# ming71/rotate-yolov3

Measured on AMD Instinct MI355X. Metric: images/sec fwd+bwd at 608^2 (train step, backend=hip), higher is better.
Workload: dtype bf16; 1 GPU; configs[3]: Darknet-53 train step (fwd + riou loss + bwd + grad all-reduce + SGD), bs=64/GPU 608x608, synthetic HRSC-shaped targets; global_batch=64, parallelism=dp1, gradients=250 MB fp32 in 4 flat buckets, fp32 on the wire

## Files before the change

### __graft_entry__.py

```python
import os
import subprocess
import sys

ROOT = os.path.dirname(os.path.abspath(__file__))
PKG = os.path.join(ROOT, "rotate-yolov3_amd")
CSRC = os.path.join(PKG, "csrc")
LIB = os.path.join(PKG, "libryolo_hip.so")
LIB_ABL = os.path.join(PKG, "libryolo_hip_ablation.so")

UNITS = {
    "rnms.hip": ["-ffp-contract=off", "-fhip-fp32-correctly-rounded-divide-sqrt"],
    "conv.hip": [],
    "conv_dispatch.hip": [],
    "conv_dgrad.hip": [],
    "conv_mp.hip": [],
    "conv_mq.hip": [],
    "conv_stem.hip": [],
    "conv_pw.hip": [],
    "conv_dil.hip": [],
    "conv0_bwd.hip": [],
    "yolo.hip": [],
    "se.hip": [],
    "se_bwd.hip": [],
    "skewiou.hip": ["-ffp-contract=off"],
    "wgrad.hip": [],
    "wgrad_dil.hip": [],
    "train.hip": [],
    "optim.hip": ["-ffp-contract=off", "-fhip-fp32-correctly-rounded-divide-sqrt"],
    "loss.hip": ["-ffp-contract=off"],
    "augment.hip": ["-ffp-contract=off", "-fhip-fp32-correctly-rounded-divide-sqrt"],
    "letterbox_area.hip": ["-ffp-contract=off", "-fhip-fp32-correctly-rounded-divide-sqrt"],
    "detpost.hip": ["-ffp-contract=off", "-fhip-fp32-correctly-rounded-divide-sqrt"],
}
COMMON = ["--offload-arch=gfx950", "-O3", "-std=c++17", "-fPIC", "-fno-gpu-rdc", "-Wno-unused-value"]


def _sha(*chunks):
    import hashlib
    h = hashlib.sha256()
    for c in chunks:
        h.update(c if isinstance(c, bytes) else str(c).encode())
        h.update(b"\0")
    return h.hexdigest()


def _headers():
    hs = [os.path.join(ROOT, "include", "ryolo.h")] + sorted(os.path.join(CSRC, h) for h in os.listdir(CSRC) if h.endswith(".h"))
    return [open(h, "rb").read() for h in hs]


def unit_hashes(defines=()):
    hdr = _headers()
    out = {}
    for unit, extra in sorted(UNITS.items()):
        src = os.path.join(CSRC, unit)
        if os.path.exists(src):
            out[unit] = _sha(open(src, "rb").read(), *hdr, " ".join(COMMON + list(defines) + extra))
    return out


def source_id(defines=()):
    hs = unit_hashes(defines)
    return _sha(*["%s=%s" % kv for kv in sorted(hs.items())])[:16]


def embedded_id(lib):
    if not os.path.exists(lib):
        return None
    data = open(lib, "rb").read()
    k = data.find(b"RYOLO_BUILD_ID=")
    return data[k + 15:k + 31].decode("ascii", "replace") if k >= 0 else None


def _compile(lib, objsuffix, defines, force=False):
    hipcc = os.environ.get("HIPCC", "hipcc")
    objs = []
    hashes = unit_hashes(defines)
    for unit, extra in UNITS.items():
        src = os.path.join(CSRC, unit)
        if not os.path.exists(src):
            continue
        obj = os.path.join(CSRC, unit.replace(".hip", objsuffix))
        side = obj + ".hash"
        have = open(side).read().strip() if os.path.exists(side) and os.path.exists(obj) else None
        if force or have != hashes[unit]:
            subprocess.run([hipcc] + COMMON + defines + extra + ["-c", src, "-o", obj], check=True)
            with open(side, "w") as fh:
                fh.write(hashes[unit])
        objs.append(obj)
    want = source_id(defines)
    if force or embedded_id(lib) != want:
        idobj = os.path.join(CSRC, "build_id" + objsuffix)
        subprocess.run([hipcc] + COMMON + defines + ['-DRYOLO_BUILD_ID="%s"' % want, "-c", os.path.join(CSRC, "build_id.hip"), "-o", idobj],
                       check=True)
        subprocess.run([hipcc, "--offload-arch=gfx950", "-shared", "-fPIC", "-o", lib] + objs + [idobj], check=True)
    assert embedded_id(lib) == want, "library %s carries id %s, sources are %s" % (lib, embedded_id(lib), want)
    return want


def build_ablation(force=False):
    _compile(LIB_ABL, ".abl.o", ["-DRYOLO_MP_ABLATION"], force)
    return LIB_ABL


def build(force=False):
    bid = _compile(LIB, ".o", [], force)
    subprocess.run(["make", "-C", os.path.join(ROOT, "oracle"), "-s"], check=True)
    if ROOT not in sys.path:
        sys.path.insert(0, ROOT)
    import rotate_yolov3_amd
    from rotate_yolov3_amd import _lib
    assert _lib.lib().ryolo_abi_version() >= 1
    got = _lib.lib().ryolo_build_id().decode()
    assert got == "RYOLO_BUILD_ID=" + bid, (got, bid)
    print("build id %s (library == sources)" % bid)


def smoke():
    if ROOT not in sys.path:
        sys.path.insert(0, ROOT)
    import numpy as np
    import torch
    assert torch.cuda.is_available(), "smoke() needs cuda:0"
    if not os.path.exists(LIB):
        build()
    from rotate_yolov3_amd import _lib
    lib_id, src_id = _lib.lib().ryolo_build_id().decode().split("=", 1)[1], source_id()
    assert lib_id == src_id, "libryolo_hip.so was built from other sources (library %s, tree %s): run build()" % (lib_id, src_id)
    print("smoke: build id %s (the loaded library is this tree's sources)" % lib_id)
    from oracle import riou
    from rotate_yolov3_amd.utils.nms.r_nms import r_nms
    dev = torch.device("cuda:0")
    d = riou.random_boxes(3000, seed=5, extent=300.0)
    keep = r_nms(torch.from_numpy(d).to(dev), 0.5).cpu().numpy()
    want = riou.rnms(d, 0.5)
    assert np.array_equal(keep, want), "rotated NMS keep list differs from the oracle"
    print("smoke: rotated NMS n=3000 kept %d, identical to the oracle" % len(keep))
    _smoke_forward(dev)


def _smoke_forward(dev):
    import torch
    import oracle
    from oracle import darknet_oracle as do
    from tests.procedural import fill_procedural
    from rotate_yolov3_amd.cfg import make_cfg
    from rotate_yolov3_amd.model.models import Darknet
    from rotate_yolov3_amd.utils.nms.nms import non_max_suppression
    torch.set_num_threads(oracle.host_cores(16))
    cfg = make_cfg.darknet53()
    m = fill_procedural(Darknet(cfg, {"context_factor": 1.0}).eval())
    x = torch.rand(1, 3, 96, 96, generator=torch.Generator().manual_seed(0))
    sd = {k: v.clone() for k, v in m.state_dict().items()}
    mg = m.to(dev)
    with torch.no_grad():
        io, p = mg(x.to(dev))
    torch.cuda.synchronize()
    io_o, _ = do.forward(cfg, sd, x, bf16=True)
    scale = io_o.abs().mean().item()
    err = (io.cpu() - io_o).abs().mean().item() / scale
    assert err < 0.01, "HIP forward differs from the oracle: mean rel err %.4g" % err
    thr = float(io[..., 5].flatten().kthvalue(int(io[..., 5].numel() * 0.8)).values)
    det = non_max_suppression(io.clone(), thr, 0.3)
    ref = do.non_max_suppression(io.cpu().clone(), thr, 0.3)
    assert (det[0] is None) == (ref[0] is None)
    if det[0] is not None:
        assert torch.equal(det[0].cpu(), ref[0]), "NMS wrapper output differs from the oracle"
    print("smoke: Darknet-53 96x96 forward on the HIP path, mean rel err vs oracle %.2e; %d detections, NMS identical"
          % (err, 0 if det[0] is None else len(det[0])))


if __name__ == "__main__":
    build(force="--force" in sys.argv)
    print("built", LIB)
    if "--ablation" in sys.argv:
        print("built", build_ablation(force="--force" in sys.argv))
```

### include/ryolo.h

```cpp
#ifndef RYOLO_H
#define RYOLO_H

#include <stddef.h>
#include <stdint.h>

#ifdef __cplusplus
extern "C" {
#endif

#define RYOLO_OK 0
#define RYOLO_EINVAL -1
#define RYOLO_ELAUNCH -2
#define RYOLO_ETOOBIG -3

#define RYOLO_RNMS_MAX_BOXES 262144

const char *ryolo_strerror(int code);
int ryolo_abi_version(void);
const char *ryolo_build_id(void);
int ryolo_set_tuning(const char *name, const char *value);

size_t ryolo_rnms_workspace_bytes(int n);
int ryolo_rnms(const float *dets, int n, int row_stride, float thr, int64_t *keep_out, int32_t *num_keep,
               void *workspace, size_t workspace_bytes, void *stream);
// ... 25 lines not shown

typedef struct ryolo_conv_desc {
    int N, H, W;
    int Cin, Cout;
    int ksize, stride, pad;
    int in_cstride, out_cstride, res_cstride;
    int act;
    float slope;
    int upsample;
    int tile;
} ryolo_conv_desc;

size_t ryolo_conv_packed_weight_bytes(int Cout, int Cin_pad, int ksize);
int ryolo_conv_pack_weights(const float *w_oihw, int Cout, int Cin, int ksize, int Cin_pad, void *packed,
                            void *stream);
int ryolo_conv2d_bn_act(const ryolo_conv_desc *desc , const void *x, const void *w_packed,
                        const float *scale, const float *shift, const void *residual , void *y,
                        void *stream);
int ryolo_conv_pair_supported(const ryolo_conv_desc *first, const ryolo_conv_desc *second, int shortcut_from_input);
int ryolo_conv2d_bn_act_pair(const ryolo_conv_desc *first, const ryolo_conv_desc *second, const void *x, const void *w_first,
                             const float *scale_first, const float *shift_first, const void *w_second, const float *scale_second,
                             const float *shift_second, int shortcut_from_input, void *y, void *stream);
#define RYOLO_CONV_KERNEL_MP256 1
#define RYOLO_CONV_KERNEL_MP192 2
#define RYOLO_CONV_KERNEL_MQ 3
#define RYOLO_CONV_KERNEL_DIRECT8 4
#define RYOLO_CONV_KERNEL_STEM 5
#define RYOLO_CONV_KERNEL_PW 6
#define RYOLO_CONV_KERNEL_STEM0 8
#define RYOLO_CONV_KERNEL_STEM_DGRAD 7
#define RYOLO_CONV_KERNEL_STEM64 11
#define RYOLO_CONV_KERNEL_MQ128 9
#define RYOLO_CONV_KERNEL_MQ64 10
#define RYOLO_CONV_KERNEL_IGEMM 16
int ryolo_conv_kernel_choice(const ryolo_conv_desc *desc, int with_residual, int with_statistics);
#define RYOLO_WGRAD_KERNEL_TAPS 1000
int ryolo_conv_dgrad_kernel_choice(const ryolo_conv_desc *forward_desc, int with_bn_reduce );
int ryolo_conv_wgrad_kernel_choice(const ryolo_conv_desc *forward_desc);
int ryolo_conv2d_dilated_supported(const ryolo_conv_desc *desc, int dil_h, int dil_w);
int ryolo_conv2d_dilated(const ryolo_conv_desc *desc, int dil_h, int dil_w, const void *x, const void *w_packed, const float *scale,
                         const float *shift, const void *residual , void *y, void *stream);
int ryolo_conv2d_dilated_dgrad_supported(const ryolo_conv_desc *forward_desc, int dil_h, int dil_w);
int ryolo_conv2d_dilated_dgrad(const ryolo_conv_desc *forward_desc, int dil_h, int dil_w, const void *dz, int dz_cstride,
                               const void *packed_dgrad, const float *ones, const float *zeros , void *dx,
                               void *stream);
int ryolo_conv2d_dilated_wgrad_supported(const ryolo_conv_desc *forward_desc, int dil_h, int dil_w);
size_t ryolo_conv2d_dilated_wgrad_workspace_bytes(const ryolo_conv_desc *forward_desc, int dil_h, int dil_w);
int ryolo_conv2d_dilated_wgrad(const ryolo_conv_desc *forward_desc, int dil_h, int dil_w, const void *x, const void *dz, int dz_cstride,
                               float *grad_oihw, int accumulate, void *workspace, size_t workspace_bytes, void *stream);
int ryolo_nchw_f32_to_nhwc_bf16(const float *x, int N, int C, int H, int W, int Cpad, void *y, void *stream);
int ryolo_nhwc_bf16_to_nchw_f32(const void *x, int N, int C, int H, int W, int cstride, float *y, void *stream);

int ryolo_aug_nparam(void);
float ryolo_aug_max_blur_sigma(void);
int ryolo_letterbox_augment(const uint8_t *pixels, const long long *img_offset, const int *img_hw , int n_cache,
                            const int *src_index , const float *params , long long seed, int N, int H, int W,
                            void *y , void *stream);

int ryolo_letterbox_area(const uint8_t *pixels, const long long *img_offset, const int *img_hw , int n_cache,
                         const int *src_index , const int *place , int N, int H, int W,
                         void *y , void *stream);

int ryolo_det_rescale(float *det , int M, const int *det_off , int bs,
                      const float *geom , void *stream);
int ryolo_det_quads(const float *det , int M, int *quad , void *stream);


int ryolo_yolo_decode_filter(const void *head, int head_cstride, int bs, int ny, int nx, int na, int no,
                             const float *anchors, float stride, float context_factor, int arc, float conf_thres,
                             float min_wh, long long io_rows_per_image, long long io_row_offset, float *cand,
                             long long *cand_row, int *counter, int capacity, void *stream);

int ryolo_yolo_decode(const void *head, int head_cstride, int bs, int ny, int nx, int na, int no,
                      const float *anchors, float stride, float context_factor, int arc, float *io,
                      long long io_rows_per_image, long long io_row_offset, float *p, void *stream);

int ryolo_conv_head_decode_supported(const ryolo_conv_desc *desc, int na, int no);
int ryolo_conv_head_decode(const ryolo_conv_desc *desc, const void *x, const void *w_packed, const float *scale, const float *shift,
                           const float *anchors, int na, int no, float stride, float context_factor, int arc, float *io,
                           long long io_rows_per_image, long long io_row_offset, float *p, void *stream);
int ryolo_conv_head_decode_store(const ryolo_conv_desc *desc, const void *x, const void *w_packed, const float *scale, const float *shift,
                                 int na, int no, void *head, int head_cstride, float *p, void *stream);

int ryolo_add_nhwc(const void *a, int a_cstride, const void *b, int b_cstride, void *y, int y_cstride,
                   long long npix, int C, void *stream);
int ryolo_upsample_nhwc(const void *x, int x_cstride, void *y, int y_cstride, int N, int H, int W, int C, int scale,
                        void *stream);
int ryolo_maxpool_nhwc(const void *x, int x_cstride, void *y, int y_cstride, int N, int H, int W, int C, int ksize,
                       int stride, void *stream);

size_t ryolo_se_workspace_bytes(int N, int H, int W, int C);
int ryolo_se_nhwc(const void *x, int x_cstride, const float *w1 , const float *w2 ,
                  int hidden, void *y, int y_cstride, int N, int H, int W, int C,
                  float *gate_out , void *workspace, size_t workspace_bytes, void *stream);
size_t ryolo_se_bwd_workspace_bytes(int N, int H, int W, int C, int hidden);
int ryolo_se_bwd_nhwc(const void *x, int x_cstride, const void *dy, int dy_cstride, const float *w1 ,
                      const float *w2 , int hidden, void *dx , int dx_cstride, int dx_accumulate,
                      float *dw1, float *dw2 , int accumulate_w, int N, int H, int W, int C,
                      float *gate_out , void *workspace, size_t workspace_bytes, void *stream);


int ryolo_conv0_recompute_supported(const ryolo_conv_desc *desc);
int ryolo_conv0_bn_act_fwd(const ryolo_conv_desc *desc, const void *x, const void *w_packed, const float *scale, const float *shift,
                           int act, const float *slope, void *y, void *stream);
size_t ryolo_conv0_bn_bwd_workspace_bytes(void);
int ryolo_conv0_bn_bwd(const ryolo_conv_desc *desc, const void *x, const void *w_packed, const void *dy, int dy_cstride,
                       const float *scale, const float *shift, const float *mean, const float *invstd, int act, const float *slope,
                       void *dz, int dz_cstride, float *dgamma, float *dbeta, float *dslope, void *workspace, size_t workspace_bytes,
                       int workspace_is_zero, void *stream);
size_t ryolo_conv0_bn_bwd_wgrad_workspace_bytes(void);
int ryolo_conv0_bn_bwd_wgrad(const ryolo_conv_desc *desc, const void *x, const void *w_packed, const void *dy, int dy_cstride,
                             const float *scale, const float *shift, const float *mean, const float *invstd, int act, const float *slope,
                             float *dgamma, float *dbeta, float *dslope, float *grad_oihw, int cin_real, int accumulate, void *workspace,
                             size_t workspace_bytes, void *stream);
int ryolo_conv_stat_rows(const ryolo_conv_desc *desc);
int ryolo_conv2d_bn_act_stats(const ryolo_conv_desc *desc, const void *x, const void *w_packed, const float *scale,
                              const float *shift, const void *residual, void *y,
                              double *stat_part ,
                              void *stream);
int ryolo_bn_finalize(double *stat_part, int rows, int cpad, int C, long long count, float eps, float momentum,
                      const float *gamma, const float *beta, float *mean, float *invstd, float *scale, float *shift,
                      float *running_mean , float *running_var, void *stream);
int ryolo_bn_act_fwd(const void *z, int z_cstride, const float *scale, const float *shift, int act,
                     const float *slope , const void *residual, int res_cstride, void *y,
                     int y_cstride, long long npix, int C, void *stream);
size_t ryolo_bn_act_bwd_workspace_bytes(long long npix, int C);
int ryolo_bn_act_bwd(const void *z, int z_cstride, const void *dy, int dy_cstride, const float *scale, const float *shift,
                     const float *mean, const float *invstd, int act, const float *slope, void *dz, int dz_cstride,
                     long long npix, int C, float *dgamma, float *dbeta, float *dslope, void *workspace,
                     size_t workspace_bytes, void *stream);
size_t ryolo_conv_packed_dgrad_bytes(int Cout, int Cin, int ksize, int stride);
int ryolo_conv_dgrad_tap_table(int ksize, int stride, int *host_out );
int ryolo_conv_pack_weights_dgrad(const float *w_oihw, int Cout, int Cin, int ksize, int stride, void *packed,
                                  const int *taps_table ,
                                  void *stream);
int ryolo_conv2d_dgrad(const ryolo_conv_desc *forward_desc, const void *dz, int dz_cstride, const void *packed_dgrad,
                       const float *ones, const float *zeros , void *dx, int accumulate, void *stream);
int ryolo_conv2d_dgrad_bnreduce_rows(const ryolo_conv_desc *forward_desc);
int ryolo_conv2d_dgrad_bnreduce(const ryolo_conv_desc *forward_desc, const void *dz, int dz_cstride, const void *packed_dgrad,
                                const float *ones, const float *zeros, void *dx, int accumulate,
                                const void *z , int z_cstride,
                                const float *scale, const float *shift, const float *mean, const float *invstd ,
                                const float *slope , float *part , void *stream);
int ryolo_bn_act_bwd_reduced(const void *z, int z_cstride, const void *dy, int dy_cstride, const float *scale, const float *shift,
                             const float *mean, const float *invstd, int act , const float *slope, void *dz,
                             int dz_cstride, long long npix, int C, float *dgamma, float *dbeta, float *dslope, const float *part,
                             int rows, void *workspace , size_t workspace_bytes, void *stream);
size_t ryolo_conv_wgrad_workspace_bytes(const ryolo_conv_desc *forward_desc);
int ryolo_conv2d_wgrad_partials(const ryolo_conv_desc *forward_desc, const void *x, const void *dz, int dz_cstride, int Cin_real,
                                float *grad_oihw, int accumulate, void *workspace, size_t workspace_bytes, void *stream);
int ryolo_conv2d_wgrad_reduce(const ryolo_conv_desc *forward_desc, const void *x, const void *dz, int dz_cstride, int Cin_real,
                              float *grad_oihw, int accumulate, void *workspace, size_t workspace_bytes, void *stream);

typedef struct ryolo_wgrad_reduce_job {
    const float *part;
    float *g;
    int S, Cout, Cin_real, Cin_k, ks, Kpad, Cout_pad, accumulate;
    int kind;
    int block_begin, block_end;
    int wide;
} ryolo_wgrad_reduce_job;
int ryolo_conv_wgrad_reduce_job_fill(ryolo_wgrad_reduce_job *host_job, const ryolo_conv_desc *forward_desc, int Cin_real, const void *workspace,
                                     float *grad_oihw, int accumulate);
int ryolo_conv_wgrad_reduce_batch(const ryolo_wgrad_reduce_job *device_jobs, int njobs, int total_blocks, void *stream);
int ryolo_conv2d_wgrad(const ryolo_conv_desc *forward_desc, const void *x, const void *dz, int dz_cstride, int Cin_real,
                       float *grad_oihw , int accumulate, void *workspace,
                       size_t workspace_bytes, void *stream);
int ryolo_upsample2x_bwd(const void *dy, int dy_cstride, void *dx, int dx_cstride, int N, int H, int W, int C,
                         int accumulate, void *stream);
int ryolo_pgrad_to_nhwc(const float *pgrad, int bs, int na, int ny, int nx, int no, void *out, int out_cstride,
                        void *stream);

typedef struct ryolo_pack_job {
    const void *src;
    void *dst;
    int kind, Cout, Cin, KS, Cin_pad, ntaps, Kpad, rows;
    int khs[9], kws[9];
    int block_begin, block_end;
} ryolo_pack_job;
int ryolo_conv_pack_job_fill(ryolo_pack_job *host_jobs, const float *w_oihw, int Cout, int Cin, int ksize, int stride,
                             int Cin_pad, void *packed_fwd, void *packed_dgrad);
int ryolo_conv_pack_batch(const ryolo_pack_job *device_jobs, int njobs, int total_blocks, void *stream);

#define RYOLO_MAX_HEADS 4
int ryolo_build_targets(const float *tpad, const unsigned char *valid, int NT, int nheads, int na, const float *const *ng,
                        const float *const *anchor_vec, float iou_t, float ang_t, float context_factor, float *const *w,
                        long long *const *idx, float *const *box, float *const *npos, void *stream);
size_t ryolo_yolo_loss_bitmap_bytes(long long cells);
int ryolo_yolo_loss(const float *p, int bs, int na, int ny, int nx, int no, int nc, const float *w, int NT,
                    const long long *b, const long long *gj, const long long *gi, const long long *cls, const float *txy,
                    const float *twh, const float *ta, const float *anchor_vec , const float *npos, float giou,
                    float reg_w, float cls_w, float cls_pw, float obj_w, float obj_pw,
                    int iou_mode ,
                    unsigned *bitmap, float *dp, float *items , void *stream);

int ryolo_yolo_loss_nhwc(const void *head, int head_cstride, const float *p, int bs, int na, int ny, int nx, int no, int nc,
                         const float *w, int NT, const long long *b, const long long *gj, const long long *gi,
                         const long long *cls, const float *txy, const float *twh, const float *ta, const float *anchor_vec,
                         const float *npos, float giou, float reg_w, float cls_w, float cls_pw, float obj_w, float obj_pw,
                         int iou_mode, unsigned *bitmap, float *dp_sparse, void *head_grad, int head_grad_cstride, float *items,
                         void *stream);
#define RYOLO_ARC_FOCAL 1
#define RYOLO_ARC_UBCE 2
#define RYOLO_ARC_UCE 4
size_t ryolo_yolo_loss_bitmap_bytes_arc(long long cells, int nc, int arc);
int ryolo_yolo_loss_arc(const float *p, int bs, int na, int ny, int nx, int no, int nc, const float *w, int NT,
                        const long long *b, const long long *gj, const long long *gi, const long long *cls, const float *txy,
                        const float *twh, const float *ta, const float *anchor_vec, const float *npos, float giou, float reg_w,
                        float cls_w, float cls_pw, float obj_w, float obj_pw, int iou_mode, int arc, float fl_gamma, unsigned *bitmap,
                        float *dp, float *items, void *stream);
int ryolo_yolo_loss_nhwc_arc(const void *head, int head_cstride, const float *p, int bs, int na, int ny, int nx, int no, int nc,
                             const float *w, int NT, const long long *b, const long long *gj, const long long *gi,
                             const long long *cls, const float *txy, const float *twh, const float *ta, const float *anchor_vec,
                             const float *npos, float giou, float reg_w, float cls_w, float cls_pw, float obj_w, float obj_pw,
                             int iou_mode, int arc, float fl_gamma, unsigned *bitmap, float *dp_sparse, void *head_grad,
                             int head_grad_cstride, float *items, void *stream);
int ryolo_scale_bf16_if(const float *g, void *buf, int cstride, long long npix, int C, void *stream);
int ryolo_bn_act_bwd_bias_order(long long npix, int C, long long *slab_pixels, int *pixel_lanes);
int ryolo_yolo_loss_bias_rows(int bs, int na, int ny, int nx, int no, int arc);
int ryolo_yolo_loss_nhwc_bias(const void *head, int head_cstride, const float *p, int bs, int na, int ny, int nx, int no, int nc,
                              const float *w, int NT, const long long *b, const long long *gj, const long long *gi,
                              const long long *cls, const float *txy, const float *twh, const float *ta, const float *anchor_vec,
                              const float *npos, float giou, float reg_w, float cls_w, float cls_pw, float obj_w, float obj_pw,
                              int iou_mode, int arc, float fl_gamma, unsigned *bitmap, float *dp_sparse, void *head_grad,
                              int head_grad_cstride, float *items, float *bias_part, int bias_cstride, void *stream);
size_t ryolo_head_bias_workspace_bytes(long long npix, int C);
int ryolo_head_bias_finalize(const float *bias_part, long long npix, int bias_cstride, int C, const float *g, float *dbias, void *workspace,
                             size_t workspace_bytes, void *stream);

int ryolo_riou_loss_pairs(const float *pbox, const float *tbox, int n, float *iou, float *grad, void *stream);

typedef struct ryolo_sgd_job {
    void *p;
    const void *g;
    void *buf;
    long long n;
    int group, first, block_begin, block_end;
} ryolo_sgd_job;
int ryolo_sgd_step(const ryolo_sgd_job *device_jobs, int njobs, int total_blocks, const float *group_hparams, int nesterov,
                   void *stream);

typedef struct ryolo_adam_job {
    void *p;
    const void *g;
    void *m;
    void *v;
    long long n;
    int row, block_begin, block_end;
} ryolo_adam_job;
int ryolo_adam_step(const ryolo_adam_job *device_jobs, int njobs, int total_blocks, const float *rows, void *stream);

#ifdef __cplusplus
}
#endif
#endif
```

### rotate-yolov3_amd/csrc/conv_common.h

```cpp
#pragma once
#include <hip/hip_runtime.h>
#include <stdint.h>
#include <stdlib.h>

#include "../../include/ryolo.h"

namespace ryolo_detail {

typedef __attribute__((ext_vector_type(8))) __bf16 bf16x8;
typedef __attribute__((ext_vector_type(4))) __bf16 bf16x4;
typedef __attribute__((ext_vector_type(2))) __bf16 bf16x2;
typedef __attribute__((ext_vector_type(4))) float f32x4;
typedef __attribute__((ext_vector_type(4))) unsigned int u32x4;
typedef __attribute__((address_space(3))) void *lds_vp;
typedef const __attribute__((address_space(1))) void *glb_vp;

constexpr int BK = 64;
constexpr long long NT_OUT_MIN_BYTES = 128ll << 20;
constexpr int STAT_ROWS = 128;

struct ConvParams {
    const __bf16 *x;
    const __bf16 *w;
    const float *scale;
// ... 125 lines not shown
    hipStream_t stream = nullptr;
    const BnRed *bnred = nullptr;
};

struct IgemmTile {
    int code, BM, BN, WGM, WGN, NSTAGE;
};
constexpr IgemmTile IGEMM_TILES[] = {{1, 128, 128, 2, 4, 2}, {2, 256, 64, 4, 1, 2}, {3, 256, 32, 4, 1, 2},
                                     {4, 256, 128, 4, 2, 3}, {6, 128, 128, 4, 2, 2}, {7, 128, 128, 2, 2, 2}};
constexpr int IGEMM_NTILES = sizeof(IGEMM_TILES) / sizeof(IGEMM_TILES[0]);
constexpr const IgemmTile *igemm_tile(int code) {
    for (int i = 0; i < IGEMM_NTILES; i++)
        if (IGEMM_TILES[i].code == code) return &IGEMM_TILES[i];
    return nullptr;
}

struct ConvPlan {
    int kernel = -1;
    int ksize = 0;
    int bm = 0;
    bool persist = false;
    int grid = 0;
    int rows = 0;
    int variant = 0;
};

inline int cu_count() {
    static const int cus = [] {
        int dev = 0, n = 0;
        return hipGetDevice(&dev) == hipSuccess && hipDeviceGetAttribute(&n, hipDeviceAttributeMultiprocessorCount, dev) == hipSuccess && n > 0 ? n : 256;
    }();
    return cus;
}

template <auto KFN, typename... Args>
int launch_kernel(dim3 grid, dim3 block, size_t smem, hipStream_t stream, Args... args) {
    if (smem > 64 * 1024) {
        static const hipError_t raised = hipFuncSetAttribute((const void *)KFN, hipFuncAttributeMaxDynamicSharedMemorySize, (int)smem);
        if (raised != hipSuccess) return RYOLO_ELAUNCH;
    }
    hipLaunchKernelGGL(KFN, grid, block, smem, stream, args...);
    return hipGetLastError() == hipSuccess ? RYOLO_OK : RYOLO_ELAUNCH;
}

inline bool buffer_extent(unsigned long long npix, long long cs, long long c, unsigned *bytes = nullptr) {
    const unsigned long long b = ((npix - 1) * (unsigned long long)cs + (unsigned long long)c) * 2ull;
    if (b >= 0x7fffff00ull) return false;
    if (bytes) *bytes = (unsigned)b;
    return true;
}

struct PersistGrid {
    int grid, nt;
    long long tiles;
    bool deep, exact;
};
inline PersistGrid persist_grid(long long M, int BM, int Cout, int BN, int Ho, int Wo, bool force = false, int rounds2 = 5) {
    const long long mt = (M + BM - 1) / BM, nt = (Cout + BN - 1) / BN, dmax = Wo > Ho ? Wo : Ho;
    PersistGrid g;
    g.grid = (2 * cu_count()) & ~7;
    g.nt = (int)nt;
    g.tiles = mt * nt;
    g.deep = force ? g.tiles > g.grid : 2 * g.tiles >= (long long)rounds2 * g.grid;
    g.exact = g.grid >= 8 && mt * BM * dmax < 0x100000000ll && g.tiles * nt < 0x100000000ll;
    return g;
}

inline unsigned magic_u32(int d) { return d <= 1 ? 0u : (unsigned)((0x100000000ull + (unsigned)d - 1) / (unsigned)d); }

struct TileList {
    int nt;
    long long T;
    unsigned y_bytes, res_bytes;
    bool fits;
};
inline TileList tile_list(const ConvParams &p, int bm, int bn) {
    TileList t;
    const long long mt = ((long long)p.M + bm - 1) / bm, dmax = p.Wo > p.Ho ? p.Wo : p.Ho;
    t.nt = (p.Cout + bn - 1) / bn;
    t.T = mt * t.nt;
    const unsigned long long yb = (((unsigned long long)p.N * p.OH * p.OW - 1) * p.out_cs + p.Cout) * 2ull;
    const unsigned long long rb = p.res ? (((unsigned long long)p.N * p.OH * p.OW - 1) * p.res_cs + p.Cout) * 2ull : 0ull;
    t.fits = mt * bm * dmax < 0x100000000ll && t.T * t.nt < 0x100000000ll && t.T <= 0x7fffffffll && yb < 0x7fffff00ull && rb < 0x7fffff00ull;
    t.y_bytes = (unsigned)yb;
    t.res_bytes = (unsigned)rb;
    return t;
}
inline void set_tile_list(ConvParams &p, const TileList &t) {
    p.nt = t.nt;
    p.ntiles = (int)t.T;
    p.use_magic = 1;
    p.magic_wo = magic_u32(p.Wo);
    p.magic_ho = magic_u32(p.Ho);
    p.magic_nt = magic_u32(p.nt);
    p.y_bytes = t.y_bytes;
    p.res_bytes = t.res_bytes;
}

inline int grid_for(long long total, int tb = 256, int cap = 32768) {
    long long nb = (total + tb - 1) / tb;
    return (int)(nb < 1 ? 1 : (nb > cap ? cap : nb));
}

inline int ilog2_exact(int v) {
    int l = 0;
    while ((1 << l) < v) l++;
    return (1 << l) == v ? l : -1;
}

int conv_validate(const ryolo_conv_desc *d);
bool conv_shape(const ryolo_conv_desc *d, ConvParams &p);
bool conv_pixels(ConvParams &p, long long Ho, long long Wo);
bool conv0_shape(const ryolo_conv_desc *d, int out_cs);
bool conv0_params(const ryolo_conv_desc *d, int out_cs, ConvParams &p, int gpw, unsigned *nblk);
bool conv0_halo_on();
ConvPlan conv_plan(const ConvParams &p, int ksize, int pick, bool want_reduce);
int conv_launch(const ConvPlan &pl, ConvParams &p, const ConvLaunch &lc);
long long nt_out_min_bytes();

bool conv_igemm_plan(const ConvParams &p, int ksize, int tile, bool no_persist, bool force_persist, bool reduce, ConvPlan &pl);
int launch_conv_igemm(const ConvPlan &pl, ConvParams &p, const ConvLaunch &lc);
int launch_conv0_direct(const ConvPlan &pl, ConvParams &p, const ConvLaunch &lc);
bool conv_mp_eligible(const ConvParams &p);
int conv_mp_pick_bm(const ConvParams &p);
bool conv_mp_plan(const ConvParams &p, int bm, int variant, ConvPlan &pl);
int launch_conv_mp(const ConvPlan &pl, ConvParams &p, const ConvLaunch &lc);
bool conv_mq_plan(const ConvParams &p, int variant, ConvPlan &pl);
int launch_conv_mq(const ConvPlan &pl, ConvParams &p, const ConvLaunch &lc);
bool conv_mq128_eligible(const ConvParams &p);
bool conv_mq128_plan(const ConvParams &p, int bm, bool reduce, ConvPlan &pl);
int launch_conv_mq128(const ConvPlan &pl, ConvParams &p, const ConvLaunch &lc);
bool conv_stem_plan(const ConvParams &p, int ksize, ConvPlan &pl);
int launch_conv_stem(const ConvPlan &pl, ConvParams &p, const ConvLaunch &lc);
bool conv_stem64_plan(const ConvParams &p, int ksize, ConvPlan &pl);
int launch_conv_stem64(const ConvPlan &pl, ConvParams &p, const ConvLaunch &lc);
int launch_conv0_halo(ConvParams &p, const float *slope_dev, int round_z, const ConvLaunch &lc);
bool conv_stem_dgrad_plan(const ryolo_conv_desc *d, int dz_cs, ConvPlan &pl);
int launch_conv_stem_dgrad(const ConvPlan &pl, const ryolo_conv_desc *d, const void *dz, int dz_cs, const void *w_classes, void *dx, int accumulate,
                           int nt_out, const ConvLaunch &lc);
int conv_stem_pair_kind(const ryolo_conv_desc *first, const ryolo_conv_desc *second, int shortcut_from_input);
int launch_conv_stem_pair(int kind, ConvParams &p , const void *x, unsigned x_bytes, int in_cs, int H, int W,
                          const void *w_first, int kpad_first, const float *scale_first, const float *shift_first, int act_first,
                          float slope_first, hipStream_t stream);
bool conv_pw_plan(const ConvParams &p, int ksize, bool reduce, ConvPlan &pl);
bool conv_pw_preferred(const ConvParams &p);
int launch_conv_pw(const ConvPlan &pl, ConvParams &p, const ConvLaunch &lc);
bool conv_pw_decode_supported(const ConvParams &p, int na, int no);
int launch_conv_pw_decode(ConvParams &p, float *io, long long io_img_rows, long long io_row0, float *pout, const float *anchors, int na, int no,
                          float stride, float cf, int arc, hipStream_t stream, void *head = nullptr, int head_cs = 0);
#ifdef RYOLO_MP_ABLATION
int ryolo_mp_ablation_variant(int slot);
#endif

enum TuneKey { TUNE_CONV3X3 = 0, TUNE_CONV1X1, TUNE_RNMS_TILES, TUNE_MQ_KORDER, TUNE_BN_REDUCE_TILES, TUNE_STEM_DGRAD, TUNE_COUNT };
const char *tune(TuneKey k);
#ifdef RYOLO_MP_ABLATION
inline const char *abl_env(const char *name) { return getenv(name); }
#else
inline const char *abl_env(const char *) { return nullptr; }
#endif

}
```

### rotate-yolov3_amd/csrc/train.hip

```cpp
#include "conv_common.h"

using namespace ryolo_detail;

namespace {

__global__ void __launch_bounds__(1024) bn_finalize_kernel(double *__restrict__ part, int R, int cpad, int C, float count, float eps,
                                   float momentum, const float *__restrict__ gamma, const float *__restrict__ beta,
                                   float *__restrict__ mean, float *__restrict__ invstd, float *__restrict__ scale,
                                   float *__restrict__ shift, float *__restrict__ run_mean, float *__restrict__ run_var) {
    __shared__ double red[2][32][33];
    const int cx = threadIdx.x & 31, ry = threadIdx.x >> 5;
    const int c = blockIdx.x * 32 + cx;
    double s = 0.0, q = 0.0;
    if (c < C) {
        for (int r0 = ry; r0 < R; r0 += 32 * 8) {
            double a[8], b[8];
#pragma unroll
            for (int u = 0; u < 8; u++) {
                const int r = r0 + 32 * u;
                a[u] = r < R ? part[(size_t)r * 2 * cpad + c] : 0.0;
                b[u] = r < R ? part[(size_t)r * 2 * cpad + cpad + c] : 0.0;
            }
#pragma unroll
            for (int u = 0; u < 8; u++) {
                const int r = r0 + 32 * u;
                s += a[u];
                q += b[u];
                if (r < R) {
                    part[(size_t)r * 2 * cpad + c] = 0.0;
                    part[(size_t)r * 2 * cpad + cpad + c] = 0.0;
                }
            }
        }
    }
    red[0][ry][cx] = s;
    red[1][ry][cx] = q;
    __syncthreads();
    if (ry != 0 || c >= C) return;
    for (int k = 1; k < 32; k++) { s += red[0][k][cx]; q += red[1][k][cx]; }
    const double mu = s / count;
    double var = q / count - mu * mu;
    if (var < 0) var = 0;
    const float is = (float)(1.0 / sqrt(var + (double)eps));
    mean[c] = (float)mu;
    invstd[c] = is;
    scale[c] = gamma[c] * is;
    shift[c] = beta[c] - (float)mu * gamma[c] * is;
    if (run_mean) {
        const double unb = count > 1.f ? var * count / (count - 1.0) : var;
        run_mean[c] = (1.f - momentum) * run_mean[c] + momentum * (float)mu;
        run_var[c] = (1.f - momentum) * run_var[c] + momentum * (float)unb;
    }
}

__device__ __forceinline__ float mish_f(float x) {
    const float e = __expf(fminf(x, 20.f));
    const float n = (1.f + e) * (1.f + e);
    return x * (n - 1.f) / (n + 1.f);
}
__device__ __forceinline__ float mish_grad(float x) {
    const float e = __expf(fminf(x, 20.f));
    const float n = (1.f + e) * (1.f + e);
    const float t = (n - 1.f) / (n + 1.f);
    return t + x * (1.f - t * t) * (e / (1.f + e));
}

constexpr long long NT_MIN_BYTES = 128ll << 20;
#ifdef RYOLO_MP_ABLATION
static int g_nt[3] = {-1, -1, -1};
inline bool nt_pass(int kind, long long npix, int C) { return g_nt[kind] < 0 ? npix * C * 2 >= NT_MIN_BYTES : g_nt[kind] != 0; }
#else
inline bool nt_pass(int, long long npix, int C) { return npix * C * 2 >= NT_MIN_BYTES; }
#endif
template <bool NTL>
__device__ __forceinline__ bf16x8 ld8(const __bf16 *p) {
    if constexpr (NTL) return __builtin_nontemporal_load((const bf16x8 *)p);
    else return *(const bf16x8 *)p;
}
template <bool NTL>
__device__ __forceinline__ void st8(__bf16 *p, const bf16x8 &v) {
    if constexpr (NTL) __builtin_nontemporal_store(v, (bf16x8 *)p);
    else *(bf16x8 *)p = v;
}

template <int ACT, bool NTL = false>
__global__ void bn_act_fwd_kernel(const __bf16 *__restrict__ z, int z_cs, const float *__restrict__ scale,
                                  const float *__restrict__ shift, const float *__restrict__ slope_p,
                                  const __bf16 *__restrict__ res, int res_cs, __bf16 *__restrict__ y, int y_cs,
                                  long long npix, int C) {
    const int cpr = C / 8;
    const long long total = npix * cpr;
    const float slope = slope_p ? slope_p[0] : 0.f;
    for (long long i = (long long)blockIdx.x * blockDim.x + threadIdx.x; i < total;
         i += (long long)gridDim.x * blockDim.x) {
        const long long pix = i / cpr;
        const int c = (int)(i % cpr) * 8;
        const bf16x8 v = ld8<NTL>(z + pix * z_cs + c);
        bf16x8 o;
#pragma unroll
        for (int e = 0; e < 8; e++) {
            float u = (float)v[e] * scale[c + e] + shift[c + e];
            if (ACT == 1) u = u > 0.f ? u : u * slope;
            else if (ACT == 2) u = mish_f(u);
            o[e] = (__bf16)u;
        }
        if (res) {
            const bf16x8 r = ld8<NTL>(res + pix * res_cs + c);
#pragma unroll
            for (int e = 0; e < 8; e++) o[e] = (__bf16)((float)o[e] + (float)r[e]);
        }
        st8<NTL>(y + pix * y_cs + c, o);
    }
}

constexpr int BWD_SLAB_MIN = 128;
#ifdef RYOLO_MP_ABLATION
static int g_bwd_slabs = 1024, g_bwd_slab_min = BWD_SLAB_MIN;
inline long long bwd_slab(long long npix) {
    long long s = (npix + g_bwd_slabs - 1) / g_bwd_slabs;
    return s < g_bwd_slab_min ? g_bwd_slab_min : s;
}
#else
inline long long bwd_slab(long long npix) {
    const long long s = (npix + 1023) / 1024;
    return s < BWD_SLAB_MIN ? BWD_SLAB_MIN : s;
}
#endif
template <int ACT, bool NTL = false>
__global__ void __launch_bounds__(256)
bn_act_bwd_reduce_kernel(const __bf16 *__restrict__ z, int z_cs, const __bf16 *__restrict__ dy, int dy_cs,
                         const float *__restrict__ scale, const float *__restrict__ shift,
                         const float *__restrict__ mean, const float *__restrict__ invstd,
                         const float *__restrict__ slope_p, long long npix, int C, int CT, float *__restrict__ part, long long SL) {
    __shared__ float red[256][25];
    const int cl = threadIdx.x % CT, pl = threadIdx.x / CT, npl = 256 / CT;
    const int c = (blockIdx.x * CT + cl) * 8;
    const int slab = blockIdx.y;
    const long long p0 = (long long)slab * SL;
    const long long p1 = p0 + SL < npix ? p0 + SL : npix;
    const float slope = slope_p ? slope_p[0] : 0.f;
    float s1[8], s2[8], s3[8];
#pragma unroll
    for (int e = 0; e < 8; e++) s1[e] = s2[e] = s3[e] = 0.f;
    if (c < C) {
        float sc[8], sh[8], mu[8], is[8];
#pragma unroll
        for (int e = 0; e < 8; e++) {
            sc[e] = scale ? scale[c + e] : 1.f; sh[e] = scale ? shift[c + e] : 0.f;
            mu[e] = scale ? mean[c + e] : 0.f; is[e] = scale ? invstd[c + e] : 0.f;
        }
        auto accum = [&](const bf16x8 &zv, const bf16x8 &gv) {
#pragma unroll
            for (int e = 0; e < 8; e++) {
// ... 8 lines not shown
                s1[e] += g;
            }
        };
        long long pix = p0 + pl;
        for (; pix + 3 * npl < p1; pix += 4 * npl) {
            bf16x8 zv[4], gv[4];
#pragma unroll
            for (int k = 0; k < 4; k++) {
                zv[k] = ld8<NTL>(z + (pix + k * npl) * z_cs + c);
                gv[k] = ld8<NTL>(dy + (pix + k * npl) * dy_cs + c);
            }
#pragma unroll
            for (int k = 0; k < 4; k++) accum(zv[k], gv[k]);
        }
        for (; pix < p1; pix += npl) accum(*(const bf16x8 *)(z + pix * z_cs + c), *(const bf16x8 *)(dy + pix * dy_cs + c));
#pragma unroll
        for (int e = 0; e < 8; e++) s2[e] *= is[e];
    }
#pragma unroll
    for (int e = 0; e < 8; e++) { red[threadIdx.x][e] = s1[e]; red[threadIdx.x][8 + e] = s2[e]; red[threadIdx.x][16 + e] = s3[e]; }
    __syncthreads();
    for (int t = threadIdx.x; t < CT * 24; t += 256) {
        const int l = t / 24, k = t % 24;
        float v = 0.f;
        for (int q = 0; q < npl; q++) v += red[q * CT + l][k];
        const int ch = (blockIdx.x * CT + l) * 8 + (k & 7);
        if (ch < C) part[((size_t)slab * 3 + (k >> 3)) * C + ch] = v;
    }
}

__global__ void __launch_bounds__(1024)
bn_act_bwd_finalize_kernel(const float *__restrict__ part, int nslab, int C, float *__restrict__ s1o,
                           float *__restrict__ s2o, float *__restrict__ dgamma, float *__restrict__ dbeta,
                           float *__restrict__ s3o) {
    __shared__ float red[3][32][33];
    const int cx = threadIdx.x & 31, ry = threadIdx.x >> 5;
    const int c = blockIdx.x * 32 + cx;
    float a = 0.f, b = 0.f, d = 0.f;
    if (c < C) {
        for (int s0 = ry; s0 < nslab; s0 += 32 * 8) {
            float va[8], vb[8], vd[8];
#pragma unroll
            for (int u = 0; u < 8; u++) {
                const int s = s0 + 32 * u;
                va[u] = s < nslab ? part[((size_t)s * 3 + 0) * C + c] : 0.f;
                vb[u] = s < nslab ? part[((size_t)s * 3 + 1) * C + c] : 0.f;
                vd[u] = s < nslab ? part[((size_t)s * 3 + 2) * C + c] : 0.f;
            }
#pragma unroll
            for (int u = 0; u < 8; u++) { a += va[u]; b += vb[u]; d += vd[u]; }
        }
    }
    red[0][ry][cx] = a; red[1][ry][cx] = b; red[2][ry][cx] = d;
    __syncthreads();
    if (ry != 0) return;
    for (int k = 1; k < 32; k++) { a += red[0][k][cx]; b += red[1][k][cx]; d += red[2][k][cx]; }
    if (c < C) {
        s1o[c] = a;
        s2o[c] = b;
        if (dgamma) dgamma[c] += b;
        if (dbeta) dbeta[c] += a;
        if (s3o) s3o[c] = d;
    }
}

constexpr int BWD_FOLD = 64, BWD_FOLD_MIN_ROWS = 2048;
__global__ void __launch_bounds__(1024)
bn_act_bwd_fold_kernel(const float *__restrict__ part, int nrows, int C, int per, float *__restrict__ out) {
    __shared__ float red[3][32][33];
    const int cx = threadIdx.x & 31, ry = threadIdx.x >> 5;
    const int c = blockIdx.x * 32 + cx, g = blockIdx.y;
    const int r0 = g * per, r1 = min(nrows, r0 + per);
    float a = 0.f, b = 0.f, d = 0.f;
    if (c < C) {
        for (int s0 = r0 + ry; s0 < r1; s0 += 32 * 4) {
            float va[4], vb[4], vd[4];
#pragma unroll
            for (int u = 0; u < 4; u++) {
                const int s = s0 + 32 * u;
                va[u] = s < r1 ? part[((size_t)s * 3 + 0) * C + c] : 0.f;
                vb[u] = s < r1 ? part[((size_t)s * 3 + 1) * C + c] : 0.f;
                vd[u] = s < r1 ? part[((size_t)s * 3 + 2) * C + c] : 0.f;
            }
#pragma unroll
            for (int u = 0; u < 4; u++) { a += va[u]; b += vb[u]; d += vd[u]; }
        }
    }
    red[0][ry][cx] = a; red[1][ry][cx] = b; red[2][ry][cx] = d;
    __syncthreads();
    if (ry != 0 || c >= C) return;
    for (int k = 1; k < 32; k++) { a += red[0][k][cx]; b += red[1][k][cx]; d += red[2][k][cx]; }
    out[((size_t)g * 3 + 0) * C + c] = a;
    out[((size_t)g * 3 + 1) * C + c] = b;
    out[((size_t)g * 3 + 2) * C + c] = d;
}

__global__ void __launch_bounds__(256)
head_bias_lanes_kernel(const float *__restrict__ rows, int npl, int cs, int C, float *__restrict__ out) {
    const int c = blockIdx.x * 256 + threadIdx.x, slab = blockIdx.y;
    if (c >= C) return;
    float v = 0.f;
    for (int q = 0; q < npl; q++) v += rows[((size_t)slab * npl + q) * cs + c];
    out[(size_t)slab * C + c] = v;
}

__global__ void __launch_bounds__(1024)
head_bias_finalize_kernel(const float *__restrict__ part, int nslab, int C, const float *__restrict__ gsc, float *__restrict__ dbias) {
    __shared__ float red[32][33];
    const int cx = threadIdx.x & 31, ry = threadIdx.x >> 5;
    const int c = blockIdx.x * 32 + cx;
    float a = 0.f;
    if (c < C) {
        for (int s0 = ry; s0 < nslab; s0 += 32 * 8) {
            float va[8];
#pragma unroll
            for (int u = 0; u < 8; u++) {
                const int s = s0 + 32 * u;
                va[u] = s < nslab ? part[(size_t)s * C + c] : 0.f;
            }
#pragma unroll
            for (int u = 0; u < 8; u++) a += va[u];
        }
    }
    red[ry][cx] = a;
    __syncthreads();
    if (ry != 0 || c >= C) return;
    for (int k = 1; k < 32; k++) a += red[k][cx];
    dbias[c] += gsc[0] * a;
}

template <int ACT, bool NTL = false>
__global__ void __launch_bounds__(256) bn_act_bwd_apply_kernel(const __bf16 *__restrict__ z, int z_cs, const __bf16 *__restrict__ dy, int dy_cs,
                                        const float *__restrict__ scale, const float *__restrict__ shift,
                                        const float *__restrict__ mean, const float *__restrict__ invstd,
                                        const float *__restrict__ s1, const float *__restrict__ s2, float inv_count,
                                        const float *__restrict__ slope_p, __bf16 *__restrict__ dz, int dz_cs,
                                        long long npix, int C, const float *__restrict__ s3, float *__restrict__ dslope) {
    if (dslope && blockIdx.x == 0 && threadIdx.x < 64) {
        float v = 0.f;
        for (int c = threadIdx.x; c < C; c += 64) v += s3[c];
#pragma unroll
        for (int o = 32; o > 0; o >>= 1) v += __shfl_xor(v, o);
        if (threadIdx.x == 0) dslope[0] += v;
    }
    const int cpr = C / 8;
    const long long total = npix * cpr;
    const float slope = slope_p ? slope_p[0] : 0.f;
    const long long stride = (long long)gridDim.x * blockDim.x;
    long long i = (long long)blockIdx.x * blockDim.x + threadIdx.x;
    if (stride % cpr == 0) {
        if (i >= total) return;
        const int c = (int)(i % cpr) * 8;
        const long long dp = stride / cpr;
        float sc[8], sh[8], kb[8], kd[8];
#pragma unroll
        for (int e = 0; e < 8; e++) {
            sc[e] = scale[c + e];
            sh[e] = shift[c + e];
            const float k = sc[e] * invstd[c + e] * s2[c + e] * inv_count;
            kb[e] = -k;
            kd[e] = k * mean[c + e] - sc[e] * s1[c + e] * inv_count;
        }
        auto one = [&](const bf16x8 &zv, const bf16x8 &gv) {
            bf16x8 o;
#pragma unroll
            for (int e = 0; e < 8; e++) {
                const float zf = (float)zv[e];
                float g = (float)gv[e];
                const float u = zf * sc[e] + sh[e];
                if (ACT == 1 && u <= 0.f) g *= slope;
                else if (ACT == 2) g *= mish_grad(u);
                o[e] = (__bf16)(sc[e] * g + (kb[e] * zf + kd[e]));
            }
            return o;
        };
        long long pix = i / cpr;
        for (; pix + 3 * dp < npix; pix += 4 * dp) {
            bf16x8 zv[4], gv[4];
#pragma unroll
            for (int k = 0; k < 4; k++) {
                zv[k] = ld8<NTL>(z + (pix + k * dp) * z_cs + c);
                gv[k] = ld8<NTL>(dy + (pix + k * dp) * dy_cs + c);
            }
#pragma unroll
            for (int k = 0; k < 4; k++) st8<NTL>(dz + (pix + k * dp) * dz_cs + c, one(zv[k], gv[k]));
        }
        for (; pix < npix; pix += dp)
            *(bf16x8 *)(dz + pix * dz_cs + c) = one(*(const bf16x8 *)(z + pix * z_cs + c), *(const bf16x8 *)(dy + pix * dy_cs + c));
        return;
    }
    for (; i < total; i += stride) {
        const long long pix = i / cpr;
        const int c = (int)(i % cpr) * 8;
        const bf16x8 zv = *(const bf16x8 *)(z + pix * z_cs + c);
        const bf16x8 gv = *(const bf16x8 *)(dy + pix * dy_cs + c);
        bf16x8 o;
#pragma unroll
        for (int e = 0; e < 8; e++) {
            const float zf = (float)zv[e];
            float g = (float)gv[e];
            const float u = zf * scale[c + e] + shift[c + e];
            if (ACT == 1 && u <= 0.f) g *= slope;
            else if (ACT == 2) g *= mish_grad(u);
            const float xh = (zf - mean[c + e]) * invstd[c + e];
            o[e] = (__bf16)(scale[c + e] * (g - s1[c + e] * inv_count - xh * s2[c + e] * inv_count));
        }
        *(bf16x8 *)(dz + pix * dz_cs + c) = o;
    }
}

__global__ void upsample2x_bwd_kernel(const __bf16 *__restrict__ dy, int dy_cs, __bf16 *__restrict__ dx, int dx_cs, int N,
                                      int H, int W, int C, int accumulate) {
    const int cpr = C / 8;
    const long long total = (long long)N * H * W * cpr;
    for (long long i = (long long)blockIdx.x * blockDim.x + threadIdx.x; i < total;
         i += (long long)gridDim.x * blockDim.x) {
        const int c = (int)(i % cpr) * 8;
        const long long pix = i / cpr;
        const int w = (int)(pix % W);
        const long long t = pix / W;
        const int h = (int)(t % H);
        const long long n = t / H;
        float s[8];
#pragma unroll
        for (int e = 0; e < 8; e++) s[e] = 0.f;
        for (int a = 0; a < 2; a++)
            for (int b = 0; b < 2; b++) {
                const bf16x8 v = *(const bf16x8 *)(dy + ((n * 2 * H + 2 * h + a) * 2 * W + 2 * w + b) * dy_cs + c);
#pragma unroll
                for (int e = 0; e < 8; e++) s[e] += (float)v[e];
            }
        bf16x8 o;
        if (accumulate) {
            const bf16x8 old = *(const bf16x8 *)(dx + pix * dx_cs + c);
#pragma unroll
            for (int e = 0; e < 8; e++) s[e] += (float)old[e];
        }
#pragma unroll
        for (int e = 0; e < 8; e++) o[e] = (__bf16)s[e];
        *(bf16x8 *)(dx + pix * dx_cs + c) = o;
    }
}

__global__ void pgrad_to_nhwc_kernel(const float *__restrict__ g, int bs, int na, int ny, int nx, int no,
                                     __bf16 *__restrict__ out, int out_cs) {
    const long long total = (long long)bs * na * ny * nx * no;
    for (long long i = (long long)blockIdx.x * blockDim.x + threadIdx.x; i < total;
         i += (long long)gridDim.x * blockDim.x) {
        const int k = (int)(i % no);
        long long t = i / no;
        const int x = (int)(t % nx); t /= nx;
        const int y = (int)(t % ny); t /= ny;
        const int a = (int)(t % na);
        const long long n = t / na;
        out[((n * ny + y) * nx + x) * out_cs + a * no + k] = (__bf16)g[i];
    }
}

constexpr int PG_PIX = 32;
__global__ void __launch_bounds__(256) pgrad_to_nhwc_tiled_kernel(const float *__restrict__ g, int na, int plane, int no,
                                                                  __bf16 *__restrict__ out, int out_cs, int npix) {
    extern __shared__ __attribute__((aligned(16))) __bf16 pg_lds[];
    const int C = na * no;
    const int p0 = blockIdx.x * PG_PIX;
    const int per_a = PG_PIX * no;
    for (int idx = threadIdx.x; idx < na * per_a; idx += 256) {
        const int a = idx / per_a, rem = idx - a * per_a;
        const int pl = rem / no, k = rem - pl * no;
        const int gp = p0 + pl;
        if (gp < npix) {
            const int n = gp / plane, pp = gp - n * plane;
            pg_lds[pl * C + a * no + k] = (__bf16)g[((size_t)(n * na + a) * plane + pp) * no + k];
        }
    }
    __syncthreads();
    const int cpr = C / 8;
    for (int idx = threadIdx.x; idx < PG_PIX * cpr; idx += 256) {
        const int pl = idx / cpr, c = (idx - pl * cpr) * 8;
        if (p0 + pl < npix) *(bf16x8 *)(out + (size_t)(p0 + pl) * out_cs + c) = *(const bf16x8 *)(pg_lds + pl * C + c);
    }
}

constexpr int ELEM_BLOCKS = 4096;
inline int ok_launch() { return hipGetLastError() == hipSuccess ? RYOLO_OK : RYOLO_ELAUNCH; }

}

extern "C" {

int ryolo_bn_finalize(double *stat_part, int rows, int cpad, int C, long long count, float eps, float momentum,
                      const float *gamma, const float *beta, float *mean, float *invstd, float *scale, float *shift,
                      float *running_mean, float *running_var, void *stream) {
    if (!stat_part || !gamma || !beta || !mean || !invstd || !scale || !shift || rows <= 0 || C <= 0 || count <= 0)
        return RYOLO_EINVAL;
    hipLaunchKernelGGL(bn_finalize_kernel, dim3((C + 31) / 32), dim3(1024), 0, (hipStream_t)stream, stat_part, rows, cpad, C,
                       (float)count, eps, momentum, gamma, beta, mean, invstd, scale, shift, running_mean, running_var);
    return ok_launch();
}

int ryolo_bn_act_fwd(const void *z, int z_cstride, const float *scale, const float *shift, int act, const float *slope,
                     const void *residual, int res_cstride, void *y, int y_cstride, long long npix, int C, void *stream) {
    if (!z || !scale || !shift || !y || npix <= 0 || C <= 0 || (C & 7) || (z_cstride & 7) || (y_cstride & 7))
        return RYOLO_EINVAL;
    if (act < 0 || act > 2) return RYOLO_EINVAL;
    const bool ntl = nt_pass(0, npix, C);
#define RYOLO_BN_FWD(A)                                                                                                   \
    hipLaunchKernelGGL((ntl ? bn_act_fwd_kernel<A, true> : bn_act_fwd_kernel<A, false>), dim3(grid_for(npix * (C / 8))), dim3(256), 0, (hipStream_t)stream,           \
                       (const __bf16 *)z, z_cstride, scale, shift, slope, (const __bf16 *)residual, res_cstride,          \
                       (__bf16 *)y, y_cstride, npix, C)
    if (act == 0) RYOLO_BN_FWD(0); else if (act == 1) RYOLO_BN_FWD(1); else RYOLO_BN_FWD(2);
#undef RYOLO_BN_FWD
    return ok_launch();
}

size_t ryolo_bn_act_bwd_workspace_bytes(long long npix, int C) {
    const long long nslab = (npix + bwd_slab(npix) - 1) / bwd_slab(npix);
    return (size_t)nslab * 3 * C * 4 + (size_t)3 * C * 4;
}

static int bn_act_bwd_impl(const void *z, int z_cstride, const void *dy, int dy_cstride, const float *scale, const float *shift,
                           const float *mean, const float *invstd, int act, const float *slope, void *dz, int dz_cstride,
                           long long npix, int C, float *dgamma, float *dbeta, float *dslope, void *workspace,
                           size_t workspace_bytes, const float *pre_part, int pre_rows, void *stream_);

int ryolo_bn_act_bwd(const void *z, int z_cstride, const void *dy, int dy_cstride, const float *scale, const float *shift,
                     const float *mean, const float *invstd, int act, const float *slope, void *dz, int dz_cstride,
                     long long npix, int C, float *dgamma, float *dbeta, float *dslope, void *workspace,
                     size_t workspace_bytes, void *stream_) {
    return bn_act_bwd_impl(z, z_cstride, dy, dy_cstride, scale, shift, mean, invstd, act, slope, dz, dz_cstride, npix, C, dgamma, dbeta,
                           dslope, workspace, workspace_bytes, nullptr, 0, stream_);
}

int ryolo_bn_act_bwd_reduced(const void *z, int z_cstride, const void *dy, int dy_cstride, const float *scale, const float *shift,
                             const float *mean, const float *invstd, int act, const float *slope, void *dz, int dz_cstride,
                             long long npix, int C, float *dgamma, float *dbeta, float *dslope, const float *part, int rows,
                             void *workspace, size_t workspace_bytes, void *stream_) {
    if (!part || rows <= 0 || !scale || act != 1) return RYOLO_EINVAL;
    return bn_act_bwd_impl(z, z_cstride, dy, dy_cstride, scale, shift, mean, invstd, act, slope, dz, dz_cstride, npix, C, dgamma, dbeta,
                           dslope, workspace, workspace_bytes, part, rows, stream_);
}

static int bn_act_bwd_impl(const void *z, int z_cstride, const void *dy, int dy_cstride, const float *scale, const float *shift,
                           const float *mean, const float *invstd, int act, const float *slope, void *dz, int dz_cstride,
                           long long npix, int C, float *dgamma, float *dbeta, float *dslope, void *workspace,
                           size_t workspace_bytes, const float *pre_part, int pre_rows, void *stream_) {
    if (!z || !dy || npix <= 0 || C <= 0 || (C & 7) || (z_cstride & 7) || (dy_cstride & 7) || !workspace) return RYOLO_EINVAL;
    if (workspace_bytes < (pre_part ? (size_t)3 * C * 4 : ryolo_bn_act_bwd_workspace_bytes(npix, C))) return RYOLO_EINVAL;
    if (scale && (!shift || !mean || !invstd || !dz || (dz_cstride & 7))) return RYOLO_EINVAL;
    hipStream_t stream = (hipStream_t)stream_;
    int nslab = pre_part ? pre_rows : (int)((npix + bwd_slab(npix) - 1) / bwd_slab(npix));
    float *part = pre_part ? const_cast<float *>(pre_part) : (float *)workspace;
    float *s1 = pre_part ? (float *)workspace : part + (size_t)nslab * 3 * C, *s2 = s1 + C, *s3 = s2 + C;
    if (pre_part && pre_rows >= BWD_FOLD_MIN_ROWS && workspace_bytes >= (size_t)(3 + 3 * BWD_FOLD) * C * 4) {
        float *folded = s3 + C;
        const int per = (pre_rows + BWD_FOLD - 1) / BWD_FOLD;
        hipLaunchKernelGGL(bn_act_bwd_fold_kernel, dim3((C + 31) / 32, BWD_FOLD), dim3(1024), 0, stream, part, pre_rows, C, per, folded);
        part = folded;
        nslab = (pre_rows + per - 1) / per;
    }
    float *dsl = (scale && act == 1) ? dslope : nullptr;
    int CT = 32;
    while (CT > 1 && CT > C / 8) CT >>= 1;
    if (act < 0 || act > 2) return RYOLO_EINVAL;
    const bool nt_red = nt_pass(1, npix, C), nt_app = nt_pass(2, npix, C);
#define RYOLO_BN_REDK(A) (nt_red ? bn_act_bwd_reduce_kernel<A, true> : bn_act_bwd_reduce_kernel<A, false>)
#define RYOLO_BN_RED(A)                                                                                                   \
    hipLaunchKernelGGL(RYOLO_BN_REDK(A), dim3((C / 8 + CT - 1) / CT, nslab), dim3(256), 0, stream,             \
                       (const __bf16 *)z, z_cstride, (const __bf16 *)dy, dy_cstride, scale, shift, mean, invstd, slope,   \
                       npix, C, CT, part, bwd_slab(npix))
    if (pre_part) {  }
    else if (act == 0) RYOLO_BN_RED(0); else if (act == 1) RYOLO_BN_RED(1); else RYOLO_BN_RED(2);
#undef RYOLO_BN_RED
    hipLaunchKernelGGL(bn_act_bwd_finalize_kernel, dim3((C + 31) / 32), dim3(1024), 0, stream, part, nslab, C, s1, s2,
                       scale ? dgamma : nullptr, dbeta, dsl ? s3 : nullptr);
#define RYOLO_BN_APP(A)                                                                                                   \
    hipLaunchKernelGGL((nt_app ? bn_act_bwd_apply_kernel<A, true> : bn_act_bwd_apply_kernel<A, false>), dim3(grid_for(npix * (C / 8), 256, ELEM_BLOCKS)), dim3(256), 0, stream,                  \
                       (const __bf16 *)z, z_cstride, (const __bf16 *)dy, dy_cstride, scale, shift, mean, invstd, s1, s2,  \
                       1.0f / (float)npix, slope, (__bf16 *)dz, dz_cstride, npix, C, s3, dsl)
    if (scale) {
        if (act == 0) RYOLO_BN_APP(0); else if (act == 1) RYOLO_BN_APP(1); else RYOLO_BN_APP(2);
    }
#undef RYOLO_BN_APP
    return ok_launch();
}

int ryolo_bn_act_bwd_bias_order(long long npix, int C, long long *slab_pixels, int *pixel_lanes) {
    if (npix <= 0 || C <= 0 || (C & 7) || !slab_pixels || !pixel_lanes) return 0;
    int CT = 32;
    while (CT > 1 && CT > C / 8) CT >>= 1;
    const long long SL = bwd_slab(npix), nslab = (npix + SL - 1) / SL;
    if (nslab > 0x7fffffffll) return 0;
    *slab_pixels = SL;
    *pixel_lanes = 256 / CT;
    return (int)nslab;
}

size_t ryolo_head_bias_workspace_bytes(long long npix, int C) {
    long long SL;
    int npl;
    const int nslab = ryolo_bn_act_bwd_bias_order(npix, C, &SL, &npl);
    return (size_t)nslab * C * 4;
}

int ryolo_head_bias_finalize(const float *bias_part, long long npix, int bias_cstride, int C, const float *g, float *dbias, void *workspace,
                             size_t workspace_bytes, void *stream_) {
    long long SL;
    int npl;
    const int nslab = ryolo_bn_act_bwd_bias_order(npix, C, &SL, &npl);
    if (!bias_part || !g || !dbias || nslab <= 0 || bias_cstride < C || !workspace || workspace_bytes < (size_t)nslab * C * 4 || nslab > 65535)
        return RYOLO_EINVAL;
    hipStream_t stream = (hipStream_t)stream_;
    hipLaunchKernelGGL(head_bias_lanes_kernel, dim3((C + 255) / 256, nslab), dim3(256), 0, stream, bias_part, npl, bias_cstride, C,
                       (float *)workspace);
    hipLaunchKernelGGL(head_bias_finalize_kernel, dim3((C + 31) / 32), dim3(1024), 0, stream, (const float *)workspace, nslab, C, g, dbias);
    return ok_launch();
}

#ifdef RYOLO_MP_ABLATION
void ryolo_debug_bn_set(int slabs, int slab_min, int nt_fwd, int nt_red, int nt_app) {
    g_bwd_slabs = slabs; g_bwd_slab_min = slab_min; g_nt[0] = nt_fwd; g_nt[1] = nt_red; g_nt[2] = nt_app;
}
#endif

int ryolo_upsample2x_bwd(const void *dy, int dy_cstride, void *dx, int dx_cstride, int N, int H, int W, int C,
                         int accumulate, void *stream) {
    if (!dy || !dx || N <= 0 || H <= 0 || W <= 0 || C <= 0 || (C & 7) || (dy_cstride & 7) || (dx_cstride & 7))
        return RYOLO_EINVAL;
    hipLaunchKernelGGL(upsample2x_bwd_kernel, dim3(grid_for((long long)N * H * W * (C / 8))), dim3(256), 0,
                       (hipStream_t)stream, (const __bf16 *)dy, dy_cstride, (__bf16 *)dx, dx_cstride, N, H, W, C, accumulate);
    return ok_launch();
}

int ryolo_pgrad_to_nhwc(const float *pgrad, int bs, int na, int ny, int nx, int no, void *out, int out_cstride,
                        void *stream) {
    if (!pgrad || !out || bs <= 0 || na <= 0 || ny <= 0 || nx <= 0 || no <= 0 || out_cstride < na * no) return RYOLO_EINVAL;
    const long long npix = (long long)bs * ny * nx;
    const size_t smem = (size_t)PG_PIX * na * no * 2;
    if ((na * no) % 8 == 0 && (out_cstride & 7) == 0 && (((uintptr_t)out) & 15) == 0 && smem <= 64 * 1024 && npix < 0x7fffffffll) {
        hipLaunchKernelGGL(pgrad_to_nhwc_tiled_kernel, dim3((unsigned)((npix + PG_PIX - 1) / PG_PIX)), dim3(256), smem,
                           (hipStream_t)stream, pgrad, na, ny * nx, no, (__bf16 *)out, out_cstride, (int)npix);
        return ok_launch();
    }
    hipLaunchKernelGGL(pgrad_to_nhwc_kernel, dim3(grid_for((long long)bs * na * ny * nx * no)), dim3(256), 0,
                       (hipStream_t)stream, pgrad, bs, na, ny, nx, no, (__bf16 *)out, out_cstride);
    return ok_launch();
}

}
```

### rotate-yolov3_amd/csrc/wgrad.hip

```cpp
#include "conv_common.h"

using namespace ryolo_detail;

namespace {

typedef short s16x4 __attribute__((ext_vector_type(4)));
typedef short s16x8 __attribute__((ext_vector_type(8)));

__device__ __forceinline__ s16x4 lds_read_tr16(const char *addr) {
#if defined(__HIP_DEVICE_COMPILE__)
    return __builtin_amdgcn_ds_read_tr16_b64_v4i16((__attribute__((address_space(3))) s16x4 *)(addr));
#else
    return s16x4{0, 0, 0, 0};
#endif
}

template <int T>
__device__ __forceinline__ int wg_swz(int row) {
    if (T >= 128) return (row & 3) | (((row >> 3) & 1) << 2);
    if (T == 64) return ((row >> 1) & 1) | (((row >> 3) & 1) << 1);
    return (row >> 3) & 1;
}

typedef int i32x4 __attribute__((ext_vector_type(4)));
__device__ __forceinline__ i32x4 make_rsrc_words(const void *base, unsigned bytes) {
    const unsigned long long a = (unsigned long long)base;
    i32x4 r;
    r[0] = __builtin_amdgcn_readfirstlane((int)(unsigned)a);
    r[1] = __builtin_amdgcn_readfirstlane((int)(unsigned)(a >> 32));
    r[2] = __builtin_amdgcn_readfirstlane((int)bytes);
    r[3] = 0x00020000;
    return r;
}
__device__ __forceinline__ void buffer_load_lds16_raw(i32x4 rsrc, unsigned lds_addr , int voffset) {
#if defined(__HIP_DEVICE_COMPILE__)
    asm volatile("s_mov_b32 m0, %0\n\ts_nop 0\n\tbuffer_load_dwordx4 %1, %2, 0 offen lds" ::"s"(lds_addr), "v"(voffset), "s"(rsrc) : "memory", "m0");
#endif
}

constexpr int KP = 64;

struct WgradParams {
    const __bf16 *x;
    const __bf16 *dz;
    float *part;
    int N, H, W, Cin, x_cs;
    int Ho, Wo, Cout, dz_cs;
    int ks, stride, pad;
    int Kpad, Cout_pad;
    int M;
    int S, chunk;
    int co_tiles, ci_tiles;
    unsigned x_bytes, dz_bytes;
};

template <int T>
__global__ void __launch_bounds__(256) wgrad_kernel(const WgradParams p) {
    constexpr int WT = T / 2, NF = WT / 16;
    constexpr int CHUNKS = T / 8;
    constexpr int ROWB = T * 2;
    constexpr int TILE_B = KP * ROWB;
    constexpr int PIECES = TILE_B / 1024;
    constexpr int PPW = PIECES / 4 > 0 ? PIECES / 4 : 1;
    constexpr int PIX_PER_PIECE = 64 / CHUNKS;
    static_assert(PIECES % 4 == 0 || PIECES < 4, "pieces must split over the 4 waves");
    extern __shared__ __attribute__((aligned(16))) char smem[];

    const int tid = threadIdx.x, lane = tid & 63;
    const int wave = __builtin_amdgcn_readfirstlane(tid >> 6);
    int b = blockIdx.x;
    {
        const int per = gridDim.x >> 3;
        if (b < per * 8) b = (b & 7) * per + (b >> 3);
    }
    const int ci_t = b % p.ci_tiles; b /= p.ci_tiles;
    const int co_t = b % p.co_tiles; b /= p.co_tiles;
    const int tap = b % (p.ks * p.ks); b /= (p.ks * p.ks);
    const int split = b;
    const int kh = tap / p.ks, kw = tap % p.ks;
    const int co0 = co_t * T, ci0 = ci_t * T;
    const int pix_lo = split * p.chunk, pix_hi = min(p.M, pix_lo + p.chunk);

    const int lp = lane / CHUNKS, lc = lane % CHUNKS;
    int a_off[PPW], b_img[PPW], b_ho[PPW], b_wo[PPW], s_pix[PPW];
#pragma unroll
    for (int j = 0; j < PPW; j++) {
        const int piece = wave * PPW + j;
        const int tp = piece * PIX_PER_PIECE + lp;
        s_pix[j] = tp;
        const int pg = pix_lo + tp;
        const int chunk = lc ^ (wg_swz<T>(tp) << 1);
        a_off[j] = (int)(((long long)pg * p.dz_cs + co0 + chunk * 8) * 2);
        b_wo[j] = pg % p.Wo;
        const int t = pg / p.Wo;
        b_ho[j] = t % p.Ho;
        b_img[j] = t / p.Ho;
    }
    const bool piece_active = (wave * PPW) < PIECES;

    auto stage = [&](int kt, int buf) {
        char *abuf = smem + buf * 2 * TILE_B;
        char *bbuf = abuf + TILE_B;
#pragma unroll
        for (int j = 0; j < PPW; j++) {
            if (!piece_active) continue;
            const int piece = wave * PPW + j;
            const int pg = pix_lo + kt * KP + s_pix[j];
            const int chunk = lc ^ (wg_swz<T>(s_pix[j]) << 1);
            const bool in_rng = pg < pix_hi;
            const bool a_ok = in_rng && (co0 + chunk * 8 < p.Cout);
            const int a_v = a_ok ? a_off[j] + kt * KP * p.dz_cs * 2 : (int)0x80000000;
            buffer_load_lds16(p.dz, p.dz_bytes, abuf + piece * 1024, a_v, 0);
            const int hi = b_ho[j] * p.stride - p.pad + kh, wi = b_wo[j] * p.stride - p.pad + kw;
            const bool b_ok = in_rng && (unsigned)hi < (unsigned)p.H && (unsigned)wi < (unsigned)p.W &&
                              (ci0 + chunk * 8 < p.Cin);
            const int b_v = b_ok ? (int)((((long long)(b_img[j] * p.H + hi) * p.W + wi) * p.x_cs + ci0 + chunk * 8) * 2)
                                 : (int)0x80000000;
            buffer_load_lds16(p.x, p.x_bytes, bbuf + piece * 1024, b_v, 0);
            b_wo[j] += KP;
            while (b_wo[j] >= p.Wo) {
                b_wo[j] -= p.Wo;
                if (++b_ho[j] == p.Ho) { b_ho[j] = 0; b_img[j]++; }
            }
        }
    };

    const int wr = wave >> 1, wc = wave & 1;
    const int fr = lane & 15, kg = lane >> 4;
    const int trow = kg * 8 + (fr >> 2);
    const int tsw = wg_swz<T>(trow);
    const int tbase = trow * ROWB + (fr & 3) * 8;
    int offa[NF], offb[NF];
#pragma unroll
    for (int f = 0; f < NF; f++) {
        offa[f] = tbase + ((((wr * WT) >> 4) + f) ^ tsw) * 32;
        offb[f] = tbase + ((((wc * WT) >> 4) + f) ^ tsw) * 32;
    }

    f32x4 acc[NF][NF];
#pragma unroll
    for (int a = 0; a < NF; a++)
#pragma unroll
        for (int c = 0; c < NF; c++) acc[a][c] = f32x4{0.f, 0.f, 0.f, 0.f};

    const int nsteps = (pix_hi - pix_lo + KP - 1) / KP;
    if (nsteps > 0) stage(0, 0);
    for (int kt = 0; kt < nsteps; kt++) {
        __syncthreads();
        if (kt + 1 < nsteps) stage(kt + 1, (kt + 1) & 1);
        const char *abuf = smem + (kt & 1) * 2 * TILE_B;
        const char *bbuf = abuf + TILE_B;
#pragma unroll
        for (int ks = 0; ks < 2; ks++) {
            bf16x8 af[NF], bfr[NF];
#pragma unroll
            for (int f = 0; f < NF; f++) {
                const s16x4 a0 = lds_read_tr16(abuf + offa[f] + (ks * 32) * ROWB);
                const s16x4 a1 = lds_read_tr16(abuf + offa[f] + (ks * 32 + 4) * ROWB);
                const s16x4 b0 = lds_read_tr16(bbuf + offb[f] + (ks * 32) * ROWB);
                const s16x4 b1 = lds_read_tr16(bbuf + offb[f] + (ks * 32 + 4) * ROWB);
                af[f] = __builtin_bit_cast(bf16x8, __builtin_shufflevector(a0, a1, 0, 1, 2, 3, 4, 5, 6, 7));
                bfr[f] = __builtin_bit_cast(bf16x8, __builtin_shufflevector(b0, b1, 0, 1, 2, 3, 4, 5, 6, 7));
            }
#pragma unroll
            for (int a = 0; a < NF; a++)
#pragma unroll
                for (int c = 0; c < NF; c++)
                    acc[a][c] = __builtin_amdgcn_mfma_f32_16x16x32_bf16(af[a], bfr[c], acc[a][c], 0, 0, 0);
        }
    }
    float *out = p.part + (size_t)split * p.Cout_pad * p.Kpad;
#pragma unroll
    for (int a = 0; a < NF; a++)
#pragma unroll
        for (int c = 0; c < NF; c++)
#pragma unroll
            for (int r = 0; r < 4; r++) {
                const int co = co0 + wr * WT + a * 16 + kg * 4 + r;
                const int ci = ci0 + wc * WT + c * 16 + fr;
                if (co < p.Cout && ci < p.Cin) out[(size_t)co * p.Kpad + tap * p.Cin + ci] = acc[a][c][r];
            }
}

template <int TM, int TN, int ABL = 0, int NW = 4, int NT = 1>
__global__ void __launch_bounds__(NW * 64, NW == 8 ? (TM * TN > 256 * 128 ? 2 : 4) : 1) wgrad_wide_kernel(const WgradParams p) {
    constexpr int KPX = 32, NST = 3;
    constexpr int WM = TM / (NW / 2), WN = NT * TN / 2, NFA = WM / 16, NFB = WN / 16;
    constexpr int ROW_A = TM * 2, ROW_B = TN * 2;
    constexpr int TILE_A = KPX * ROW_A, TILE_B = KPX * ROW_B, STAGE = TILE_A + NT * TILE_B;
    constexpr int CH_A = TM / 8, CH_B = TN / 8;
    constexpr int PPP_A = 64 / CH_A, PPP_B = 64 / CH_B;
// ... 715 lines not shown
        if (S > nsteps) S = nsteps;
        if (S < 1) S = 1;
        const long long per = (nsteps + S - 1) / S;
        w.S = (int)((nsteps + per - 1) / per);
        w.chunk = (int)per;
    } else {
        const int mn = d->Cin < d->Cout ? d->Cin : d->Cout;
        const bool square = d->tile & 0x2000;
        const int co256 = (d->Cout + 255) / 256;
        w.kernel = mn >= 128 ? WG_SQ128 : (mn >= 64 ? WG_SQ64 : WG_SQ32);
        if (d->Cout >= 256 && (co256 * 256 - d->Cout) * 8 <= 256 && d->Cin % 128 == 0 && !square) {
            w.kernel = WG_256x128;
#ifdef RYOLO_MP_ABLATION
            if (g_wgrad_abl == 9 && d->Cin % 256 == 0) w.kernel = WG_ABL_256x256;
#endif
        } else if (d->Cout % 128 == 0 && d->Cin == 64 && ks == 3 && !square) {
            w.kernel = WG_128x3x64;
#ifdef RYOLO_MP_ABLATION
            if (g_wgrad_abl == 11) w.kernel = WG_ABL_128x64;
#endif
        } else if (d->Cout == 64 && d->Cin % 128 == 0 && !square) {
            w.kernel = WG_64x128;
        } else if (d->Cout % 128 == 0 && d->Cin % 128 == 0 && !square) {
            w.kernel = WG_128x128;
        } else if (d->Cout % 128 == 0 && d->Cin % 256 == 0 && (d->tile & 0x4000)) {
            w.kernel = WG_128x256;
        }
        const WgradTile t = wgrad_tile(w.kernel);
        w.Cout_pad = (d->Cout + 127) / 128 * 128;
        w.co_tiles = (d->Cout + t.tm - 1) / t.tm;
        w.ci_tiles = (d->Cin + t.tn - 1) / t.tn;
        w.tap_groups = ks * ks / t.taps;
        const int base = w.co_tiles * w.ci_tiles * w.tap_groups;
        const int target = (ks == 3 ? t.split3 : t.split1) * (d->Cin <= 8 ? 2 : 1);
        int S = target / base;
        if (2 * base > target) {
            double best = -1.0;
            for (int c = 1; c <= 5; c++) {
                const int blocks = c * base;
                const double eff = (double)blocks / (double)((blocks + 511) / 512 * 512);
                if (eff > best + 0.02) { best = eff; S = c; }
            }
        }
        if (forced_s) S = forced_s;
        const long long max_s = (M + KP - 1) / KP;
        if (S > max_s) S = (int)max_s;
        const size_t per = (size_t)w.Cout_pad * w.Kpad * 4;
        while (S > 1 && per * S > (size_t)512 << 20) S--;
        if (S < 1) S = 1;
        long long chunk = (M + S - 1) / S;
        chunk = (chunk + KP - 1) / KP * KP;
        w.S = (int)((M + chunk - 1) / chunk);
        w.chunk = (int)chunk;
    }
    const WgradTile t = wgrad_tile(w.kernel);
    w.blocks = (unsigned)(w.co_tiles * w.ci_tiles * w.tap_groups * w.S);
    w.threads = (unsigned)t.waves * 64;
    w.lds = (size_t)t.lds;
    w.part_bytes = (size_t)w.S * w.Cout_pad * w.Kpad * 4;
    const long long total = (long long)d->Cout * Cin_real * ks * ks;
    if (w.S < 8 && ks == 3 && Cin_real % 64 == 0 && total >= (1 << 20)) {
        w.reduce_kind = 2;
        w.reduce_blocks = (unsigned)(d->Cout * (Cin_real / 64));
    } else {
        w.reduce_kind = w.S >= 8 ? 1 : 0;
        w.reduce_blocks = (unsigned)grid_for(total, w.S >= 8 ? 64 : 256);
    }
    return w;
}

template <int K>
int launch_wgrad_tiles(const WgradPlan &w, const WgradParams &p, hipStream_t stream) {
    constexpr WgradTile t = wgrad_tile(K);
    const dim3 grid(w.blocks), block(w.threads);
#ifdef RYOLO_MP_ABLATION
    if constexpr (K == WG_256x128) {
#define RYOLO_WG_ABL(A, NW) \
    if (g_wgrad_abl == (NW == 8 ? 8 : A)) return launch_kernel<wgrad_wide_kernel<t.tm, t.tn, A, NW>>(grid, dim3(NW * 64), w.lds, stream, p);
        RYOLO_WG_ABL(1, 4) RYOLO_WG_ABL(2, 4) RYOLO_WG_ABL(4, 4) RYOLO_WG_ABL(6, 4) RYOLO_WG_ABL(7, 4) RYOLO_WG_ABL(0, 8)
#undef RYOLO_WG_ABL
    }
#endif
    if constexpr (t.stages == 2) return launch_kernel<wgrad_kernel<t.tm>>(grid, block, w.lds, stream, p);
    else return launch_kernel<wgrad_wide_kernel<t.tm, t.tn, 0, t.waves, t.taps>>(grid, block, w.lds, stream, p);
}

template <int CO, int CI, int KS, int ST>
int launch_wgrad_taps(const WgradPlan &w, const WgradParams &p, hipStream_t stream) {
    WgradTapsParams q;
    q.x = p.x; q.dz = p.dz; q.part = p.part;
    q.N = p.N; q.H = p.H; q.W = p.W; q.x_cs = p.x_cs; q.Ho = p.Ho; q.Wo = p.Wo; q.dz_cs = p.dz_cs; q.pad = p.pad;
    q.Cout = p.Cout; q.Kpad = p.Kpad;
    q.nseg = w.nseg; q.nsteps = w.nsteps; q.steps_per_split = w.chunk;
    q.x_bytes = p.x_bytes; q.dz_bytes = p.dz_bytes;
    return launch_kernel<wgrad_taps_kernel<CO, CI, KS, ST>>(dim3(w.blocks), dim3(w.threads), w.lds, stream, q);
}

enum WgradPhase { WG_BOTH, WG_TILES_ONLY, WG_REDUCE_ONLY };

int wgrad_launch(const WgradPlan &w, const ryolo_conv_desc *d, const void *x, const void *dz, int dz_cstride, int Cin_real, float *grad_oihw,
                 int accumulate, void *workspace, WgradPhase phase, hipStream_t stream) {
    WgradParams p;
    p.x = (const __bf16 *)x; p.dz = (const __bf16 *)dz; p.part = (float *)workspace;
    p.N = d->N; p.H = d->H; p.W = d->W; p.Cin = d->Cin; p.x_cs = d->in_cstride;
    p.Ho = w.Ho; p.Wo = w.Wo; p.Cout = d->Cout; p.dz_cs = dz_cstride;
    p.ks = d->ksize; p.stride = d->stride; p.pad = d->pad;
    p.Kpad = w.Kpad; p.Cout_pad = w.Cout_pad; p.M = w.M;
    p.S = w.S; p.chunk = w.chunk; p.co_tiles = w.co_tiles; p.ci_tiles = w.ci_tiles;
    if (!buffer_extent((unsigned long long)d->N * d->H * d->W, d->in_cstride, d->Cin, &p.x_bytes) ||
        !buffer_extent((unsigned long long)w.M, dz_cstride, d->Cout, &p.dz_bytes))
        return RYOLO_EINVAL;
    int rc = RYOLO_OK;
    if (phase != WG_REDUCE_ONLY) switch (w.kernel) {
    case WG_TAPS + 1: rc = launch_wgrad_taps<64, 32, 3, 1>(w, p, stream); break;
    case WG_TAPS + 2: rc = launch_wgrad_taps<64, 32, 3, 2>(w, p, stream); break;
    case WG_TAPS + 3: rc = launch_wgrad_taps<32, 64, 1, 1>(w, p, stream); break;
    case WG_TAPS + 4: rc = launch_wgrad_taps<32, 8, 3, 1>(w, p, stream); break;
    case WG_256x128: rc = launch_wgrad_tiles<WG_256x128>(w, p, stream); break;
    case WG_128x256: rc = launch_wgrad_tiles<WG_128x256>(w, p, stream); break;
    case WG_128x3x64: rc = launch_wgrad_tiles<WG_128x3x64>(w, p, stream); break;
    case WG_128x128: rc = launch_wgrad_tiles<WG_128x128>(w, p, stream); break;
    case WG_64x128: rc = launch_wgrad_tiles<WG_64x128>(w, p, stream); break;
#ifdef RYOLO_MP_ABLATION
    case WG_ABL_256x256: rc = launch_wgrad_tiles<WG_ABL_256x256>(w, p, stream); break;
    case WG_ABL_128x64: rc = launch_wgrad_tiles<WG_ABL_128x64>(w, p, stream); break;
#endif
    case WG_SQ128: rc = launch_wgrad_tiles<WG_SQ128>(w, p, stream); break;
    case WG_SQ64: rc = launch_wgrad_tiles<WG_SQ64>(w, p, stream); break;
    default: rc = launch_wgrad_tiles<WG_SQ32>(w, p, stream); break;
    }
    if (rc != RYOLO_OK || phase == WG_TILES_ONLY) return rc;
    const float *part = (const float *)workspace;
    const dim3 grid(w.reduce_blocks), block(256);
    if (w.reduce_kind == 2)
        return launch_kernel<wgrad_reduce_t3_kernel>(grid, block, 0, stream, part, w.S, Cin_real, d->Cin, w.Kpad, w.Cout_pad, grad_oihw, accumulate);
    if (w.reduce_kind == 1)
        return launch_kernel<wgrad_reduce_kernel<4>>(grid, block, 0, stream, part, w.S, d->Cout, Cin_real, d->Cin, d->ksize, w.Kpad, w.Cout_pad,
                                                     grad_oihw, accumulate);
    return launch_kernel<wgrad_reduce_kernel<1>>(grid, block, 0, stream, part, w.S, d->Cout, Cin_real, d->Cin, d->ksize, w.Kpad, w.Cout_pad, grad_oihw,
                                                 accumulate);
}

int wgrad_call(WgradPhase phase, const ryolo_conv_desc *d, const void *x, const void *dz, int dz_cstride, int Cin_real, float *grad_oihw,
               int accumulate, void *workspace, size_t workspace_bytes, void *stream) {
    if (!x || !dz || !grad_oihw || !workspace || !wgrad_validate(d)) return RYOLO_EINVAL;
    if ((d->Cin & 7) || (d->Cout & 7) || (d->in_cstride & 7) || (dz_cstride & 7) || Cin_real <= 0 || Cin_real > d->Cin) return RYOLO_EINVAL;
    const WgradPlan w = wgrad_plan(d, Cin_real);
    if (workspace_bytes < w.part_bytes) return RYOLO_EINVAL;
    return wgrad_launch(w, d, x, dz, dz_cstride, Cin_real, grad_oihw, accumulate, workspace, phase, (hipStream_t)stream);
}

}

extern "C" {

#ifdef RYOLO_MP_ABLATION
void ryolo_debug_wgrad_set(int abl) { g_wgrad_abl = abl; }
#endif

size_t ryolo_conv_wgrad_workspace_bytes(const ryolo_conv_desc *d) { return wgrad_validate(d) ? wgrad_plan(d, d->Cin).part_bytes : 0; }

int ryolo_conv_wgrad_kernel_choice(const ryolo_conv_desc *d) { return wgrad_validate(d) ? wgrad_plan(d, d->Cin).kernel : -1; }

int ryolo_conv2d_wgrad(const ryolo_conv_desc *d, const void *x, const void *dz, int dz_cstride, int Cin_real, float *grad_oihw, int accumulate,
                       void *workspace, size_t workspace_bytes, void *stream) {
    return wgrad_call(WG_BOTH, d, x, dz, dz_cstride, Cin_real, grad_oihw, accumulate, workspace, workspace_bytes, stream);
}
int ryolo_conv2d_wgrad_partials(const ryolo_conv_desc *d, const void *x, const void *dz, int dz_cstride, int Cin_real, float *grad_oihw,
                                int accumulate, void *workspace, size_t workspace_bytes, void *stream) {
    return wgrad_call(WG_TILES_ONLY, d, x, dz, dz_cstride, Cin_real, grad_oihw, accumulate, workspace, workspace_bytes, stream);
}
int ryolo_conv2d_wgrad_reduce(const ryolo_conv_desc *d, const void *x, const void *dz, int dz_cstride, int Cin_real, float *grad_oihw,
                              int accumulate, void *workspace, size_t workspace_bytes, void *stream) {
    return wgrad_call(WG_REDUCE_ONLY, d, x, dz, dz_cstride, Cin_real, grad_oihw, accumulate, workspace, workspace_bytes, stream);
}

int ryolo_conv_wgrad_reduce_job_fill(ryolo_wgrad_reduce_job *job, const ryolo_conv_desc *d, int Cin_real, const void *workspace, float *grad_oihw,
                                     int accumulate) {
    if (!job || !workspace || !grad_oihw || !wgrad_validate(d) || Cin_real <= 0 || Cin_real > d->Cin) return 0;
    const WgradPlan w = wgrad_plan(d, Cin_real);
    *job = ryolo_wgrad_reduce_job{};
    job->part = (const float *)workspace; job->g = grad_oihw; job->accumulate = accumulate ? 1 : 0;
    job->S = w.S; job->Cout = d->Cout; job->Cin_real = Cin_real; job->Cin_k = d->Cin; job->ks = d->ksize;
    job->Kpad = w.Kpad; job->Cout_pad = w.Cout_pad; job->kind = w.reduce_kind;
    unsigned blocks = w.reduce_blocks;
    const char *env = abl_env("RYOLO_WGRAD_REDUCE_V4");
    const bool v4 = !(env && env[0] == '0'), t3v = !(env && (env[0] == '0' || env[0] == '1'));
    const int wide = !(env && env[0] >= '0' && env[0] <= '2');
    const long long step_bytes = (long long)w.Cout_pad * w.Kpad * 4;
    if (job->kind == 1 && v4 && Cin_real % 4 == 0 && d->Cin % 4 == 0 && ((uintptr_t)workspace & 15) == 0 &&
        ((w.S + 3) / 4 + 17) * step_bytes < (1ll << 31)) {
        job->kind = 3;
        job->wide = wide;
        blocks = (unsigned)grid_for((long long)d->Cout * Cin_real * d->ksize * d->ksize, 256 * (wide ? wgrad_reduce_v4_groups(w.S) : 1));
    }
    if (job->kind == 2 && t3v && w.S < 8 && 8 * step_bytes < (1ll << 31)) {
        job->kind = 4;
        job->wide = wide;
        const int r = wide ? wgrad_reduce_t3v_units_per_block(w.S) : 1;
        blocks = (blocks + r - 1) / r;
    }
    job->block_begin = 0;
    job->block_end = (int)blocks;
    return (int)blocks;
}

int ryolo_conv_wgrad_reduce_batch(const ryolo_wgrad_reduce_job *device_jobs, int njobs, int total_blocks, void *stream) {
    if (!device_jobs || njobs <= 0 || total_blocks <= 0) return RYOLO_EINVAL;
    return launch_kernel<wgrad_reduce_batch_kernel>(dim3((unsigned)total_blocks), dim3(256), 0, (hipStream_t)stream, device_jobs, njobs);
}

}
```

### rotate-yolov3_amd/model/hip_train_ops.py

```python
import ctypes as C

import torch

from .. import _lib
from .._lib import PackJob, WgradReduceJob
from . import hip_ops
from .hip_ops import ConvDesc, _check_nhwc, cpad, pack_weights

ARC_FOCAL, ARC_UBCE, ARC_UCE = 1, 2, 4


def arc_flags(arc):
    f = ARC_FOCAL if 'F' in arc else 0
    if 'default' in arc:
        return f
    if 'BCE' in arc:
        return f | ARC_UBCE
    if 'CE' in arc:
        return f | ARC_UCE
    raise ValueError("unknown arc %r" % (arc,))


class WgradReduceBatch(object):

# ... 116 lines not shown


def conv0_bn_bwd(d, x, packed_w, dy, stats, act, slope, dz, dgamma, dbeta, dslope, ws, ws_is_zero=True):
    mean, invstd, scale, shift = stats
    _lib.check(_lib.lib().ryolo_conv0_bn_bwd(C.byref(d), x.data_ptr(), packed_w.data_ptr(), dy.data_ptr(), dy.stride(2),
                                             scale.data_ptr(), shift.data_ptr(), mean.data_ptr(), invstd.data_ptr(), act,
                                             slope.data_ptr() if slope is not None else None, dz.data_ptr(), dz.stride(2),
                                             dgamma.data_ptr(), dbeta.data_ptr(), dslope.data_ptr() if dslope is not None else None,
                                             ws.data_ptr(), ws.numel(), 1 if ws_is_zero else 0, _s(x.device)), "ryolo_conv0_bn_bwd")
    return dz


def conv0_bn_bwd_wgrad_ws(device):
    return torch.empty(_lib.lib().ryolo_conv0_bn_bwd_wgrad_workspace_bytes(), dtype=torch.uint8, device=device)


def conv0_bn_bwd_wgrad(d, x, packed_w, dy, stats, act, slope, dgamma, dbeta, dslope, grad_w, cin_real, accumulate, ws):
    mean, invstd, scale, shift = stats
    _lib.check(_lib.lib().ryolo_conv0_bn_bwd_wgrad(C.byref(d), x.data_ptr(), packed_w.data_ptr(), dy.data_ptr(), dy.stride(2),
                                                   scale.data_ptr(), shift.data_ptr(), mean.data_ptr(), invstd.data_ptr(), act,
                                                   slope.data_ptr() if slope is not None else None, dgamma.data_ptr(), dbeta.data_ptr(),
                                                   dslope.data_ptr() if dslope is not None else None, grad_w.data_ptr(), int(cin_real),
                                                   1 if accumulate else 0, ws.data_ptr(), ws.numel(), _s(x.device)), "ryolo_conv0_bn_bwd_wgrad")


def conv_fwd_plain(d, x, packed_w, ones, shift, z):
    d.out_cstride = _check_nhwc(z, "z")
    _lib.check(_lib.lib().ryolo_conv2d_bn_act(C.byref(d), x.data_ptr(), packed_w.data_ptr(), ones.data_ptr(), shift.data_ptr(),
                                              None, z.data_ptr(), _s(x.device)), "ryolo_conv2d_bn_act")


def conv_head_decode_store(hf, x, packed_w, ones, shift, head, p):
    d = ConvDesc(*hf['desc'])
    d.in_cstride = _check_nhwc(x, "x")
    hcs = _check_nhwc(head, "head")
    if not p.is_contiguous() or p.dtype != torch.float32:
        raise ValueError("conv_head_decode_store: p must be contiguous fp32")
    _lib.check(_lib.lib().ryolo_conv_head_decode_store(C.byref(d), x.data_ptr(), packed_w.data_ptr(), ones.data_ptr(), shift.data_ptr(),
                                                       hf['na'], hf['no'], head.data_ptr(), hcs, p.data_ptr(), _s(x.device)),
               "ryolo_conv_head_decode_store")


def bn_finalize(part, C_, count, gamma, beta, eps=1e-5, momentum=0.1, running_mean=None, running_var=None, out=None):
    dev = part.device
    if out is None:
        out = [torch.empty(C_, dtype=torch.float32, device=dev) for _ in range(4)]
    _lib.check(_lib.lib().ryolo_bn_finalize(part.data_ptr(), part.shape[0], part.shape[2], C_, int(count), eps, momentum,
                                            gamma.data_ptr(), beta.data_ptr(), out[0].data_ptr(), out[1].data_ptr(),
                                            out[2].data_ptr(), out[3].data_ptr(),
                                            running_mean.data_ptr() if running_mean is not None else None,
                                            running_var.data_ptr() if running_var is not None else None, _s(dev)),
               "ryolo_bn_finalize")
    return out


def bn_act_fwd(z, scale, shift, act, slope, y, residual=None):
    n, h, w, c = z.shape
    _lib.check(_lib.lib().ryolo_bn_act_fwd(z.data_ptr(), z.stride(2), scale.data_ptr(), shift.data_ptr(), act,
                                           slope.data_ptr() if slope is not None else None,
                                           residual.data_ptr() if residual is not None else None,
                                           residual.stride(2) if residual is not None else 0, y.data_ptr(), y.stride(2),
                                           n * h * w, c, _s(z.device)), "ryolo_bn_act_fwd")
    return y


def bn_act_bwd(z, dy, stats, act, slope, dz, dgamma, dbeta, dslope, ws):
    n, h, w, c = z.shape
    mean, invstd, scale, shift = stats if stats is not None else (None, None, None, None)
    p = lambda t: t.data_ptr() if t is not None else None
    _lib.check(_lib.lib().ryolo_bn_act_bwd(z.data_ptr(), z.stride(2), dy.data_ptr(), dy.stride(2), p(scale), p(shift), p(mean),
                                           p(invstd), act, p(slope), p(dz), dz.stride(2) if dz is not None else 0,
                                           n * h * w, c, p(dgamma), p(dbeta), p(dslope), ws.data_ptr(), ws.numel(),
                                           _s(z.device)), "ryolo_bn_act_bwd")


def bn_bwd_ws_bytes(npix, c):
    return _lib.lib().ryolo_bn_act_bwd_workspace_bytes(npix, c)


_tap_tables = {}


def dgrad_tap_table(ksize, stride, device):
    key = (ksize, stride, device.index)
    t = _tap_tables.get(key)
    if t is None:
        host = (C.c_int * 72)()
        _lib.check(_lib.lib().ryolo_conv_dgrad_tap_table(ksize, stride, host), "ryolo_conv_dgrad_tap_table")
        t = torch.tensor(list(host), dtype=torch.int32, device=device)
        _tap_tables[key] = t
    return t


def pack_weights_dgrad(weight, stride, out=None):
    cout, cin, k, _ = weight.shape
    L = _lib.lib()
    nbytes = L.ryolo_conv_packed_dgrad_bytes(cout, cin, k, stride)
    if out is None:
        out = torch.empty(nbytes, dtype=torch.uint8, device=weight.device)
    w = weight.contiguous()
    table = dgrad_tap_table(k, stride, weight.device)
    _lib.check(L.ryolo_conv_pack_weights_dgrad(w.data_ptr(), cout, cin, k, stride, out.data_ptr(), table.data_ptr(),
                                               _s(weight.device)), "ryolo_conv_pack_weights_dgrad")
    return out


def conv_dgrad(d, dz, packed_dgrad, ones, zeros, dx, accumulate):
    _lib.check(_lib.lib().ryolo_conv2d_dgrad(C.byref(d), dz.data_ptr(), dz.stride(2), packed_dgrad.data_ptr(), ones.data_ptr(),
                                             zeros.data_ptr(), dx.data_ptr(), 1 if accumulate else 0, _s(dz.device)),
               "ryolo_conv2d_dgrad")


def dgrad_bnreduce_rows(d):
    return _lib.lib().ryolo_conv2d_dgrad_bnreduce_rows(C.byref(d))


def conv_dgrad_bnreduce(d, dz, packed_dgrad, ones, zeros, dx, accumulate, z, stats, slope, part):
    mean, invstd, scale, shift = stats
    _lib.check(_lib.lib().ryolo_conv2d_dgrad_bnreduce(C.byref(d), dz.data_ptr(), dz.stride(2), packed_dgrad.data_ptr(), ones.data_ptr(),
                                                      zeros.data_ptr(), dx.data_ptr(), 1 if accumulate else 0, z.data_ptr(), z.stride(2),
                                                      scale.data_ptr(), shift.data_ptr(), mean.data_ptr(), invstd.data_ptr(),
                                                      slope.data_ptr(), part.data_ptr(), _s(dz.device)), "ryolo_conv2d_dgrad_bnreduce")


def bn_act_bwd_reduced(z, dy, stats, act, slope, dz, dgamma, dbeta, dslope, part, ws):
    n, h, w, c = z.shape
    mean, invstd, scale, shift = stats
    p = lambda t: t.data_ptr() if t is not None else None
    _lib.check(_lib.lib().ryolo_bn_act_bwd_reduced(z.data_ptr(), z.stride(2), dy.data_ptr(), dy.stride(2), scale.data_ptr(), shift.data_ptr(),
                                                   mean.data_ptr(), invstd.data_ptr(), act, p(slope), dz.data_ptr(), dz.stride(2), n * h * w, c,
                                                   p(dgamma), p(dbeta), p(dslope), part.data_ptr(), part.shape[0], ws.data_ptr(), ws.numel(),
                                                   _s(z.device)), "ryolo_bn_act_bwd_reduced")


def wgrad_ws_bytes(d):
    return _lib.lib().ryolo_conv_wgrad_workspace_bytes(C.byref(d))


def conv_wgrad(d, x, dz, cin_real, grad, accumulate, ws):
    L = _lib.lib()
    args = (C.byref(d), x.data_ptr(), dz.data_ptr(), dz.stride(2), cin_real, grad.data_ptr(), 1 if accumulate else 0, ws.data_ptr(),
            ws.numel(), _s(x.device))
    if isinstance(L, _lib._CallTracer):
        _lib.check(L.ryolo_conv2d_wgrad_partials(*args), "ryolo_conv2d_wgrad_partials")
        _lib.check(L.ryolo_conv2d_wgrad_reduce(*args), "ryolo_conv2d_wgrad_reduce")
        return
    _lib.check(L.ryolo_conv2d_wgrad(*args), "ryolo_conv2d_wgrad")


def conv_wgrad_partials(d, x, dz, cin_real, grad, accumulate, ws):
    _lib.check(_lib.lib().ryolo_conv2d_wgrad_partials(C.byref(d), x.data_ptr(), dz.data_ptr(), dz.stride(2), cin_real, grad.data_ptr(),
                                                      1 if accumulate else 0, ws.data_ptr(), ws.numel(), _s(x.device)),
               "ryolo_conv2d_wgrad_partials")


def _dil(dil):
    dh, dw = (dil, dil) if isinstance(dil, int) else dil
    return int(dh), int(dw)


def dilated_desc(n, h, w, cin, cout, in_cs=None, out_cs=None):
    return ConvDesc(n, h, w, cin, cout, 3, 1, 1, in_cs or cin, out_cs or cout, 0, 0, 0.0, 1, 0)


def conv_dilated_dgrad_supported(d, dil):
    return bool(_lib.lib().ryolo_conv2d_dilated_dgrad_supported(C.byref(d), *_dil(dil)))


def conv_dilated_wgrad_supported(d, dil):
    return bool(_lib.lib().ryolo_conv2d_dilated_wgrad_supported(C.byref(d), *_dil(dil)))


def conv_dilated_wgrad_ws_bytes(d, dil):
    return _lib.lib().ryolo_conv2d_dilated_wgrad_workspace_bytes(C.byref(d), *_dil(dil))


def conv_dilated_dgrad(d, dil, dz, packed_dgrad, ones, zeros, dx):
    _check_nhwc(dz, "dz")
    _check_nhwc(dx, "dx")
    dh, dw = _dil(dil)
    with torch.cuda.device(dz.device):
        rc = _lib.lib().ryolo_conv2d_dilated_dgrad(C.byref(d), dh, dw, dz.data_ptr(), dz.stride(2), packed_dgrad.data_ptr(), ones.data_ptr(),
                                                   zeros.data_ptr(), dx.data_ptr(), _s(dz.device))
    _lib.check(rc, "ryolo_conv2d_dilated_dgrad")


def conv_dilated_wgrad(d, dil, x, dz, grad, accumulate, ws):
    _check_nhwc(x, "x")
    _check_nhwc(dz, "dz")
    dh, dw = _dil(dil)
    with torch.cuda.device(x.device):
        rc = _lib.lib().ryolo_conv2d_dilated_wgrad(C.byref(d), dh, dw, x.data_ptr(), dz.data_ptr(), dz.stride(2), grad.data_ptr(),
                                                   1 if accumulate else 0, ws.data_ptr(), ws.numel() * ws.element_size(), _s(x.device))
    _lib.check(rc, "ryolo_conv2d_dilated_wgrad")


class SharedConvPacks(object):

    def __init__(self):
        self._fwd, self._dgrad, self._vec = {}, {}, {}

    @staticmethod
    def _get(table, weight, pack):
        ent = table.get(weight.data_ptr())
        if ent is None or ent[0] != weight._version:
            ent = (weight._version, pack(weight))
            table[weight.data_ptr()] = ent
        return ent[1]

    def forward_image(self, weight):
        return self._get(self._fwd, weight, lambda w: pack_weights(w.detach()))

    def dgrad_image(self, weight):
        return self._get(self._dgrad, weight, lambda w: pack_weights_dgrad(w.detach(), 1))

    def vectors(self, c, device):
        key = (cpad(c), device.index)
        v = self._vec.get(key)
        if v is None:
            v = (torch.ones(key[0], dtype=torch.float32, device=device), torch.zeros(key[0], dtype=torch.float32, device=device))
            self._vec[key] = v
        return v


class SharedDilatedConv(torch.autograd.Function):

    @staticmethod
    def forward(ctx, x, weight, dil, packs=None):
        packs = packs if packs is not None else SharedConvPacks()
        cout, cin = weight.shape[0], weight.shape[1]
        xb = hip_ops.nchw_f32_to_nhwc_bf16(x)
        ones, zeros = packs.vectors(cout, x.device)
        yb = hip_ops.conv2d_dilated(xb, packs.forward_image(weight), ones, zeros, cout, dil)
        ctx.save_for_backward(xb, weight)
        ctx.dil, ctx.packs = _dil(dil), packs
        return hip_ops.nhwc_bf16_to_nchw_f32(yb)

    @staticmethod
    def backward(ctx, dy):
        xb, weight = ctx.saved_tensors
        n, h, w, cin = xb.shape
        cout = weight.shape[0]
        d = dilated_desc(n, h, w, cin, cout)
        dyb = hip_ops.nchw_f32_to_nhwc_bf16(dy.float())
        dx = dw = None
        if ctx.needs_input_grad[0]:
            ones, zeros = ctx.packs.vectors(cin, dy.device)
            dxb = torch.empty((n, h, w, cin), dtype=torch.bfloat16, device=dy.device)
            conv_dilated_dgrad(d, ctx.dil, dyb, ctx.packs.dgrad_image(weight), ones, zeros, dxb)
            dx = hip_ops.nhwc_bf16_to_nchw_f32(dxb)
        if ctx.needs_input_grad[1]:
            dw = torch.empty(weight.shape, dtype=torch.float32, device=dy.device)
            ws = torch.empty(conv_dilated_wgrad_ws_bytes(d, ctx.dil), dtype=torch.uint8, device=dy.device)
            conv_dilated_wgrad(d, ctx.dil, xb, dyb, dw, False, ws)
        return dx, dw, None, None


def se_bwd_ws_bytes(n, h, w, c, hidden):
    return _lib.lib().ryolo_se_bwd_workspace_bytes(int(n), int(h), int(w), int(c), int(hidden))


def se_bwd_nhwc(x, dy, w1, w2, dx=None, dw1=None, dw2=None, dx_accumulate=False, accumulate_w=False, gate_out=None, workspace=None):
    x_cs = _check_nhwc(x, "x")
    dy_cs = _check_nhwc(dy, "dy")
    n, h, w, c = x.shape
    assert tuple(dy.shape) == (n, h, w, c), (tuple(dy.shape), (n, h, w, c))
    hidden = w1.shape[0]
    for t, shape, name in ((w1, (hidden, c), "w1"), (w2, (c, hidden), "w2"), (dw1, (hidden, c), "dw1"), (dw2, (c, hidden), "dw2"),
                           (gate_out, (n, c), "gate_out")):
        if t is not None and not (t.is_cuda and t.dtype == torch.float32 and t.is_contiguous() and tuple(t.shape) == shape):
            raise RuntimeError("%s must be a contiguous fp32 GPU tensor of shape %s" % (name, shape))
    dx_cs = 0
    if dx is not None:
        dx_cs = _check_nhwc(dx, "dx")
        assert tuple(dx.shape) == (n, h, w, c), (tuple(dx.shape), (n, h, w, c))
    if workspace is None:
        nbytes = se_bwd_ws_bytes(n, h, w, c, hidden)
        if nbytes == 0:
            raise RuntimeError("se backward: unsupported shape N %d, H %d, W %d, C %d, hidden %d (C a multiple of 8 from 16 to 2048, "
                               "hidden from 1 to 128)" % (n, h, w, c, hidden))
        workspace = torch.empty(nbytes, dtype=torch.uint8, device=x.device)

    def ptr(t):
        return t.data_ptr() if t is not None else None
    with torch.cuda.device(x.device):
        rc = _lib.lib().ryolo_se_bwd_nhwc(x.data_ptr(), x_cs, dy.data_ptr(), dy_cs, w1.data_ptr(), w2.data_ptr(), hidden, ptr(dx), dx_cs,
                                          1 if dx_accumulate else 0, ptr(dw1), ptr(dw2), 1 if accumulate_w else 0, n, h, w, c,
                                          ptr(gate_out), workspace.data_ptr(), workspace.numel() * workspace.element_size(), _s(x.device))
    _lib.check(rc, "ryolo_se_bwd_nhwc")
    return dx


def se_supported(n, h, w, c, hidden):
    return _lib.lib().ryolo_se_workspace_bytes(int(n), int(h), int(w), int(c)) > 0 and se_bwd_ws_bytes(n, h, w, c, hidden) > 0


class SqueezeExcite(torch.autograd.Function):

    @staticmethod
    def forward(ctx, x, w1, w2):
        if not (x.is_cuda and w1.is_cuda and w2.is_cuda):
            raise RuntimeError("SqueezeExcite runs on the HIP kernels: x, w1 and w2 must be GPU tensors")
        if x.shape[1] % 8:
            raise RuntimeError("SqueezeExcite: %d channels (the kernels need a multiple of 8)" % x.shape[1])
        xb = hip_ops.nchw_f32_to_nhwc_bf16(x.float())
        w1c, w2c = w1.detach().float().contiguous(), w2.detach().float().contiguous()
# ... 148 lines not shown
```

### rotate-yolov3_amd/model/plan.py

```python
import ctypes as C
from collections import namedtuple

from .. import _lib
from .._lib import ACT_LINEAR, ConvDesc

View = namedtuple('View', 'buf off C H W cs')
EvalPlan = namedtuple('EvalPlan', 'shapes buffers x views ops')
CONV_TYPES = ('convolutional', 'd-convolutional')
TrainPlan = namedtuple('TrainPlan', 'shapes buffers x act grd forward blocks backward')


class Refused(RuntimeError):
    """the configuration is refused at plan time (as opposed to a bug in the planner)"""


def _abs(i, l):
    return l if l > 0 else i + l


def _sources(i, d):
    return [_abs(i, int(v)) for v in d['layers'].split(',')]


def shared_attrs(d):
# ... 204 lines not shown
            desc = (N, xin.H, xin.W, xin.C, cv['cout'], cv['k'], cv['s'], cv['pad'], xin.cs, out.cs, res.cs if res is not None else 0,
                    cv['act'], cv['slope'], ups, 0)
            if src is not None and res is None and ups == 1 and i not in home:
                shared_seen.setdefault(key, i)
            ops.append(dict(kind='conv', layer=i, xin=xin, out=out, res=res, res_layer=conv_res.get(i), ups=ups, desc=desc, src=src))
        elif t == 'shortcut':
            views[i] = view_for(i)
            ops.append(dict(kind='add', layer=i, a=views[i - 1], b=views[_abs(i, int(d['from']))], out=views[i]))
        elif t == 'upsample':
            views[i] = view_for(i)
            ops.append(dict(kind='upsample', layer=i, xin=views[i - 1], out=views[i], stride=int(d['stride'])))
        elif t == 'maxpool':
            views[i] = view_for(i)
            ops.append(dict(kind='maxpool', layer=i, xin=views[i - 1], out=views[i], size=int(d['size']), stride=int(d['stride'])))
        elif t == 'se':
            c = shp[i][0]
            if c % 8 or c < 16 or c > 2048:
                raise Refused("se %d: %d channels (the HIP path serves multiples of 8 from 16 to 2048)" % (i, c))
            views[i] = view_for(i)
            ops.append(dict(kind='se', layer=i, xin=views[i - 1], out=views[i], C=c))
        elif t == 'route':
            if i in alias:
                views[i] = views[alias[i]]
            for src, off in copies.get(i, ()):
                ops.append(dict(kind='copy', layer=i, xin=views[src], out=_slice(views[i], off, shp[src][0])))
        elif t == 'yolo':
            if pending_head is not None:
                ops.append(dict(pending_head, layer=i))
                pending_head = None
            else:
                views[i] = views[i - 1]
                ops.append(dict(kind='decode', layer=i, xin=views[i]))
        elif t == 'reorg3d':
            views[i] = views[i - 1]
    return EvalPlan(shp, buffers, x, views, ops)


def plan_train(defs, convs, N, H, W, conv0_recompute=True, conv0_one_pass=True, cin=3, yolos=None, head_decode=True):
    n = len(defs)
    if any(d['type'] == 'd-convolutional' or 'weight_from' in d for d in defs):
        raise Refused("training path: weight_from / d-convolutional layers have no HIP training kernels (use model.backend = 'torch')")
    shp = _shapes(defs, convs, cin, H, W)
    for i, d in enumerate(defs):
        if d['type'] == 'upsample' and int(d['stride']) != 2:
            raise Refused("training path: only x2 upsampling")
        if d['type'] == 'se':
            raise Refused("training path: se layers have no HIP training kernels (use model.backend = 'torch')")
        if d['type'] == 'maxpool':
            raise Refused("training path: maxpool graphs (yolov3-tiny) cannot train in the reference either "
                          "(model/loss.py:248 hard-codes three heads)")
    readers = _readers(defs)
    fused_into, conv_res = {}, {}
    for i, d in enumerate(defs):
        if d['type'] == 'shortcut' and i > 0 and defs[i - 1]['type'] == 'convolutional' and readers[i - 1] == [i] \
                and _abs(i, int(d['from'])) != i - 1 and convs[i - 1]['bn']:
            fused_into[i] = i - 1
            conv_res[i - 1] = _abs(i, int(d['from']))

    buffers = []
    x = _new(buffers, 8, H, W)

    def new_pair(c, h, w):
        return _new(buffers, c, h, w), _new(buffers, c, h, w)

    act, grd = [None] * n, [None] * n
    alias, concat = _routes(defs, shp)
    home = {}
    children = {}
    for i, srcs in concat.items():
        act[i], grd[i] = new_pair(*shp[i])
        for src, off in srcs:
            if src in home or defs[src]['type'] not in ('convolutional', 'shortcut', 'upsample') or shp[src][0] % 8 or off % 8:
                raise Refused("training path: route %d needs a copy (unsupported graph)" % i)
            home[src] = (_slice(act[i], off, shp[src][0]), _slice(grd[i], off, shp[src][0]))
            children.setdefault(grd[i], []).append(home[src][1])

    def pair_for(i):
        return home[i] if i in home else new_pair(*shp[i])

    forward, blocks = [], []
    for i, d in enumerate(defs):
        t = d['type']
        if i in fused_into:
            act[i], grd[i] = act[fused_into[i]], grd[fused_into[i]]
            continue
        if t == 'convolutional':
            cv = convs[i]
            if cv.get('refuse'):
                raise Refused(cv['refuse'])
            xin, xin_g = (x, None) if i == 0 else (act[i - 1], grd[i - 1])
            final = i + 1 if i in conv_res else i
            y, dy = pair_for(final)
            res_alias = False
            if i in conv_res and final not in home:
                rg = grd[conv_res[i]]
                if rg is not None and rg[2:5] == dy[2:5] and rg.cs == rg.C:
                    dy, res_alias = rg, True
            act[i], grd[i] = y, dy
            c, h, w = shp[i]
            desc = (N, xin.H, xin.W, xin.C, c, cv['k'], cv['s'], cv['pad'], xin.cs, c, 0, 0, 0.0, 1, 0)
            recompute = bool(i == 0 and cv['bn'] and i not in conv_res and conv0_recompute
                             and _query('ryolo_conv0_recompute_supported', desc))
            head_fused = None
            if (head_decode and yolos is not None and i + 1 < n and defs[i + 1]['type'] == 'yolo' and readers[i] == [i + 1] and i not in home
                    and i not in conv_res and not cv['bn'] and cv['k'] == 1 and cv['s'] == 1 and c % 8 == 0):
                na, no = yolos[i + 1]
                ht = (N, xin.H, xin.W, xin.C, c, 1, 1, 0, xin.cs, c, 0, ACT_LINEAR, 0.0, 1, 0)
                if _query('ryolo_conv_head_decode_supported', ht, int(na), int(no)):
                    head_fused = dict(desc=ht, na=int(na), no=int(no))
            blk = dict(layer=i, desc=desc, xin=xin, xin_g=xin_g, y=y, dy=dy, res=act[conv_res[i]] if i in conv_res else None,
                       res_g=grd[conv_res[i]] if i in conv_res else None, res_alias=res_alias, bn=cv['bn'], act=cv['act'], shape=shp[i],
                       recompute=recompute, one_pass=bool(recompute and xin_g is None and conv0_one_pass), head_fused=head_fused)
            blocks.append(blk)
            forward.append(('conv', i, blk))
        elif t == 'shortcut':
            a, b = i - 1, _abs(i, int(d['from']))
            act[i], grd[i] = pair_for(i)
            forward.append(('add', i, (act[a], act[b], act[i], grd[a], grd[b], grd[i])))
        elif t == 'upsample':
            act[i], grd[i] = pair_for(i)
            forward.append(('up', i, (act[i - 1], act[i], grd[i - 1], grd[i])))
        elif t == 'route':
            if i in alias:
                act[i], grd[i] = act[alias[i]], grd[alias[i]]
        elif t == 'yolo':
            act[i], grd[i] = act[i - 1], grd[i - 1]
            forward.append(('yolo', i, (act[i], grd[i])))

    init = set()

    def first(g):
        if g in init:
            return False
        init.add(g)
        init.update(children.get(g, ()))
        return True

    heads = [i for kind, i, _ in forward if kind == 'yolo']
    backward = []
    for kind, i, pl in reversed(forward):
        if kind == 'yolo':
            first(pl[1])
            backward.append((kind, i, heads.index(i)))
        elif kind == 'conv':
            res_first = first(pl['res_g']) if (pl['res_g'] is not None and not pl['res_alias']) else None
            backward.append((kind, i, (res_first, first(pl['xin_g']) if pl['xin_g'] is not None else None)))
        elif kind == 'add':
            backward.append((kind, i, (first(pl[3]), first(pl[4]))))
        elif kind == 'up':
            backward.append((kind, i, first(pl[2])))
    return TrainPlan(shp, buffers, x, act, grd, forward, blocks, backward)


def reduce_fusion_pairs(tp):
    by = {b['layer']: b for b in tp.blocks}
    pairs = []
    for (k0, i0, _), (k1, i1, _) in zip(tp.backward[:-1], tp.backward[1:]):
        if k0 != 'conv' or k1 != 'conv':
            continue
        x, y = by[i0], by[i1]
        g, dy = x['xin_g'], y['dy']
        if g is None or not y['bn'] or y['recompute'] or g != dy or dy[2:5] != y['shape'] or g.cs != g.C:
            continue
        rows = _query('ryolo_conv2d_dgrad_bnreduce_rows', x['desc'])
        if rows > 0:
            pairs.append((x, y, rows))
    return pairs
```

### rotate-yolov3_amd/model/train_engine.py

```python
import ctypes as C
import os

import torch
import torch.nn as nn

from .. import _lib
from . import hip_ops as ops
from . import hip_train_ops as tr
from . import plan
from .engine import HipEngine
from .nhwc_batch import NHWC8Batch


class _Fn(torch.autograd.Function):
    @staticmethod
    def forward(ctx, engine, x, anchor):
        ctx.engine = engine
        outs = engine.forward(x)
        return tuple(outs)

    @staticmethod
    def backward(ctx, *grads):
        ctx.engine.backward(grads)
        return None, None, None


class TrainEngine(object):
    def __init__(self, model, x_shape, device, use_graph=True):
        _lib.lib()
        self.model = model
        self.no_graph_env = os.environ.get('RYOLO_NO_GRAPH', '0') == '1'
        self.use_graph = use_graph and not self.no_graph_env
        self.graph_fallback = None
        self.reduce_fallback = None
        self.force_eager = False
        self.g_fwd = self.g_bwd = None
        self._segs = None
        self._red_planned = False
        self.nbt = None
        self.packs = None
        self.steps = 0
        self.device = device
        self.bs, cin, self.H, self.W = [int(v) for v in x_shape]
        defs, mods = model.module_defs, model.module_list
        self.defs, self.mods = defs, mods

        convs = {i: self._conv_attrs(mods[i]) for i, d in enumerate(defs) if d['type'] == 'convolutional'}
        tp = self._tplan = plan.plan_train(defs, convs, self.bs, self.H, self.W,
                                           conv0_recompute=os.environ.get('RYOLO_CONV0_RECOMPUTE', '1') != '0',
                                           conv0_one_pass=os.environ.get('RYOLO_CONV0_ONE_PASS', '1') != '0', cin=cin,
                                           yolos={i: (mods[i].na, model.nc + 6) for i, d in enumerate(defs) if d['type'] == 'yolo'},
                                           head_decode=os.environ.get('RYOLO_HEAD_DECODE', '1') != '0')
        self.shp = tp.shapes

        def new_buf(c, h, w):
            return torch.empty((self.bs, h, w, c), dtype=torch.bfloat16, device=device)

        bufs = [new_buf(*b) for b in tp.buffers]
        tensors = {None: None}

        def tv(v):
            if v not in tensors:
                tensors[v] = bufs[v.buf][..., v.off:v.off + v.C]
            return tensors[v]

        self.x_nhwc = tv(tp.x)
        cmax = max(ops.cpad(max(c.out_channels, c.in_channels)) for c in (HipEngine._conv_of(mods[i]) for i in convs))
        self.ones = torch.ones(cmax, device=device)
        self.zeros = torch.zeros(cmax, device=device)
        self.stat_part = torch.zeros((tr.stat_rows(), 2, cmax), dtype=torch.float64, device=device)
        self.blocks = []
        self.p, self.p_src = [], []
        self.static_grad = {}
        self.direct = False
        self.static_flat = None
        wgrad_ws, bn_ws = 0, 0
        self.plan = fwd = []
        for kind, i, rec in tp.forward:
            if kind == 'conv':
                conv = HipEngine._conv_of(mods[i])
                bn = HipEngine._bn_of(mods[i])
                actmod = [s_ for s_ in mods[i] if isinstance(s_, (nn.PReLU, nn.LeakyReLU))]
                xin, y, dy = tv(rec['xin']), tv(rec['y']), tv(rec['dy'])
                c, h, w = rec['shape']
                desc = ops.ConvDesc(*rec['desc'])
                if bn is not None:
                    z = None if rec['recompute'] else new_buf(c, h, w)
                    dz = None if rec['one_pass'] else new_buf(c, h, w)
                else:
                    z, dz = y, dy
                blk = dict(i=i, conv=conv, bn=bn, act=actmod[-1] if actmod else None, mish=any(type(s_).__name__ == 'Mish' for s_ in mods[i]),
                           xin=xin, xin_g=tv(rec['xin_g']), z=z, dz=dz, y=y, dy=dy, desc=desc, res=tv(rec['res']), res_g=tv(rec['res_g']),
                           res_alias=rec['res_alias'], cin_k=xin.shape[-1], k=desc.ksize, s=desc.stride, pad=desc.pad,
                           npix=self.bs * h * w, C=c, recompute=rec['recompute'])
                if rec.get('head_fused') and not actmod and not blk['mish']:
                    blk['head_fused'] = rec['head_fused']
                wgrad_ws = max(wgrad_ws, tr.wgrad_ws_bytes(desc))
                bn_ws = max(bn_ws, tr.bn_bwd_ws_bytes(blk['npix'], c))
                self.blocks.append(blk)
                fwd.append(('conv', i, blk))
            elif kind in ('add', 'up'):
                fwd.append((kind, i, tuple(tv(v) for v in rec)))
            elif kind == 'yolo':
                m = mods[i]
                c, h, w = tp.shapes[i]
                anchors = m.anchors.to(device=device, dtype=torch.float32).contiguous()
                pbuf = torch.empty((self.bs, m.na, h, w, model.nc + 6), dtype=torch.float32, device=device)
                io = None
                if model.nc + 6 > 96 or m.na * (model.nc + 6) > 1024:
                    io = torch.empty((self.bs, m.na * h * w, model.nc + 6), dtype=torch.float32, device=device)
                self.p.append(pbuf)
                hb = self.blocks[-1] if self.blocks and self.blocks[-1]['i'] == i - 1 and self.blocks[-1].get('head_fused') else None
                if hb is not None and (hb['head_fused']['na'], hb['head_fused']['no']) != (m.na, model.nc + 6):
                    hb.pop('head_fused')
                    hb = None
                fwd.append(('yolo', i, (tv(rec[0]), tv(rec[1]), m, anchors, pbuf, io, h, w, hb)))
        self.head_pairs = [(pl[0], pl[1]) for kind, _, pl in fwd if kind == 'yolo']
        self.fused_nhwc = False
        self.head_g_ready = False
        self.head_bias_fold = os.environ.get('RYOLO_HEAD_BIAS_FOLD', '1') != '0'
        self.head_gscale = torch.ones(1, device=device)
        self.head_bias_ready = None
        self._bias_parts = self._bias_ws = None
        self._fold_now = (False,) * len(self.head_pairs)
        self._g_bwd_fold = None
        readers = plan._readers(defs)
        for k, (hd, _) in enumerate(self.head_pairs):
            for b in self.blocks:
                i = b['i']
                if (b['y'] is hd and b['bn'] is None and b['conv'].bias is not None and i + 1 < len(defs) and defs[i + 1]['type'] == 'yolo'
                        and readers[i] == [i + 1]):
                    b['head_k'] = k
        self.batch_reduce = os.environ.get('RYOLO_WGRAD_BATCH_REDUCE', '1') != '0'
        self._wr_batches = {}
        self._ws_w_bytes = max(wgrad_ws, 256)
        self._ws_w = None
        self.ws_b = torch.empty(max(bn_ws, 256), dtype=torch.uint8, device=device)

        self.bplan = [(kind, i, pl, flags) for (kind, i, pl), (_, _, flags) in zip(reversed(fwd), tp.backward)]

    @staticmethod
    def _conv_attrs(m):
        conv = HipEngine._conv_of(m)
        other = [type(s_).__name__ for s_ in m if not isinstance(s_, (nn.Conv2d, nn.BatchNorm2d, nn.PReLU, nn.LeakyReLU))
                 and type(s_).__name__ != 'Mish']
        return dict(cout=conv.out_channels, k=conv.kernel_size[0], s=conv.stride[0], pad=conv.padding[0],
                    bn=HipEngine._bn_of(m) is not None, act=None,
                    refuse="activation %s has no HIP training kernels (use model.backend = 'torch')" % other[0] if other else None)

    def _build_grad_sink(self):
        plist = [q for q in self.model.parameters()]
        views = getattr(self.model, '_dp_grad_views', None)
        ok = views is not None and os.environ.get("RYOLO_DIRECT_GRADS", "1") != "0"
        if ok:
            for q in plist:
                v = views.get(q)
                if (v is None or v.dtype != torch.float32 or not v.is_contiguous() or v.device != q.device or v.shape != q.shape
                        or q.grad is None or q.grad.data_ptr() != v.data_ptr()):
                    ok = False
                    break
        self.direct = bool(ok)
        if ok:
            self.static_flat = None
            self.static_grad = {q: views[q] for q in plist}
        else:
            self.static_flat = torch.zeros(sum(q.numel() for q in plist), dtype=torch.float32, device=self.device)
            off = 0
            for q in plist:
                self.static_grad[q] = self.static_flat[off:off + q.numel()].view_as(q)
                off += q.numel()

    def _reset_grad_sink(self):
        self.static_grad, self.static_flat, self.direct = {}, None, False
        self._segs, self.g_bwd = None, None
        self._wr_batches = {}

    def _check_direct_sink(self):
        if not self.direct:
            return
        rebound = 0
        for q, v in self.static_grad.items():
            g = q.grad
            if g is None:
                v.zero_()
            elif g.data_ptr() != v.data_ptr():
                v.copy_(g)
            else:
                continue
            q.grad = v
            rebound += 1
        if rebound and not getattr(self, '_warned_rebind', False):
            self._warned_rebind = True
            import warnings
            warnings.warn("TrainEngine: %d param.grad tensors had been replaced (zero_grad(set_to_none=True)?) while a GradientAllReducer "
                          "owns them; they were re-bound to the reducer's buckets.  Use reducer.zero_grad() to clear gradients." % rebound)

    def _grad_of(self, p):
        g = self.static_grad.get(p)
        if g is None:
            self._build_grad_sink()
            g = self.static_grad[p]
        return g

    def _flush_param_grads(self, params=None):
        add_to, add_from = [], []
        plist = list(self.static_grad.keys()) if params is None else params
        if not self.direct:
            views = getattr(self.model, '_dp_grad_views', None) or {}
            for p in plist:
                g = self.static_grad[p]
                v = views.get(p)
                if v is not None and (p.grad is None or p.grad.data_ptr() != v.data_ptr()):
                    if p.grad is None:
                        v.zero_()
                    else:
                        v.copy_(p.grad)
                    p.grad = v
                if p.grad is None:
                    p.grad = g.clone()
                else:
                    add_to.append(p.grad)
                    add_from.append(g)
            if add_to:
                torch._foreach_add_(add_to, add_from)
        for p in plist:
            hooks = getattr(p, '_post_accumulate_grad_hooks', None)
            if hooks:
                for hk in list(hooks.values()):
                    hk(p)

    def head_bias_parts(self, arc=0):
        if not self.head_bias_fold or arc != 0:
            return None
        if self._bias_parts is None:
            by_head = {b['head_k']: b for b in self.blocks if 'head_k' in b}
            parts, ws = [], 256
            for k, q in enumerate(self.p):
                rows = tr.yolo_loss_bias_rows(q, arc) if k in by_head else 0
                parts.append(torch.empty((rows, ops.cpad(by_head[k]['C'])), dtype=torch.float32, device=self.device) if rows > 0 else None)
                if rows > 0:
                    ws = max(ws, tr.head_bias_ws_bytes(by_head[k]['npix'], by_head[k]['C']))
            self._bias_parts = parts
            self._bias_ws = torch.empty(ws, dtype=torch.uint8, device=self.device)
        return self._bias_parts if any(q is not None for q in self._bias_parts) else None

    @staticmethod
    def _has_wgrad(b):
        return not (b['bn'] is not None and b['recompute'] and b['xin_g'] is None and b['dz'] is None)

    @property
    def ws_w(self):
        if self._ws_w is None:
            self._ws_w = torch.empty(self._ws_w_bytes, dtype=torch.uint8, device=self.device)
        return self._ws_w

    def _ensure_reduce_batches(self, segs):
        if not self.batch_reduce:
            return
        try:
            self._build_reduce_batches(segs)
        except torch.cuda.OutOfMemoryError as e:
            for kind, i, pl, flags in self.bplan:
                if kind == 'conv':
                    pl.pop('ws_w', None)
            self._wr_batches = {}
            torch.cuda.empty_cache()
            self.batch_reduce = False
            self.reduce_fallback = "per-layer split-K reduces on one shared workspace (the per-layer workspaces did not fit: %s)" % str(e)[:120]
            self.g_bwd = None

    def _build_reduce_batches(self, segs):
        for lo, hi, _ in segs:
            if (lo, hi) in self._wr_batches:
                continue
            blks = [pl for kind, i, pl, flags in self.bplan[lo:hi] if kind == 'conv' and self._has_wgrad(pl)]
            wb = None
            if blks:
                wb = tr.WgradReduceBatch(self.device)
                for b in blks:
                    if 'ws_w' not in b:
                        b['ws_w'] = torch.empty(max(tr.wgrad_ws_bytes(b['desc']), 256), dtype=torch.uint8, device=self.device)
                    wb.add(b['desc'], b['conv'].in_channels, b['ws_w'], self._grad_of(b['conv'].weight), True)
                wb.finalize()
            self._wr_batches[(lo, hi)] = wb

    def _segments(self):
        if self._segs is not None:
            return self._segs
        pos = {}
        for k, (kind, i, pl, flags) in enumerate(self.bplan):
            if kind == 'conv':
                for q in list(pl['conv'].parameters()) + (list(pl['bn'].parameters()) if pl['bn'] is not None else []) + (
                        list(pl['act'].parameters()) if isinstance(pl['act'], nn.Module) else []):
                    pos[q] = k
        cuts = set()
        for bucket in getattr(self.model, '_dp_buckets', None) or []:
            ks = [pos[q] for q in bucket if q in pos]
            if ks:
                cuts.add(max(ks) + 1)
        cuts.add(len(self.bplan))
        segs, lo = [], 0
        for hi in sorted(cuts):
            if hi > lo:
                segs.append((lo, hi, [q for q, k in pos.items() if lo <= k < hi]))
                lo = hi
        self._segs = segs
        return segs


    def forward(self, x):
        dev = self.device
        nhwc = isinstance(x, NHWC8Batch)
        if not nhwc:
            x = x.float().contiguous()
        with torch.cuda.device(dev), torch.no_grad():
            if nhwc:
                x.copy_into(self.x_nhwc)
            else:
                n, c, h, w = x.shape
                _lib.check(_lib.lib().ryolo_nchw_f32_to_nhwc_bf16(x.data_ptr(), n, c, h, w, 8, self.x_nhwc.data_ptr(), _lib.stream_ptr(dev)),
                           "ryolo_nchw_f32_to_nhwc_bf16")
            if not self.use_graph or self.steps < 2 or self.force_eager:
                self._forward_launch()
            else:
                if self.g_fwd is None:
                    self.g_fwd = self._capture(self._forward_launch)
                if self.g_fwd is not None:
                    self.g_fwd.replay()
        return [p for p in self.p]

    def _capture(self, launch):
        dev = self.device
        torch.cuda.synchronize(dev)
        g = torch.cuda.CUDAGraph()
        try:
            with torch.cuda.graph(g, capture_error_mode="thread_local"):
                launch()
            return g
        except Exception as e:
            self.use_graph = False
            self.graph_fallback = "%s: %s" % (type(e).__name__, str(e).splitlines()[0][:200] if str(e) else "")
            import warnings
            warnings.warn("TrainEngine: hipGraph capture failed (%s); continuing with eager launches" % self.graph_fallback)
            try:
                torch.cuda.synchronize(dev)
            except Exception:
                pass
            launch()
            return None

    def _forward_launch(self):
        dev = self.device
        L = _lib.lib()
        if self.nbt is None:
            self.nbt = [pl['bn'].num_batches_tracked for kind, i, pl in self.plan if kind == 'conv' and pl['bn'] is not None]
        if self.nbt:
            torch._foreach_add_(self.nbt, 1)
        if self.packs is None:
            self.packs = tr.WeightPackBatch(dev)
            for kind, i, pl in self.plan:
                if kind != 'conv':
                    continue
                w = pl['conv'].weight
                if w.dtype != torch.float32 or not w.is_contiguous():
                    raise RuntimeError("TrainEngine expects contiguous fp32 conv weights")
                cout, cin, k, _ = w.shape
                pl['packed'] = torch.empty(L.ryolo_conv_packed_weight_bytes(cout, pl['cin_k'], k), dtype=torch.uint8, device=dev)
                pl['packed_d'] = torch.empty(L.ryolo_conv_packed_dgrad_bytes(cout, cin, k, pl['s']), dtype=torch.uint8,
                                             device=dev) if pl['xin_g'] is not None else None
                self.packs.add(w.detach(), pl['s'], pl['cin_k'], pl['packed'], pl['packed_d'])
            self.packs.finalize()
        self.packs.run()
        for kind, i, pl in self.plan:
            if kind == 'conv':
                b = pl
                conv, bn = b['conv'], b['bn']
                if bn is not None:
                    part = tr.conv_fwd_stats(b['desc'], b['xin'], b['packed'], self.ones, self.zeros, b['z'], part=self.stat_part,
                                             clear=False)
                    b['stats'] = tr.bn_finalize(part, b['C'], b['npix'], bn.weight.detach(), bn.bias.detach(), eps=bn.eps,
                                                momentum=bn.momentum, running_mean=bn.running_mean,
                                                running_var=bn.running_var, out=b.get('stats'))
                    slope = b['act'].weight.detach() if isinstance(b['act'], nn.PReLU) else None
                    if isinstance(b['act'], nn.LeakyReLU):
                        if 'leaky' not in b:
                            b['leaky'] = torch.full((1,), b['act'].negative_slope, device=dev)
                        slope = b['leaky']
                    b['slope'] = slope
                    b['actcode'] = 2 if b['mish'] else (1 if slope is not None else 0)
                    if b['recompute']:
                        tr.conv0_bn_act_fwd(b['desc'], b['xin'], b['packed'], b['stats'][2], b['stats'][3], b['actcode'], slope, b['y'])
                    else:
                        tr.bn_act_fwd(b['z'], b['stats'][2], b['stats'][3], b['actcode'], slope, b['y'], residual=b['res'])
                else:
                    if conv.bias is not None:
                        if 'bias_pad' not in b:
                            b['bias_pad'] = torch.zeros(ops.cpad(b['C']), device=dev)
                        b['bias_pad'][:b['C']].copy_(conv.bias.detach())
                        bias = b['bias_pad']
                    else:
                        bias = self.zeros
                    b['bias_now'] = bias
                    if not b.get('head_fused'):
                        tr.conv_fwd_plain(b['desc'], b['xin'], b['packed'], self.ones, bias, b['z'])
                    b['stats'] = None
            elif kind == 'add':
                a, bb, y = pl[0], pl[1], pl[2]
                nn_, hh, ww, cc = y.shape
                _lib.check(L.ryolo_add_nhwc(a.data_ptr(), a.stride(2), bb.data_ptr(), bb.stride(2), y.data_ptr(), y.stride(2),
                                            nn_ * hh * ww, cc, _lib.stream_ptr(dev)), "ryolo_add_nhwc")
            elif kind == 'up':
                xin, y = pl[0], pl[1]
                nn_, hh, ww, cc = xin.shape
                _lib.check(L.ryolo_upsample_nhwc(xin.data_ptr(), xin.stride(2), y.data_ptr(), y.stride(2), nn_, hh, ww, cc, 2,
                                                 _lib.stream_ptr(dev)), "ryolo_upsample_nhwc")
            elif kind == 'yolo':
                head, _, m, anchors, pbuf, io, hh, ww, hb = pl
                stride = float(max(self.H, self.W)) / float(max(hh, ww))
                if hb is not None:
                    tr.conv_head_decode_store(hb['head_fused'], hb['xin'], hb['packed'], self.ones, hb['bias_now'], head, pbuf)
                else:
                    _lib.check(L.ryolo_yolo_decode(head.data_ptr(), head.stride(2), self.bs, hh, ww, m.na, self.model.nc + 6,
                                                   anchors.data_ptr(), stride, 1.0, 0, io.data_ptr() if io is not None else None, m.na * hh * ww, 0,
                                                   pbuf.data_ptr(), _lib.stream_ptr(dev)), "ryolo_yolo_decode")
                if (m.nx, m.ny) != (ww, hh):
                    from .models import create_grids
                    create_grids(m, (self.H, self.W), (ww, hh), dev)

    def backward(self, pgrads):
        dev = self.device
        with torch.cuda.device(dev), torch.no_grad():
            if not hasattr(self, "static_pg"):
                self.static_pg = [torch.zeros_like(p) for p in self.p]
            ready, bias_ready = self.head_g_ready, self.head_bias_ready
            self.head_g_ready, self.head_bias_ready = False, None
            fold = [False] * len(self.static_pg)
            for k, (buf, g) in enumerate(zip(self.static_pg, pgrads)):
                if g is not None and ready and g.data_ptr() == buf.data_ptr():
                    fold[k] = bias_ready is not None and bias_ready[k] is not None
                    continue
                if g is None:
                    buf.zero_()
                elif g.data_ptr() != buf.data_ptr():
                    buf.copy_(g)
                tr.pgrad_to_nhwc(buf, self.head_pairs[k][1])
                if self.fused_nhwc and g is not None:
                    buf.zero_()
            self._check_direct_sink()
            self._grad_of(next(self.model.parameters()))
            segs = self._segments()
            if self.batch_reduce:
                self._ensure_reduce_batches(segs)
            if self.g_bwd is None:
                self.g_bwd = [None] * len(segs)
                self._g_bwd_fold = None
            self._fold_now = tuple(fold)
            eager = not self.use_graph or self.steps < 2 or self.force_eager
            if not eager:
                if self._g_bwd_fold is None:
                    self._g_bwd_fold = self._fold_now
                eager = self._g_bwd_fold != self._fold_now
            for k, (lo, hi, params) in enumerate(segs):
                if eager:
                    self._backward_launch(lo, hi)
                else:
                    if self.g_bwd[k] is None:
                        self.g_bwd[k] = self._capture(lambda lo=lo, hi=hi: self._backward_launch(lo, hi))
                    if self.g_bwd[k] is not None:
                        self.g_bwd[k].replay()
                self._flush_param_grads(params)
            self.steps += 1

    def _backward_launch(self, lo=0, hi=None):
        dev = self.device
        L = _lib.lib()
        pgrads = self.static_pg
        if lo == 0 and self.static_flat is not None:
            self.static_flat.zero_()
        if not self._red_planned:
            self._plan_reduce_fusion()
        hook = getattr(self, 'backward_hook', None)

        def entry(kind, i, pl, flags):
            if kind == 'yolo':
                pass
            elif kind == 'conv':
                b = pl
                conv, bn = b['conv'], b['bn']
                res_first, in_first = flags
                dy = b['dy']
                if b['res_g'] is not None and not b['res_alias']:
                    self._passthrough(dy, b['res_g'], res_first)
                if bn is not None:
                    dsl = self._grad_of(b['act'].weight) if isinstance(b['act'], nn.PReLU) else None
                    if b['recompute'] and b['xin_g'] is None and b['dz'] is None:
                        if 'ws0f' not in b:
                            b['ws0f'] = tr.conv0_bn_bwd_wgrad_ws(dev)
                        tr.conv0_bn_bwd_wgrad(b['desc'], b['xin'], b['packed'], dy, b['stats'], b['actcode'], b['slope'],
                                              self._grad_of(bn.weight), self._grad_of(bn.bias), dsl, self._grad_of(conv.weight),
                                              conv.in_channels, True, b['ws0f'])
                        return
                    elif b['recompute']:
                        if 'ws0' not in b:
                            b['ws0'] = tr.conv0_bn_bwd_ws(dev)
                        tr.conv0_bn_bwd(b['desc'], b['xin'], b['packed'], dy, b['stats'], b['actcode'], b['slope'], b['dz'],
                                        self._grad_of(bn.weight), self._grad_of(bn.bias), dsl, b['ws0'])
                    elif b.get('red_part') is not None:
                        tr.bn_act_bwd_reduced(b['z'], dy, b['stats'], 1, b['slope'], b['dz'],
                                              self._grad_of(bn.weight), self._grad_of(bn.bias), dsl, b['red_part'], self.ws_b)
                    else:
                        tr.bn_act_bwd(b['z'], dy, b['stats'], b['actcode'], b['slope'], b['dz'],
                                      self._grad_of(bn.weight), self._grad_of(bn.bias), dsl, self.ws_b)
                elif conv.bias is not None:
                    hk = b.get('head_k')
                    if hk is not None and self._fold_now[hk]:
                        tr.head_bias_finalize(self._bias_parts[hk], b['npix'], b['C'], self.head_gscale, self._grad_of(conv.bias), self._bias_ws)
                    else:
                        tr.bn_act_bwd(b['z'], dy, None, 0, None, None, None, self._grad_of(conv.bias), None, self.ws_b)
                if self.batch_reduce:
                    tr.conv_wgrad_partials(b['desc'], b['xin'], b['dz'], conv.in_channels, self._grad_of(conv.weight), True, b['ws_w'])
                else:
                    tr.conv_wgrad(b['desc'], b['xin'], b['dz'], conv.in_channels, self._grad_of(conv.weight), True, self.ws_w)
                if b['xin_g'] is not None:
                    y = b.get('red_for')
                    if y is not None:
                        tr.conv_dgrad_bnreduce(b['desc'], b['dz'], b['packed_d'], self.ones, self.zeros, b['xin_g'], not in_first,
                                               y['z'], y['stats'], y['slope'], y['red_part'])
                    else:
                        tr.conv_dgrad(b['desc'], b['dz'], b['packed_d'], self.ones, self.zeros, b['xin_g'], not in_first)
            elif kind == 'add':
                dyv = pl[5]
                self._passthrough(dyv, pl[3], flags[0])
                self._passthrough(dyv, pl[4], flags[1])
            elif kind == 'up':
                tr.upsample2x_bwd(pl[3], pl[2], not flags)

        for kind, i, pl, flags in self.bplan[lo:hi]:
            if hook is not None:
                hook('pre', kind, i, pl, flags)
            entry(kind, i, pl, flags)
            if hook is not None:
                hook('post', kind, i, pl, flags)
        if self.batch_reduce:
            wb = self._wr_batches[(lo, len(self.bplan) if hi is None else hi)]
            if wb is not None:
                wb.run()

    def _plan_reduce_fusion(self):
        self._red_planned = True
        if os.environ.get("RYOLO_BN_REDUCE_FUSION", "1") == "0":
            return
        blk = {b['i']: b for b in self.blocks}
        pairs = []
        for xr, yr, rows in plan.reduce_fusion_pairs(self._tplan):
            x, y = blk[xr['layer']], blk[yr['layer']]
            if y.get('actcode') == 1 and y.get('slope') is not None and y.get('stats') is not None:
                pairs.append((x, y, rows, x['xin_g'].shape[3]))
        if not pairs:
            return
        part = torch.empty(max(rows * 3 * c for _, _, rows, c in pairs), dtype=torch.float32, device=self.device)
        for x, y, rows, c in pairs:
            x['red_for'] = y
            y['red_part'] = part[:rows * 3 * c].view(rows, 3, c)

    def _passthrough(self, src, dst, is_first):
        L = _lib.lib()
        n, h, w, c = dst.shape
        if is_first:
            _lib.check(L.ryolo_upsample_nhwc(src.data_ptr(), src.stride(2), dst.data_ptr(), dst.stride(2), n, h, w, c, 1,
                                             _lib.stream_ptr(self.device)), "ryolo_upsample_nhwc")
        else:
            _lib.check(L.ryolo_add_nhwc(src.data_ptr(), src.stride(2), dst.data_ptr(), dst.stride(2), dst.data_ptr(),
                                        dst.stride(2), n * h * w, c, _lib.stream_ptr(self.device)), "ryolo_add_nhwc")

    def __call__(self, x):
        anchor = next(self.model.parameters())
        return list(_Fn.apply(self, x, anchor))
```

Baseline: 1372 images/s.

## Fuse 1x1 bottleneck backward: BN-act bwd, wgrad, dgrad and residual in one kernel

Adds a fused backward kernel for 1x1 conv blocks that computes the BN/leaky activation backward, writes dz into LDS, accumulates the weight gradient with MFMA, computes the data gradient from register-held weights, adds the residual, and optionally accumulates the next layer's BN reduction partials. It targets repeated HBM round-trips of dz and dx across separate BN-bwd, wgrad, dgrad and add kernels in Darknet-53 residual blocks. The kernel is enabled by default via RYOLO_BNECK_BWD, relies on a complex hand-scheduled pipeline with waitcnt constants, and only skips writing dz to global memory when no hook is installed.

```diff
diff --git a/__graft_entry__.py b/__graft_entry__.py
--- a/__graft_entry__.py
+++ b/__graft_entry__.py
@@ -26,6 +26,7 @@
     "wgrad.hip": [],
     "wgrad_dil.hip": [],
     "train.hip": [],
+    "bneck_bwd.hip": [],
     "optim.hip": ["-ffp-contract=off", "-fhip-fp32-correctly-rounded-divide-sqrt"],
     "loss.hip": ["-ffp-contract=off"],
     "augment.hip": ["-ffp-contract=off", "-fhip-fp32-correctly-rounded-divide-sqrt"],
diff --git a/include/ryolo.h b/include/ryolo.h
--- a/include/ryolo.h
+++ b/include/ryolo.h
@@ -201,6 +201,17 @@
 int ryolo_conv2d_wgrad_reduce(const ryolo_conv_desc *forward_desc, const void *x, const void *dz, int dz_cstride, int Cin_real,
                               float *grad_oihw, int accumulate, void *workspace, size_t workspace_bytes, void *stream);
 
+int ryolo_conv1x1_bwd_fused_rows(const ryolo_conv_desc *forward_desc);
+size_t ryolo_conv1x1_bwd_fused_workspace_bytes(const ryolo_conv_desc *forward_desc, int own_reduce);
+int ryolo_conv1x1_bwd_fused(const ryolo_conv_desc *forward_desc, const void *z, int z_cstride, const void *dy, int dy_cstride,
+                            const float *scale, const float *shift, const float *mean, const float *invstd, const float *slope,
+                            void *dz_out, int dz_cstride, float *dgamma, float *dbeta, float *dslope, const float *part, int rows,
+                            void *bn_workspace, size_t bn_workspace_bytes, const void *x, void *wgrad_workspace,
+                            size_t wgrad_workspace_bytes, const void *packed_dgrad, const float *ones, const float *zeros, void *dx,
+                            int accumulate, const void *prev_z, int prev_z_cstride,
+                            const float *prev_scale, const float *prev_shift, const float *prev_mean, const float *prev_invstd,
+                            const float *prev_slope, float *part_out, void *stream);
+
 typedef struct ryolo_wgrad_reduce_job {
     const float *part;
     float *g;
diff --git a/rotate-yolov3_amd/csrc/bn_bwd_elem.h b/rotate-yolov3_amd/csrc/bn_bwd_elem.h
--- /dev/null
+++ b/rotate-yolov3_amd/csrc/bn_bwd_elem.h
@@ -0,0 +1,36 @@
+#pragma once
+#include "conv_common.h"
+
+namespace ryolo_detail {
+
+struct BnBwdConst {
+    float sc, sh, kb, kd;
+};
+__device__ __forceinline__ BnBwdConst bn_bwd_const(float scale, float shift, float mean, float invstd, float s1, float s2, float inv_count) {
+    BnBwdConst c;
+    c.sc = scale;
+    c.sh = shift;
+    const float k = scale * invstd * s2 * inv_count;
+    c.kb = -k;
+    c.kd = __builtin_fmaf(k, mean, -(scale * s1 * inv_count));
+    return c;
+}
+
+template <int ACT>
+__device__ __forceinline__ __bf16 bn_bwd_elem(const BnBwdConst &c, __bf16 zb, __bf16 gb, float slope) {
+    const float zf = (float)zb;
+    float g = (float)gb;
+    const float u = __builtin_fmaf(zf, c.sc, c.sh);
+    if (ACT == 1 && u <= 0.f) g *= slope;
+    return (__bf16)__builtin_fmaf(c.sc, g, __builtin_fmaf(c.kb, zf, c.kd));
+}
+
+struct BnBwdSums {
+    const float *s1, *s2, *s3;
+    float *dslope;
+};
+int bn_act_bwd_sums(const void *z, int z_cstride, const void *dy, int dy_cstride, const float *scale, const float *shift, const float *mean,
+                    const float *invstd, int act, const float *slope, long long npix, int C, float *dgamma, float *dbeta, float *dslope,
+                    void *workspace, size_t workspace_bytes, const float *pre_part, int pre_rows, hipStream_t stream, BnBwdSums *out);
+
+}
diff --git a/rotate-yolov3_amd/csrc/bneck_bwd.hip b/rotate-yolov3_amd/csrc/bneck_bwd.hip
--- /dev/null
+++ b/rotate-yolov3_amd/csrc/bneck_bwd.hip
@@ -0,0 +1,426 @@
+#include <type_traits>
+
+#include "bn_bwd_elem.h"
+#include "conv_common.h"
+#include "wgrad_frag.h"
+
+using namespace ryolo_detail;
+
+namespace {
+
+template <int N> using ic_ = std::integral_constant<int, N>;
+
+__device__ __forceinline__ void issue_order_fence() { asm volatile("" ::: "memory"); }
+
+struct BneckParams {
+    const __bf16 *z, *dy, *x, *wd, *pz;
+    __bf16 *dx, *dzo;
+    float *part, *part_out, *dslope;
+    const float *scale, *shift, *mean, *invstd, *s1, *s2, *s3, *slope, *ones, *zeros;
+    const float *p_scale, *p_shift, *p_mean, *p_invstd, *p_slope;
+    int z_cs, dy_cs, x_cs, dzo_cs, pz_cs;
+    int Cin, Kpad, Cout_pad, ci_tiles, chunk, M, wd_kpad;
+    int accumulate;
+    float inv_count;
+    unsigned z_bytes, dy_bytes, x_bytes, dzo_bytes, pz_bytes, wd_bytes;
+};
+
+constexpr int BQ_PX = 32, BQ_NST = 3, BQ_C = 128;
+constexpr int BQ_ROW = BQ_C * 2, BQ_TILE = BQ_PX * BQ_ROW, BQ_STAGE = 2 * BQ_TILE;
+constexpr int BQ_CST = BQ_NST * BQ_STAGE;
+constexpr int BQ_BNC = BQ_CST + 4 * BQ_C * 4;
+constexpr int BQ_LDS = BQ_BNC + 3 * BQ_C * 4;
+constexpr int OOB = (int)0x80000000;
+
+template <bool RED, bool NT>
+__global__ void __launch_bounds__(256, 1) bneck_bwd_kernel(const BneckParams p) {
+    extern __shared__ __attribute__((aligned(16))) char smem[];
+#if defined(__HIP_DEVICE_COMPILE__)
+    const int tid = threadIdx.x, lane = tid & 63;
+    const int wave = __builtin_amdgcn_readfirstlane(tid >> 6);
+    const int fr = lane & 15, g = lane >> 4;
+    int b = blockIdx.x;
+    {
+        const int per = gridDim.x >> 3;
+        if (b < per * 8) b = (b & 7) * per + (b >> 3);
+    }
+    const int ci_t = b % p.ci_tiles, split = b / p.ci_tiles;
+    const int ci0 = ci_t * BQ_C;
+    const int pix_lo = split * p.chunk, pix_hi = min(p.M, pix_lo + p.chunk);
+    const int npx = pix_hi - pix_lo;
+    const int nsteps = (npx + BQ_PX - 1) / BQ_PX;
+
+    if constexpr (RED) {
+        for (int t = tid; t < 3 * p.Cin; t += 256) p.part_out[(size_t)blockIdx.x * 3 * p.Cin + t] = 0.f;
+        __syncthreads();
+    }
+    if (p.dslope && blockIdx.x == 0 && tid < 64) {
+        float v = 0.f;
+        for (int c = tid; c < BQ_C; c += 64) v += p.s3[c];
+#pragma unroll
+        for (int o = 32; o > 0; o >>= 1) v += __shfl_xor(v, o);
+        if (tid == 0) p.dslope[0] += v;
+    }
+
+    const int cz = tid & 15, rz = tid >> 4;
+    float *cst = (float *)(smem + BQ_CST), *bnc = (float *)(smem + BQ_BNC);
+    if (tid < BQ_C) {
+        const BnBwdConst c1 = bn_bwd_const(p.scale[tid], p.shift[tid], p.mean[tid], p.invstd[tid], p.s1[tid], p.s2[tid], p.inv_count);
+        cst[tid] = c1.sc; cst[BQ_C + tid] = c1.sh; cst[2 * BQ_C + tid] = c1.kb; cst[3 * BQ_C + tid] = c1.kd;
+        if constexpr (RED) {
+            bnc[tid] = p.p_scale[ci0 + tid]; bnc[BQ_C + tid] = p.p_shift[ci0 + tid]; bnc[2 * BQ_C + tid] = p.p_mean[ci0 + tid];
+        }
+    }
+    __syncthreads();
+    const float slope = p.slope[0];
+    const int dz_lds = rz * BQ_ROW + ((cz ^ (wg_swz<BQ_C>(rz) << 1)) << 4);
+    const bool dzo_on = p.dzo != nullptr && ci_t == 0;
+
+    int xf_pix[2], xf_col[2];
+#pragma unroll
+    for (int j = 0; j < 2; j++) {
+        const int tp = (wave * 2 + j) * 4 + (lane >> 4);
+        xf_pix[j] = tp;
+        xf_col[j] = (ci0 + (((lane & 15) ^ (wg_swz<BQ_C>(tp) << 1)) * 8)) * 2;
+    }
+    const i32x4 rs_x = make_rsrc_words(p.x, p.x_bytes);
+    const unsigned lds0 = (unsigned)(size_t)(__attribute__((address_space(3))) char *)smem;
+
+    const __amdgpu_buffer_rsrc_t zrs = __builtin_amdgcn_make_buffer_rsrc((void *)p.z, 0, p.z_bytes, 0x00020000);
+    const __amdgpu_buffer_rsrc_t grs = __builtin_amdgcn_make_buffer_rsrc((void *)p.dy, 0, p.dy_bytes, 0x00020000);
+    const __amdgpu_buffer_rsrc_t ors = __builtin_amdgcn_make_buffer_rsrc((void *)(p.dzo ? p.dzo : p.dx), 0, p.dzo ? p.dzo_bytes : 0u, 0x00020000);
+    const __amdgpu_buffer_rsrc_t yrs = __builtin_amdgcn_make_buffer_rsrc((void *)p.dx, 0, p.x_bytes, 0x00020000);
+    const __amdgpu_buffer_rsrc_t rrs = __builtin_amdgcn_make_buffer_rsrc((void *)p.dx, 0, p.accumulate ? p.x_bytes : 0u, 0x00020000);
+    const __amdgpu_buffer_rsrc_t prs = __builtin_amdgcn_make_buffer_rsrc((void *)(RED ? (const void *)p.pz : (const void *)p.dx), 0, RED ? p.pz_bytes : 0u, 0x00020000);
+    (void)prs;
+    const __amdgpu_buffer_rsrc_t wrs = __builtin_amdgcn_make_buffer_rsrc((void *)p.wd, 0, p.wd_bytes, 0x00020000);
+
+    const int wr = wave >> 1, wc = wave & 1;
+    const int trow = g * 8 + (fr >> 2);
+    const int tsw = wg_swz<BQ_C>(trow);
+    int offa[4], offb[4];
+#pragma unroll
+    for (int f = 0; f < 4; f++) {
+        offa[f] = trow * BQ_ROW + (fr & 3) * 8 + (((wr * 4) + f) ^ tsw) * 32;
+        offb[f] = BQ_TILE + trow * BQ_ROW + (fr & 3) * 8 + (((wc * 4) + f) ^ tsw) * 32;
+    }
+    f32x4 acc[4][4];
+#pragma unroll
+    for (int a = 0; a < 4; a++)
+#pragma unroll
+        for (int c = 0; c < 4; c++) acc[a][c] = f32x4{0.f, 0.f, 0.f, 0.f};
+
+    bf16x8 wreg[2][2][2];
+#pragma unroll
+    for (int kt = 0; kt < 2; kt++)
+#pragma unroll
+        for (int ks = 0; ks < 2; ks++)
+#pragma unroll
+            for (int cf = 0; cf < 2; cf++)
+                wreg[kt][ks][cf] = __builtin_bit_cast(
+                    bf16x8, __builtin_amdgcn_raw_buffer_load_b128(wrs, ((ci0 + wave * 32 + cf * 16 + fr) * p.wd_kpad + g * 8) * 2, (kt * 64 + ks * 32) * 2, 0));
+    int d_rd[2][2];
+#pragma unroll
+    for (int kt = 0; kt < 2; kt++)
+#pragma unroll
+        for (int ks = 0; ks < 2; ks++) d_rd[kt][ks] = fr * BQ_ROW + (((kt * 8 + ks * 4 + g) ^ (wg_swz<BQ_C>(fr) << 1)) << 4);
+    f32x4 sc[2], sh[2];
+#pragma unroll
+    for (int cf = 0; cf < 2; cf++) {
+        const int ch = ci0 + wave * 32 + cf * 16 + g * 4;
+        sc[cf] = *(const f32x4 *)(p.ones + ch);
+        sh[cf] = *(const f32x4 *)(p.zeros + ch);
+    }
+    const int och = ci0 + wave * 32 + (g & 1) * 16 + (g >> 1) * 8;
+    float bs1[8], bs2[8], bs3[8];
+    float bn_slope = 0.f;
+    if constexpr (RED) bn_slope = p.p_slope[0];
+#pragma unroll
+    for (int e = 0; e < 8; e++) bs1[e] = bs2[e] = bs3[e] = 0.f;
+    const float *bnl = bnc + (och - ci0);
+    const bool do_add = RED || p.accumulate;
+
+    u32x4 zr[2][2], gr[2][2], rv[2][2], pv[2][2];
+
+    auto fill_x = [&](int k) __attribute__((always_inline)) {
+        const int slot = k % BQ_NST;
+#pragma unroll
+        for (int j = 0; j < 2; j++) {
+            const int r = k * BQ_PX + xf_pix[j];
+            const unsigned off = (unsigned)(pix_lo + r) * (unsigned)(p.x_cs * 2) + (unsigned)xf_col[j];
+            buffer_load_lds16_raw(rs_x, lds0 + slot * BQ_STAGE + BQ_TILE + (wave * 2 + j) * 1024, r < npx ? (int)off : OOB);
+        }
+    };
+    auto load_zg = [&](int k, auto PARc) __attribute__((always_inline)) {
+        constexpr int PAR = decltype(PARc)::value;
+#pragma unroll
+        for (int j = 0; j < 2; j++) {
+            const int r = k * BQ_PX + rz + 16 * j;
+            const bool ok = r < npx;
+            const unsigned pg = (unsigned)(pix_lo + r);
+            zr[PAR][j] = __builtin_amdgcn_raw_buffer_load_b128(zrs, ok ? (int)(pg * (unsigned)(p.z_cs * 2) + cz * 16) : OOB, 0, 0);
+            gr[PAR][j] = __builtin_amdgcn_raw_buffer_load_b128(grs, ok ? (int)(pg * (unsigned)(p.dy_cs * 2) + cz * 16) : OOB, 0, 0);
+        }
+    };
+    auto load_res = [&](int k, auto PARc) __attribute__((always_inline)) {
+        constexpr int PAR = decltype(PARc)::value;
+#pragma unroll
+        for (int s = 0; s < 2; s++) {
+            const int r = k * BQ_PX + s * 16 + fr;
+            const bool ok = r < npx;
+            const unsigned pg = (unsigned)(pix_lo + r);
+            rv[PAR][s] = __builtin_amdgcn_raw_buffer_load_b128(rrs, ok ? (int)(pg * (unsigned)(p.x_cs * 2) + och * 2) : OOB, 0, 0);
+            if constexpr (RED) pv[PAR][s] = __builtin_amdgcn_raw_buffer_load_b128(prs, ok ? (int)(pg * (unsigned)(p.pz_cs * 2) + och * 2) : OOB, 0, 0);
+        }
+    };
+
+    auto step = [&](int k, auto PARc) __attribute__((always_inline)) {
+        constexpr int PAR = decltype(PARc)::value;
+        char *stage = smem + (k % BQ_NST) * BQ_STAGE;
+        BnBwdConst cc[8];
+#pragma unroll
+        for (int h = 0; h < 2; h++) {
+            const f32x4 a = *(const f32x4 *)(cst + cz * 8 + h * 4), bq = *(const f32x4 *)(cst + BQ_C + cz * 8 + h * 4);
+            const f32x4 c = *(const f32x4 *)(cst + 2 * BQ_C + cz * 8 + h * 4), d = *(const f32x4 *)(cst + 3 * BQ_C + cz * 8 + h * 4);
+#pragma unroll
+            for (int e = 0; e < 4; e++) cc[h * 4 + e] = BnBwdConst{a[e], bq[e], c[e], d[e]};
+        }
+#pragma unroll
+        for (int j = 0; j < 2; j++) {
+            const int r = k * BQ_PX + rz + 16 * j;
+            const bool ok = r < npx;
+            const bf16x8 zv = __builtin_bit_cast(bf16x8, zr[PAR][j]), gv = __builtin_bit_cast(bf16x8, gr[PAR][j]);
+            bf16x8 o;
+#pragma unroll
+            for (int e = 0; e < 8; e++) o[e] = bn_bwd_elem<1>(cc[e], zv[e], gv[e], slope);
+            u32x4 ou = __builtin_bit_cast(u32x4, o);
+            if (!ok) ou = u32x4{0u, 0u, 0u, 0u};
+            *(u32x4 *)(stage + dz_lds + j * 16 * BQ_ROW) = ou;
+            const unsigned pg = (unsigned)(pix_lo + r);
+            __builtin_amdgcn_raw_buffer_store_b128(ou, ors, ok && dzo_on ? (int)(pg * (unsigned)(p.dzo_cs * 2) + cz * 16) : OOB, 0, 0);
+        }
+        issue_order_fence();
+        asm volatile("s_waitcnt vmcnt(%0) lgkmcnt(0)" ::"n"(RED ? 16 : 14) : "memory");
+        __builtin_amdgcn_s_barrier();
+        issue_order_fence();
+        fill_x(k + 2);
+        load_zg(k + 2, ic_<PAR>{});
+        load_res(k + 1, ic_<1 - PAR>{});
+        issue_order_fence();
+        {
+            bf16x8 af[4], bfr[4];
+#pragma unroll
+            for (int f = 0; f < 4; f++) {
+                const s16x4 b0 = lds_read_tr16(stage + offb[f]);
+                const s16x4 b1 = lds_read_tr16(stage + offb[f] + 4 * BQ_ROW);
+                bfr[f] = __builtin_bit_cast(bf16x8, __builtin_shufflevector(b0, b1, 0, 1, 2, 3, 4, 5, 6, 7));
+            }
+#pragma unroll
+            for (int f = 0; f < 4; f++) {
+                const s16x4 a0 = lds_read_tr16(stage + offa[f]);
+                const s16x4 a1 = lds_read_tr16(stage + offa[f] + 4 * BQ_ROW);
+                af[f] = __builtin_bit_cast(bf16x8, __builtin_shufflevector(a0, a1, 0, 1, 2, 3, 4, 5, 6, 7));
+            }
+#pragma unroll
+            for (int a = 0; a < 4; a++)
+#pragma unroll
+                for (int c = 0; c < 4; c++) acc[a][c] = __builtin_amdgcn_mfma_f32_16x16x32_bf16(af[a], bfr[c], acc[a][c], 0, 0, 0);
+        }
+        f32x4 dacc[2][2];
+#pragma unroll
+        for (int cf = 0; cf < 2; cf++)
+#pragma unroll
+            for (int f = 0; f < 2; f++) dacc[cf][f] = f32x4{0.f, 0.f, 0.f, 0.f};
+#pragma unroll
+        for (int kt = 0; kt < 2; kt++)
+#pragma unroll
+            for (int ks = 0; ks < 2; ks++) {
+                bf16x8 xf[2];
+#pragma unroll
+                for (int f = 0; f < 2; f++) xf[f] = *(const bf16x8 *)(stage + d_rd[kt][ks] + f * 16 * BQ_ROW);
+#pragma unroll
+                for (int cf = 0; cf < 2; cf++)
+#pragma unroll
+                    for (int f = 0; f < 2; f++) dacc[cf][f] = __builtin_amdgcn_mfma_f32_16x16x32_bf16(wreg[kt][ks][cf], xf[f], dacc[cf][f], 0, 0, 0);
+            }
+        unsigned R[2][2][2];
+#pragma unroll
+        for (int cf = 0; cf < 2; cf++)
+#pragma unroll
+            for (int f = 0; f < 2; f++) {
+                bf16x4 o;
+#pragma unroll
+                for (int rr = 0; rr < 4; rr++) o[rr] = (__bf16)(dacc[cf][f][rr] * sc[cf][rr] + sh[cf][rr]);
+                const uint2 u2 = __builtin_bit_cast(uint2, o);
+                R[cf][f][0] = u2.x;
+                R[cf][f][1] = u2.y;
+            }
+        float bn_sc[8], bn_sh[8], bn_mu[8];
+        if constexpr (RED) {
+#pragma unroll
+            for (int h = 0; h < 2; h++) {
+                const f32x4 a = *(const f32x4 *)(bnl + h * 4), bq = *(const f32x4 *)(bnl + BQ_C + h * 4), c = *(const f32x4 *)(bnl + 2 * BQ_C + h * 4);
+#pragma unroll
+                for (int e = 0; e < 4; e++) { bn_sc[h * 4 + e] = a[e]; bn_sh[h * 4 + e] = bq[e]; bn_mu[h * 4 + e] = c[e]; }
+            }
+        }
+#pragma unroll
+        for (int s = 0; s < 2; s++) {
+            auto s0 = __builtin_amdgcn_permlane16_swap(R[0][s][0], R[1][s][0], false, false);
+            auto s1 = __builtin_amdgcn_permlane16_swap(R[0][s][1], R[1][s][1], false, false);
+            u32x4 out = u32x4{s0[0], s1[0], s0[1], s1[1]};
+            const int r = k * BQ_PX + s * 16 + fr;
+            const bool ok = r < npx;
+            if (do_add) {
+                bf16x8 a = __builtin_bit_cast(bf16x8, out);
+                const bf16x8 bb = __builtin_bit_cast(bf16x8, rv[PAR][s]);
+#pragma unroll
+                for (int e = 0; e < 8; e++) a[e] = (__bf16)((float)a[e] + (float)bb[e]);
+                out = __builtin_bit_cast(u32x4, a);
+            }
+            if constexpr (RED) {
+                const bf16x8 dv = __builtin_bit_cast(bf16x8, out), zq = __builtin_bit_cast(bf16x8, pv[PAR][s]);
+#pragma unroll
+                for (int e = 0; e < 8; e++) {
+                    const float zf = (float)zq[e], d = (float)dv[e];
+                    const float u = zf * bn_sc[e] + bn_sh[e];
+                    float gg = d;
+                    if (u <= 0.f) { gg = d * bn_slope; bs3[e] += d * u; }
+                    bs2[e] += gg * (zf - bn_mu[e]);
+                    bs1[e] += gg;
+                }
+            }
+            const int voff = ok ? (int)((unsigned)(pix_lo + r) * (unsigned)(p.x_cs * 2) + och * 2) : OOB;
+            __builtin_amdgcn_raw_buffer_store_b128(out, yrs, voff, 0, NT ? 2 : 0);
+        }
+        issue_order_fence();
+    };
+
+    issue_order_fence();
+    fill_x(0);
+    load_zg(0, ic_<0>{});
+    issue_order_fence();
+    fill_x(1);
+    load_zg(1, ic_<1>{});
+    load_res(0, ic_<0>{});
+    issue_order_fence();
+#pragma unroll
+    for (int j = 0; j < 2; j++) {
+        asm volatile("" : "+v"(zr[0][j]), "+v"(gr[0][j]), "+v"(zr[1][j]), "+v"(gr[1][j]));
+        asm volatile("" : "+v"(rv[0][j]));
+        if constexpr (RED) asm volatile("" : "+v"(pv[0][j]));
+    }
+
+    int k = 0;
+    for (; k + 1 < nsteps; k += 2) {
+        step(k, ic_<0>{});
+        step(k + 1, ic_<1>{});
+    }
+    if (k < nsteps) step(k, ic_<0>{});
+    asm volatile("s_waitcnt vmcnt(0)" ::: "memory");
+
+    float *outp = p.part + (size_t)split * p.Cout_pad * p.Kpad;
+#pragma unroll
+    for (int a = 0; a < 4; a++)
+#pragma unroll
+        for (int c = 0; c < 4; c++)
+#pragma unroll
+            for (int r = 0; r < 4; r++) {
+                const int co = wr * 64 + a * 16 + g * 4 + r;
+                const int ci = ci0 + wc * 64 + c * 16 + fr;
+                if (ci < p.Cin) outp[(size_t)co * p.Kpad + ci] = acc[a][c][r];
+            }
+
+    if constexpr (RED) {
+        float t1 = 0.f, t2 = 0.f, t3 = 0.f;
+#pragma unroll
+        for (int e = 0; e < 8; e++) {
+            const float a = row16_sum(bs1[e]), bsum = row16_sum(bs2[e]), d = row16_sum(bs3[e]);
+            if (fr == e) { t1 = a; t2 = bsum; t3 = d; }
+        }
+        const int ch = och + fr;
+        if (fr < 8 && ch < p.Cin) {
+            float *row = p.part_out + (size_t)blockIdx.x * 3 * p.Cin;
+            row[ch] = t1;
+            row[p.Cin + ch] = t2 * p.p_invstd[ch];
+            row[2 * p.Cin + ch] = t3;
+        }
+    }
+#endif
+}
+
+bool fused_served(const ryolo_conv_desc *d, int Cin_real, WgradWide128 *w) {
+    if (!d || conv_validate(d) != RYOLO_OK) return false;
+    if (d->ksize != 1 || d->stride != 1 || d->pad != 0 || d->Cout != BQ_C || d->Cin <= 0 || d->Cin % BQ_C || d->upsample > 1) return false;
+    if (d->act == RYOLO_ACT_MISH || (d->in_cstride & 7) || d->in_cstride < d->Cin) return false;
+    if ((long long)d->N * d->H * d->W > 0x7fffffffLL - 512) return false;
+    return wgrad_wide128_geometry(d, Cin_real, w);
+}
+
+}
+
+extern "C" {
+
+int ryolo_conv1x1_bwd_fused_rows(const ryolo_conv_desc *d) {
+    WgradWide128 w;
+    return fused_served(d, d ? d->Cin : 0, &w) ? (int)w.blocks : 0;
+}
+
+size_t ryolo_conv1x1_bwd_fused_workspace_bytes(const ryolo_conv_desc *d, int own_reduce) {
+    WgradWide128 w;
+    if (!fused_served(d, d ? d->Cin : 0, &w)) return 0;
+    return own_reduce ? ryolo_bn_act_bwd_workspace_bytes(w.M, BQ_C) : (size_t)(3 + 3 * 64) * BQ_C * 4;
+}
+
+int ryolo_conv1x1_bwd_fused(const ryolo_conv_desc *d, const void *z, int z_cstride, const void *dy, int dy_cstride, const float *scale,
+                            const float *shift, const float *mean, const float *invstd, const float *slope, void *dz_out,
+                            int dz_cstride, float *dgamma, float *dbeta, float *dslope, const float *part, int rows, void *bn_workspace,
+                            size_t bn_workspace_bytes, const void *x, void *wgrad_workspace,
+                            size_t wgrad_workspace_bytes, const void *packed_dgrad, const float *ones, const float *zeros, void *dx,
+                            int accumulate, const void *prev_z, int prev_z_cstride, const float *prev_scale, const float *prev_shift,
+                            const float *prev_mean, const float *prev_invstd, const float *prev_slope, float *part_out, void *stream_) {
+    const int act = RYOLO_ACT_LEAKY;
+    WgradWide128 w;
+    if (!fused_served(d, d ? d->Cin : 0, &w)) return RYOLO_EINVAL;
+    if (!z || !dy || !scale || !shift || !mean || !invstd || !slope || !bn_workspace) return RYOLO_EINVAL;
+    if (!x || !wgrad_workspace || wgrad_workspace_bytes < w.part_bytes) return RYOLO_EINVAL;
+    if (!packed_dgrad || !ones || !zeros || !dx) return RYOLO_EINVAL;
+    if ((z_cstride & 7) || z_cstride < BQ_C || (dy_cstride & 7) || dy_cstride < BQ_C) return RYOLO_EINVAL;
+    if (dz_out && ((dz_cstride & 7) || dz_cstride < BQ_C)) return RYOLO_EINVAL;
+    if (part && rows <= 0) return RYOLO_EINVAL;
+    if (prev_z && (!prev_scale || !prev_shift || !prev_mean || !prev_invstd || !prev_slope || !part_out || (prev_z_cstride & 7) ||
+                   prev_z_cstride < d->Cin || d->in_cstride != d->Cin))
+        return RYOLO_EINVAL;
+    BneckParams p{};
+    const int wrows = (d->Cin + 127) / 128 * 128;
+    p.wd_kpad = (d->Cout + BK - 1) / BK * BK;
+    if (!buffer_extent((unsigned long long)w.M, z_cstride, BQ_C, &p.z_bytes) || !buffer_extent((unsigned long long)w.M, dy_cstride, BQ_C, &p.dy_bytes) ||
+        !buffer_extent((unsigned long long)w.M, d->in_cstride, d->Cin, &p.x_bytes) || !buffer_extent(wrows, p.wd_kpad, p.wd_kpad + 128, &p.wd_bytes) ||
+        (dz_out && !buffer_extent((unsigned long long)w.M, dz_cstride, BQ_C, &p.dzo_bytes)) ||
+        (prev_z && !buffer_extent((unsigned long long)w.M, prev_z_cstride, d->Cin, &p.pz_bytes)))
+        return RYOLO_EINVAL;
+    if (bn_workspace_bytes < (part ? (size_t)3 * BQ_C * 4 : ryolo_bn_act_bwd_workspace_bytes(w.M, BQ_C))) return RYOLO_EINVAL;
+    hipStream_t stream = (hipStream_t)stream_;
+    BnBwdSums sm;
+    const int rc = bn_act_bwd_sums(z, z_cstride, dy, dy_cstride, scale, shift, mean, invstd, act, slope, w.M, BQ_C, dgamma, dbeta, dslope, bn_workspace,
+                                   bn_workspace_bytes, part, rows, stream, &sm);
+    if (rc != RYOLO_OK) return rc;
+    p.z = (const __bf16 *)z; p.dy = (const __bf16 *)dy; p.x = (const __bf16 *)x; p.wd = (const __bf16 *)packed_dgrad; p.pz = (const __bf16 *)prev_z;
+    p.dx = (__bf16 *)dx; p.dzo = (__bf16 *)dz_out;
+    p.part = (float *)wgrad_workspace; p.part_out = part_out; p.dslope = sm.dslope;
+    p.scale = scale; p.shift = shift; p.mean = mean; p.invstd = invstd; p.s1 = sm.s1; p.s2 = sm.s2; p.s3 = sm.s3; p.slope = slope;
+    p.ones = ones; p.zeros = zeros;
+    p.p_scale = prev_scale; p.p_shift = prev_shift; p.p_mean = prev_mean; p.p_invstd = prev_invstd; p.p_slope = prev_slope;
+    p.z_cs = z_cstride; p.dy_cs = dy_cstride; p.x_cs = d->in_cstride; p.dzo_cs = dz_cstride; p.pz_cs = prev_z_cstride;
+    p.Cin = d->Cin; p.Kpad = w.Kpad; p.Cout_pad = w.Cout_pad; p.ci_tiles = w.ci_tiles; p.chunk = w.chunk; p.M = w.M;
+    p.accumulate = accumulate ? 1 : 0;
+    p.inv_count = 1.0f / (float)w.M;
+    const dim3 grid(w.blocks), block(256);
+    const bool nt = (long long)w.M * d->Cin * 2 >= nt_out_min_bytes();
+    if (prev_z) return nt ? launch_kernel<bneck_bwd_kernel<true, true>>(grid, block, BQ_LDS, stream, p)
+                          : launch_kernel<bneck_bwd_kernel<true, false>>(grid, block, BQ_LDS, stream, p);
+    return nt ? launch_kernel<bneck_bwd_kernel<false, true>>(grid, block, BQ_LDS, stream, p)
+              : launch_kernel<bneck_bwd_kernel<false, false>>(grid, block, BQ_LDS, stream, p);
+}
+
+}
diff --git a/rotate-yolov3_amd/csrc/conv_common.h b/rotate-yolov3_amd/csrc/conv_common.h
--- a/rotate-yolov3_amd/csrc/conv_common.h
+++ b/rotate-yolov3_amd/csrc/conv_common.h
@@ -301,6 +301,13 @@
 int ryolo_mp_ablation_variant(int slot);
 #endif
 
+struct WgradWide128 {
+    int S, chunk, Kpad, Cout_pad, ci_tiles, M;
+    unsigned blocks;
+    size_t lds, part_bytes;
+};
+bool wgrad_wide128_geometry(const ryolo_conv_desc *d, int Cin_real, WgradWide128 *g);
+
 enum TuneKey { TUNE_CONV3X3 = 0, TUNE_CONV1X1, TUNE_RNMS_TILES, TUNE_MQ_KORDER, TUNE_BN_REDUCE_TILES, TUNE_STEM_DGRAD, TUNE_COUNT };
 const char *tune(TuneKey k);
 #ifdef RYOLO_MP_ABLATION
diff --git a/rotate-yolov3_amd/csrc/train.hip b/rotate-yolov3_amd/csrc/train.hip
--- a/rotate-yolov3_amd/csrc/train.hip
+++ b/rotate-yolov3_amd/csrc/train.hip
@@ -1,4 +1,5 @@
 #include "conv_common.h"
+#include "bn_bwd_elem.h"
 
 using namespace ryolo_detail;
 
@@ -313,25 +314,22 @@
         if (i >= total) return;
         const int c = (int)(i % cpr) * 8;
         const long long dp = stride / cpr;
-        float sc[8], sh[8], kb[8], kd[8];
-#pragma unroll
-        for (int e = 0; e < 8; e++) {
-            sc[e] = scale[c + e];
-            sh[e] = shift[c + e];
-            const float k = sc[e] * invstd[c + e] * s2[c + e] * inv_count;
-            kb[e] = -k;
-            kd[e] = k * mean[c + e] - sc[e] * s1[c + e] * inv_count;
-        }
+        BnBwdConst cc[8];
+#pragma unroll
+        for (int e = 0; e < 8; e++)
+            cc[e] = bn_bwd_const(scale[c + e], shift[c + e], mean[c + e], invstd[c + e], s1[c + e], s2[c + e], inv_count);
         auto one = [&](const bf16x8 &zv, const bf16x8 &gv) {
             bf16x8 o;
 #pragma unroll
             for (int e = 0; e < 8; e++) {
-                const float zf = (float)zv[e];
-                float g = (float)gv[e];
-                const float u = zf * sc[e] + sh[e];
-                if (ACT == 1 && u <= 0.f) g *= slope;
-                else if (ACT == 2) g *= mish_grad(u);
-                o[e] = (__bf16)(sc[e] * g + (kb[e] * zf + kd[e]));
+                if constexpr (ACT == 2) {
+                    const float zf = (float)zv[e];
+                    const float u = zf * cc[e].sc + cc[e].sh;
+                    const float g = (float)gv[e] * mish_grad(u);
+                    o[e] = (__bf16)(cc[e].sc * g + (cc[e].kb * zf + cc[e].kd));
+                } else {
+                    o[e] = bn_bwd_elem<ACT>(cc[e], zv[e], gv[e], slope);
+                }
             }
             return o;
         };
@@ -501,14 +499,15 @@
                            dslope, workspace, workspace_bytes, part, rows, stream_);
 }
 
-static int bn_act_bwd_impl(const void *z, int z_cstride, const void *dy, int dy_cstride, const float *scale, const float *shift,
-                           const float *mean, const float *invstd, int act, const float *slope, void *dz, int dz_cstride,
-                           long long npix, int C, float *dgamma, float *dbeta, float *dslope, void *workspace,
-                           size_t workspace_bytes, const float *pre_part, int pre_rows, void *stream_) {
+}
+
+namespace ryolo_detail {
+
+int bn_act_bwd_sums(const void *z, int z_cstride, const void *dy, int dy_cstride, const float *scale, const float *shift, const float *mean,
+                    const float *invstd, int act, const float *slope, long long npix, int C, float *dgamma, float *dbeta, float *dslope,
+                    void *workspace, size_t workspace_bytes, const float *pre_part, int pre_rows, hipStream_t stream, BnBwdSums *out) {
     if (!z || !dy || npix <= 0 || C <= 0 || (C & 7) || (z_cstride & 7) || (dy_cstride & 7) || !workspace) return RYOLO_EINVAL;
     if (workspace_bytes < (pre_part ? (size_t)3 * C * 4 : ryolo_bn_act_bwd_workspace_bytes(npix, C))) return RYOLO_EINVAL;
-    if (scale && (!shift || !mean || !invstd || !dz || (dz_cstride & 7))) return RYOLO_EINVAL;
-    hipStream_t stream = (hipStream_t)stream_;
     int nslab = pre_part ? pre_rows : (int)((npix + bwd_slab(npix) - 1) / bwd_slab(npix));
     float *part = pre_part ? const_cast<float *>(pre_part) : (float *)workspace;
     float *s1 = pre_part ? (float *)workspace : part + (size_t)nslab * 3 * C, *s2 = s1 + C, *s3 = s2 + C;
@@ -523,7 +522,7 @@
     int CT = 32;
     while (CT > 1 && CT > C / 8) CT >>= 1;
     if (act < 0 || act > 2) return RYOLO_EINVAL;
-    const bool nt_red = nt_pass(1, npix, C), nt_app = nt_pass(2, npix, C);
+    const bool nt_red = nt_pass(1, npix, C);
 #define RYOLO_BN_REDK(A) (nt_red ? bn_act_bwd_reduce_kernel<A, true> : bn_act_bwd_reduce_kernel<A, false>)
 #define RYOLO_BN_RED(A)                                                                                                   \
     hipLaunchKernelGGL(RYOLO_BN_REDK(A), dim3((C / 8 + CT - 1) / CT, nslab), dim3(256), 0, stream,             \
@@ -534,6 +533,27 @@
 #undef RYOLO_BN_RED
     hipLaunchKernelGGL(bn_act_bwd_finalize_kernel, dim3((C + 31) / 32), dim3(1024), 0, stream, part, nslab, C, s1, s2,
                        scale ? dgamma : nullptr, dbeta, dsl ? s3 : nullptr);
+    out->s1 = s1; out->s2 = s2; out->s3 = s3; out->dslope = dsl;
+    return ok_launch();
+}
+
+}
+
+extern "C" {
+
+static int bn_act_bwd_impl(const void *z, int z_cstride, const void *dy, int dy_cstride, const float *scale, const float *shift,
+                           const float *mean, const float *invstd, int act, const float *slope, void *dz, int dz_cstride,
+                           long long npix, int C, float *dgamma, float *dbeta, float *dslope, void *workspace,
+                           size_t workspace_bytes, const float *pre_part, int pre_rows, void *stream_) {
+    if (scale && (!shift || !mean || !invstd || !dz || (dz_cstride & 7))) return RYOLO_EINVAL;
+    hipStream_t stream = (hipStream_t)stream_;
+    BnBwdSums sm;
+    const int rc = bn_act_bwd_sums(z, z_cstride, dy, dy_cstride, scale, shift, mean, invstd, act, slope, npix, C, dgamma, dbeta, dslope, workspace,
+                                   workspace_bytes, pre_part, pre_rows, stream, &sm);
+    if (rc != RYOLO_OK) return rc;
+    const float *s1 = sm.s1, *s2 = sm.s2, *s3 = sm.s3;
+    float *dsl = sm.dslope;
+    const bool nt_app = nt_pass(2, npix, C);
 #define RYOLO_BN_APP(A)                                                                                                   \
     hipLaunchKernelGGL((nt_app ? bn_act_bwd_apply_kernel<A, true> : bn_act_bwd_apply_kernel<A, false>), dim3(grid_for(npix * (C / 8), 256, ELEM_BLOCKS)), dim3(256), 0, stream,                  \
                        (const __bf16 *)z, z_cstride, (const __bf16 *)dy, dy_cstride, scale, shift, mean, invstd, s1, s2,  \
diff --git a/rotate-yolov3_amd/csrc/wgrad.hip b/rotate-yolov3_amd/csrc/wgrad.hip
--- a/rotate-yolov3_amd/csrc/wgrad.hip
+++ b/rotate-yolov3_amd/csrc/wgrad.hip
@@ -1,42 +1,9 @@
 #include "conv_common.h"
+#include "wgrad_frag.h"
 
 using namespace ryolo_detail;
 
 namespace {
-
-typedef short s16x4 __attribute__((ext_vector_type(4)));
-typedef short s16x8 __attribute__((ext_vector_type(8)));
-
-__device__ __forceinline__ s16x4 lds_read_tr16(const char *addr) {
-#if defined(__HIP_DEVICE_COMPILE__)
-    return __builtin_amdgcn_ds_read_tr16_b64_v4i16((__attribute__((address_space(3))) s16x4 *)(addr));
-#else
-    return s16x4{0, 0, 0, 0};
-#endif
-}
-
-template <int T>
-__device__ __forceinline__ int wg_swz(int row) {
-    if (T >= 128) return (row & 3) | (((row >> 3) & 1) << 2);
-    if (T == 64) return ((row >> 1) & 1) | (((row >> 3) & 1) << 1);
-    return (row >> 3) & 1;
-}
-
-typedef int i32x4 __attribute__((ext_vector_type(4)));
-__device__ __forceinline__ i32x4 make_rsrc_words(const void *base, unsigned bytes) {
-    const unsigned long long a = (unsigned long long)base;
-    i32x4 r;
-    r[0] = __builtin_amdgcn_readfirstlane((int)(unsigned)a);
-    r[1] = __builtin_amdgcn_readfirstlane((int)(unsigned)(a >> 32));
-    r[2] = __builtin_amdgcn_readfirstlane((int)bytes);
-    r[3] = 0x00020000;
-    return r;
-}
-__device__ __forceinline__ void buffer_load_lds16_raw(i32x4 rsrc, unsigned lds_addr , int voffset) {
-#if defined(__HIP_DEVICE_COMPILE__)
-    asm volatile("s_mov_b32 m0, %0\n\ts_nop 0\n\tbuffer_load_dwordx4 %1, %2, 0 offen lds" ::"s"(lds_addr), "v"(voffset), "s"(rsrc) : "memory", "m0");
-#endif
-}
 
 constexpr int KP = 64;
 
@@ -1058,6 +1025,19 @@
 
 }
 
+namespace ryolo_detail {
+
+bool wgrad_wide128_geometry(const ryolo_conv_desc *d, int Cin_real, WgradWide128 *g) {
+    if (!wgrad_validate(d) || Cin_real <= 0 || Cin_real > d->Cin) return false;
+    const WgradPlan w = wgrad_plan(d, Cin_real);
+    if (w.kernel != WG_128x128 || w.co_tiles != 1 || w.tap_groups != 1) return false;
+    g->S = w.S; g->chunk = w.chunk; g->Kpad = w.Kpad; g->Cout_pad = w.Cout_pad; g->ci_tiles = w.ci_tiles; g->M = w.M;
+    g->blocks = w.blocks; g->lds = w.lds; g->part_bytes = w.part_bytes;
+    return true;
+}
+
+}
+
 extern "C" {
 
 #ifdef RYOLO_MP_ABLATION
diff --git a/rotate-yolov3_amd/csrc/wgrad_frag.h b/rotate-yolov3_amd/csrc/wgrad_frag.h
--- /dev/null
+++ b/rotate-yolov3_amd/csrc/wgrad_frag.h
@@ -0,0 +1,40 @@
+#pragma once
+#include "conv_common.h"
+
+namespace ryolo_detail {
+
+typedef short s16x4 __attribute__((ext_vector_type(4)));
+typedef short s16x8 __attribute__((ext_vector_type(8)));
+
+__device__ __forceinline__ s16x4 lds_read_tr16(const char *addr) {
+#if defined(__HIP_DEVICE_COMPILE__)
+    return __builtin_amdgcn_ds_read_tr16_b64_v4i16((__attribute__((address_space(3))) s16x4 *)(addr));
+#else
+    return s16x4{0, 0, 0, 0};
+#endif
+}
+
+template <int T>
+__device__ __forceinline__ int wg_swz(int row) {
+    if (T >= 128) return (row & 3) | (((row >> 3) & 1) << 2);
+    if (T == 64) return ((row >> 1) & 1) | (((row >> 3) & 1) << 1);
+    return (row >> 3) & 1;
+}
+
+typedef int i32x4 __attribute__((ext_vector_type(4)));
+__device__ __forceinline__ i32x4 make_rsrc_words(const void *base, unsigned bytes) {
+    const unsigned long long a = (unsigned long long)base;
+    i32x4 r;
+    r[0] = __builtin_amdgcn_readfirstlane((int)(unsigned)a);
+    r[1] = __builtin_amdgcn_readfirstlane((int)(unsigned)(a >> 32));
+    r[2] = __builtin_amdgcn_readfirstlane((int)bytes);
+    r[3] = 0x00020000;
+    return r;
+}
+__device__ __forceinline__ void buffer_load_lds16_raw(i32x4 rsrc, unsigned lds_addr , int voffset) {
+#if defined(__HIP_DEVICE_COMPILE__)
+    asm volatile("s_mov_b32 m0, %0\n\ts_nop 0\n\tbuffer_load_dwordx4 %1, %2, 0 offen lds" ::"s"(lds_addr), "v"(voffset), "s"(rsrc) : "memory", "m0");
+#endif
+}
+
+}
diff --git a/rotate-yolov3_amd/model/hip_train_ops.py b/rotate-yolov3_amd/model/hip_train_ops.py
--- a/rotate-yolov3_amd/model/hip_train_ops.py
+++ b/rotate-yolov3_amd/model/hip_train_ops.py
@@ -292,6 +292,25 @@
     _lib.check(_lib.lib().ryolo_conv2d_wgrad_partials(C.byref(d), x.data_ptr(), dz.data_ptr(), dz.stride(2), cin_real, grad.data_ptr(),
                                                       1 if accumulate else 0, ws.data_ptr(), ws.numel(), _s(x.device)),
                "ryolo_conv2d_wgrad_partials")
+
+
+def conv1x1_bwd_fused_rows(d):
+    return _lib.lib().ryolo_conv1x1_bwd_fused_rows(C.byref(d))
+
+
+def conv1x1_bwd_fused(d, z, dy, stats, slope, dgamma, dbeta, dslope, part, bn_ws, x, ws_w, packed_dgrad, ones, zeros, dx, accumulate, prev=None,
+                      dz_out=None):
+    n, h, w, c = z.shape
+    mean, invstd, scale, shift = stats
+    p = lambda t: t.data_ptr() if t is not None else None
+    pz, pstats, pslope, part_out = prev if prev is not None else (None, (None, None, None, None), None, None)
+    pmean, pinvstd, pscale, pshift = pstats
+    _lib.check(_lib.lib().ryolo_conv1x1_bwd_fused(
+        C.byref(d), z.data_ptr(), z.stride(2), dy.data_ptr(), dy.stride(2), scale.data_ptr(), shift.data_ptr(), mean.data_ptr(), invstd.data_ptr(),
+        slope.data_ptr(), p(dz_out), dz_out.stride(2) if dz_out is not None else 0, p(dgamma), p(dbeta), p(dslope), p(part),
+        part.shape[0] if part is not None else 0, bn_ws.data_ptr(), bn_ws.numel(), x.data_ptr(), ws_w.data_ptr(), ws_w.numel(), packed_dgrad.data_ptr(), ones.data_ptr(), zeros.data_ptr(), dx.data_ptr(),
+        1 if accumulate else 0, p(pz), pz.stride(2) if pz is not None else 0, p(pscale), p(pshift), p(pmean), p(pinvstd), p(pslope), p(part_out),
+        _s(z.device)), "ryolo_conv1x1_bwd_fused")
 
 
 def _dil(dil):
diff --git a/rotate-yolov3_amd/model/plan.py b/rotate-yolov3_amd/model/plan.py
--- a/rotate-yolov3_amd/model/plan.py
+++ b/rotate-yolov3_amd/model/plan.py
@@ -380,6 +380,19 @@
     return TrainPlan(shp, buffers, x, act, grd, forward, blocks, backward)
 
 
+def fused_bwd_blocks(tp, enabled=True):
+    out = {}
+    for b in tp.blocks:
+        b.pop('fused_bwd', None)
+        g = b['xin_g']
+        if not enabled or not b['bn'] or b['recompute'] or g is None or g.cs != g.C:
+            continue
+        rows = _query('ryolo_conv1x1_bwd_fused_rows', b['desc'])
+        if rows > 0:
+            b['fused_bwd'] = out[b['layer']] = rows
+    return out
+
+
 def reduce_fusion_pairs(tp):
     by = {b['layer']: b for b in tp.blocks}
     pairs = []
diff --git a/rotate-yolov3_amd/model/train_engine.py b/rotate-yolov3_amd/model/train_engine.py
--- a/rotate-yolov3_amd/model/train_engine.py
+++ b/rotate-yolov3_amd/model/train_engine.py
@@ -132,12 +132,17 @@
                         and readers[i] == [i + 1]):
                     b['head_k'] = k
         self.batch_reduce = os.environ.get('RYOLO_WGRAD_BATCH_REDUCE', '1') != '0'
+        self.bneck_bwd = self.bneck_bwd_enabled()
         self._wr_batches = {}
         self._ws_w_bytes = max(wgrad_ws, 256)
         self._ws_w = None
         self.ws_b = torch.empty(max(bn_ws, 256), dtype=torch.uint8, device=device)
 
         self.bplan = [(kind, i, pl, flags) for (kind, i, pl), (_, _, flags) in zip(reversed(fwd), tp.backward)]
+
+    @staticmethod
+    def bneck_bwd_enabled():
+        return os.environ.get('RYOLO_BNECK_BWD', '1') != '0'
 
     @staticmethod
     def _conv_attrs(m):
@@ -266,6 +271,7 @@
             self._wr_batches = {}
             torch.cuda.empty_cache()
             self.batch_reduce = False
+            self._red_planned = False
             self.reduce_fallback = "per-layer split-K reduces on one shared workspace (the per-layer workspaces did not fit: %s)" % str(e)[:120]
             self.g_bwd = None
 
@@ -491,6 +497,14 @@
                 dy = b['dy']
                 if b['res_g'] is not None and not b['res_alias']:
                     self._passthrough(dy, b['res_g'], res_first)
+                if b.get('fused_bwd') and self.batch_reduce:
+                    y = b.get('red_for')
+                    tr.conv1x1_bwd_fused(b['desc'], b['z'], dy, b['stats'], b['slope'], self._grad_of(bn.weight), self._grad_of(bn.bias),
+                                         self._grad_of(b['act'].weight) if isinstance(b['act'], nn.PReLU) else None, b.get('red_part'), self.ws_b,
+                                         b['xin'], b['ws_w'], b['packed_d'], self.ones, self.zeros, b['xin_g'], not in_first,
+                                         prev=(y['z'], y['stats'], y['slope'], y['red_part']) if y is not None else None,
+                                         dz_out=b['dz'] if hook is not None else None)
+                    return
                 if bn is not None:
                     dsl = self._grad_of(b['act'].weight) if isinstance(b['act'], nn.PReLU) else None
                     if b['recompute'] and b['xin_g'] is None and b['dz'] is None:
@@ -548,14 +562,21 @@
 
     def _plan_reduce_fusion(self):
         self._red_planned = True
+        blk = {b['i']: b for b in self.blocks}
+        for b in self.blocks:
+            for key in ('fused_bwd', 'red_for', 'red_part'):
+                b.pop(key, None)
+        for layer, rows in plan.fused_bwd_blocks(self._tplan, self.bneck_bwd and self.batch_reduce).items():
+            b = blk[layer]
+            if b.get('actcode') == 1 and b.get('slope') is not None and b.get('stats') is not None and b.get('dz') is not None:
+                b['fused_bwd'] = rows
         if os.environ.get("RYOLO_BN_REDUCE_FUSION", "1") == "0":
             return
-        blk = {b['i']: b for b in self.blocks}
         pairs = []
         for xr, yr, rows in plan.reduce_fusion_pairs(self._tplan):
             x, y = blk[xr['layer']], blk[yr['layer']]
             if y.get('actcode') == 1 and y.get('slope') is not None and y.get('stats') is not None:
-                pairs.append((x, y, rows, x['xin_g'].shape[3]))
+                pairs.append((x, y, x.get('fused_bwd') or rows, x['xin_g'].shape[3]))
         if not pairs:
             return
         part = torch.empty(max(rows * 3 * c for _, _, rows, c in pairs), dtype=torch.float32, device=self.device)
```

Result: no change. 1362 images/s (-0.8%).
